# HKUST-Aerial-Robotics/MIND

Measured on AMD Instinct MI355X. Metric: sim steps/sec (whole node) + scenario-tree nodes expanded/sec, AV2 demo scenes, higher is better.
Workload: dtype f32-class (bf16 hi+mid+lo split operands = 24 significand bits, six products, fp32 accumulate) pair kernel + ActorNet, f32 elsewhere in the predictor, f64 iLQR

## Files before the change

### include/mind_hip.h

```cpp
#ifndef MIND_HIP_H
#define MIND_HIP_H

#include <stddef.h>
#include <stdint.h>

#ifdef __cplusplus
extern "C" {
#endif

#define MIND_OK 0
#define MIND_EINVAL (-1)
#define MIND_ENOMEM (-2)
#define MIND_EHIP (-3)
#define MIND_ESTATE (-4)
#define MIND_ENOTFOUND (-5)

typedef struct mind_ctx mind_ctx;

int mind_ctx_create(int device, void *stream, mind_ctx **out);
int mind_ctx_destroy(mind_ctx *ctx);
const char *mind_last_error_string(mind_ctx *ctx);
int mind_ctx_synchronize(mind_ctx *ctx);

typedef struct {
  const char *name;
  const float *data;
  int64_t numel;
} mind_tensor_desc;

int mind_weights_load(mind_ctx *ctx, const mind_tensor_desc *tensors, int n_tensors);

typedef struct {
  int n_scenes;
  const int32_t *actor_off;
  const int32_t *lane_off;
  const float *actors;
  const float *lanes;
  const float *lane_feat;
  const float *actor_ctrs;
  const float *actor_vecs;
  const float *lane_ctrs;
  const float *lane_vecs;
  const float *const *rpe;
  const float *tgt_nodes;
  const float *tgt_rpe;
} mind_scene_batch;

typedef struct {
  float *cls;
  float *reg;
  float *vel;
  float *lane_feat;
  float *actor_emb;
  float *cls_emb;
} mind_pred_out;

int mind_predict_batch(mind_ctx *ctx, const mind_scene_batch *in, mind_pred_out *out);

typedef struct {
  float *cov_vel;
  float *param;
} mind_pred_aux;
int mind_predict_batch_aux(mind_ctx *ctx, const mind_scene_batch *in, mind_pred_out *out, const mind_pred_aux *aux);

#define MIND_BASIS_BEZIER 0
#define MIND_BASIS_MONOMIAL 1
int mind_set_decoder_basis(mind_ctx *ctx, int basis);
int mind_get_decoder_basis(mind_ctx *ctx);

#define MIND_CURVE_MAX_POINTS (1LL << 26)
int mind_curve_eval(mind_ctx *ctx, int basis, const float *param, long long n_rows, const double *tau, int n_tau,
                    float *reg, float *vel, float *cov_vel);
int mind_debug_curve_basis(int basis, const double *tau, int n_tau, float *T, float *Tp);

int mind_last_fusion_stats(mind_ctx *ctx, int *n_launches, float *total_ms, double *pairs_processed);
int mind_last_actor_stats(mind_ctx *ctx, int *layerwise, int *n_launches, int *n_chunks, float *total_ms);
int mind_last_token_stats(mind_ctx *ctx, int *layerwise, int *n_launches, int *n_chunks, float *total_ms);
int mind_last_token_stage_ms(mind_ctx *ctx, float *out_ms, int cap);
int mind_last_ilqr_stats(mind_ctx *ctx, float *kernel_ms, int *n_trees, int *workgroups_per_tree);
int mind_last_ilqr_profile(mind_ctx *ctx, double *out9);
int mind_last_ilqr_trace(mind_ctx *ctx, int tree, int phase, double *out, int cap_rows, int *n_rows);
int mind_set_profiling(mind_ctx *ctx, int enable);
int mind_debug_launch_times(mind_ctx *ctx, int kind, float *clock_ms, float *event_ms, int cap, int *n_clock, int *n_event);
int mind_debug_launch_clock(int n_blocks, int block_slots, int rate_khz, const long long *ops, int n_ops, const unsigned long long *stamps,
                            long long n_slots, double *out, int cap);

#define MIND_PAIR_F32 0
#define MIND_PAIR_BF16X3 1
#define MIND_PAIR_BF16 2
#define MIND_PAIR_BF16X6 3
int mind_set_pair_precision(mind_ctx *ctx, int mode);

int mind_set_tuning(mind_ctx *ctx, const char *name, int value);
int mind_get_tuning(mind_ctx *ctx, const char *name, int *value);
int mind_debug_tuning(int index, const char *name, const char *text, int value, const char **out_name, const char **out_env, int *out_value);
int mind_debug_live_handles(void);
int mind_get_pair_precision(mind_ctx *ctx);
int mind_debug_pack_bfrag(const float *w, int row_stride, uint32_t *out);

int mind_debug_pair_schedule(const int *scene_tokens, const int *scene_actors, int n_scenes, int n_cu, int last_layer, int *out_jobs, int cap,
                             int *out_info);

int mind_debug_predict_choice(const char *const *knob_names, const int *knob_values, int n_knobs, int pair_prec, int n_cu, int have_side,
                              const int *scene_actors, const int *scene_lanes, int n_scenes, long long *out, int cap);

int mind_debug_ilqr_plan(const char *const *knob_names, const int *knob_values, int n_knobs, int n_cu, int mode, int n_trees, const int *n_nodes,
                         const int32_t *parents, long long *out, int cap, int *bad);

int mind_debug_aime_book(int pred_len, int max_depth, int max_rounds, int n_agents, int world, int rank, int force, int n_rounds, const int *dec_len,
                         const float *dec, int n_tokens, int bytes_per_pair, int plan_chunk_mb, int per_scene, long long *out, int cap, char *msg,
                         int msg_cap);

int mind_debug_wait_word(const unsigned *word, unsigned want, double timeout_s, double (*clock)(void *user), void *user, int spins_per_look);

int mind_debug_actor_lw_plan(int n_actors, int np, int chunk, long long *out_launches, int cap, long long *out_info);

int mind_debug_token_lw_plan(int n_tokens, int mode, int chunk, long long *out_launches, int cap, long long *out_info);

int mind_debug_pack_conv_frag(const float *w, int co, int ci, int ksz, uint32_t *out, size_t cap);

int mind_debug_pack(const char *what, const float *w, int a, int b, int c, float *out, size_t cap);
int mind_debug_weight_image(const mind_tensor_desc *tensors, int n_tensors, float *blob, size_t blob_cap, char *names, size_t names_cap,
                            long long *entries, int entries_cap, long long *out_info, char *msg, int msg_cap);
int mind_debug_weight_bind(const mind_tensor_desc *tensors, int n_tensors, const char *drop, char *msg, int msg_cap);

int mind_debug_trig(mind_ctx *ctx, const double *x, int n, double *out);

int mind_debug_dec_scene(mind_ctx *ctx, const float *rows, int n_scenes, int form, float *Cout, float *cls, int reps, float *ms);

int mind_debug_set_layers(mind_ctx *ctx, int n);
int64_t mind_debug_read(mind_ctx *ctx, const char *name, float *host, int64_t max_floats);

typedef struct {
  int n_nodes;
  const int32_t *parent;
  const float *prob;
  int n_agents;
  const float *agent_mean;
  const float *agent_cov;
  const double *field;
  const double *node_w;
} mind_cost_tree;

typedef struct {
  double dt, wheelbase;
  double w_des_state[6];
  double w_state_con[6];
  double state_lower[6], state_upper[6];
  double w_ctrl[2];
  double w_tgt, w_ego, w_ego_cov_offset, w_exo, w_exo_cov_offset, w_exo_cost_offset;
  double grid_res; int grid_w, grid_h;
  int max_iter;
} mind_ilqr_cfg;

typedef struct { int iterations; int converged; double J; double mu; } mind_ilqr_stats;

int mind_ilqr_solve_trees(mind_ctx *ctx, const mind_ilqr_cfg *cfg, const mind_cost_tree *trees,
                          int n_trees, const double *x0, const double *target_lane, int n_lane_pts,
                          double target_vel, int use_exo, const double *us_init, double *xs,
                          double *us, mind_ilqr_stats *stats);

int mind_ilqr_contingency(mind_ctx *ctx, const mind_ilqr_cfg *cfg_warm, const mind_ilqr_cfg *cfg_full,
                          const mind_cost_tree *trees, int n_trees, const double *x0,
                          const double *target_lane, int n_lane_pts, double target_vel, double *xs,
                          double *us, mind_ilqr_stats *stats_warm, mind_ilqr_stats *stats_full);
int mind_ilqr_contingency_begin(mind_ctx *ctx, const mind_ilqr_cfg *cfg_warm, const mind_ilqr_cfg *cfg_full,
                                const mind_cost_tree *trees, int n_trees, const double *x0,
                                const double *target_lane, int n_lane_pts, double target_vel, double *xs,
                                double *us, mind_ilqr_stats *stats_warm, mind_ilqr_stats *stats_full);
int mind_ilqr_contingency_begin_plan(mind_ctx *ctx, const mind_ilqr_cfg *cfg_warm, const mind_ilqr_cfg *cfg_full, const double *x0,
                                     const double *target_lane, int n_lane_pts, double target_vel, double *xs, double *us,
                                     mind_ilqr_stats *stats_warm, mind_ilqr_stats *stats_full);
int mind_ilqr_finish(mind_ctx *ctx);

typedef struct {
  int n_scenes;
  const int32_t *actor_off;
  const float *reg, *vel;
  const float *actor_ctrs, *actor_vecs;
  const float *rot, *orig;
  const float *cov_last;
  const int32_t *last;
  const float *target_lane;
  int n_lane_pts;
  const float *cls;
  const float *scen_prob;
  int lane_check;
  float dist_thres;
} mind_world_in;

typedef struct {
  float *world;
  float *topo;
  float *ego_end;
  float *sel, *sel_prob;
} mind_world_out;

int mind_aime_world(mind_ctx *ctx, const mind_world_in *in, const mind_world_out *out);

int mind_debug_aime_decide(mind_ctx *ctx, int n_scenes, const int32_t *actor_off, const int32_t *cmp, const float *cls, const float *scen_prob,
                           const float *topo, const float *ego_end, const float *world, int lane_check, float dist_thres, float prob_floor,
                           int fused, int by_value, float *sel, float *sel_prob, uint32_t *hit);

typedef struct {
  int n_scenes, n_agents, n_lanes;
  const float *pos, *ang, *vel;
  const float *types;
  const float *pad;
  const float *lane_ctrs, *lane_vecs;
  const float *target_lane;
  const float *target_lane_info;
  int n_lane_pts;
  float time_ahead, min_vel;
  const float *rows_dev;
  const int32_t *parent_slot;
  const int32_t *row0;
  const int32_t *dur;
  int prev_gen;
} mind_rebase_in;

typedef struct {
  float *actors;
  float *actor_ctrs, *actor_vecs;
  float *lane_ctrs, *lane_vecs;
  float *tgt_nodes, *tgt_rpe;
  float *frames;
  int32_t *gen;
} mind_rebase_out;

int mind_aime_rebase(mind_ctx *ctx, const mind_rebase_in *in, const mind_rebase_out *out);

typedef struct {
  int n_agents, n_lanes, n_lane_pts;
  const float *actors;
  const float *actor_ctrs, *actor_vecs;
  const float *lanes;
  const float *lane_ctrs, *lane_vecs;
  const float *tgt_nodes, *tgt_rpe;
  const float *rot, *orig, *tgt_pts;
  const float *hist;
  const float *types;
  const float *target_lane;
  const float *target_lane_info;
  float time_ahead, min_vel, dist_thres;
  int max_depth;
  int max_rounds;
  int pred_len;
  const float *raw_pos, *raw_ang, *raw_vel;
  const float *raw_pad;
  const double *lane_pts;
  const int32_t *lane_flags;
  float travel0;
  const float *script_cls, *script_reg, *script_vel;
  float prob_floor;
  const mind_ilqr_cfg *solve_cfg_warm, *solve_cfg_full;
  const double *solve_x0, *solve_lane;
  int solve_n_lane_pts;
  double solve_target_vel;
} mind_aime_plan_in;

#define MIND_AIME_BRANCH 1
#define MIND_AIME_END 2
#define MIND_AIME_TERMINATE 4
typedef struct {
  int round, scene, mode;
  int parent;
  float prob;
  int cur_t, end_t;
  int flags;
  int dur;
  int64_t row_off;
  float tgt_pts[22];
} mind_aime_node;

typedef struct {
  const mind_aime_node *nodes;
  int n_nodes;
  const float *rows;
  int64_t n_row_floats;
  int n_expanded, n_rounds;
  int root_flags;
  int round_scenes[32];
  float pair_ms;
// ... 233 lines not shown
```

### mind_amd/_lib.py

```python
import ctypes as C
import os

_HERE = os.path.dirname(os.path.abspath(__file__))
LIB_PATH = os.environ.get("MIND_HIP_LIB", os.path.join(_HERE, "libmind_hip.so"))

WAIT_CLOCK = C.CFUNCTYPE(C.c_double, C.c_void_p)
MIND_OK = 0
MIND_EINVAL, MIND_ENOMEM, MIND_EHIP, MIND_ESTATE, MIND_ENOTFOUND = -1, -2, -3, -4, -5


class TensorDesc(C.Structure):
    _fields_ = [("name", C.c_char_p), ("data", C.POINTER(C.c_float)), ("numel", C.c_int64)]


class SceneBatch(C.Structure):
    _fields_ = [("n_scenes", C.c_int), ("actor_off", C.POINTER(C.c_int32)), ("lane_off", C.POINTER(C.c_int32)),
                ("actors", C.c_void_p), ("lanes", C.c_void_p), ("lane_feat", C.c_void_p),
                ("actor_ctrs", C.c_void_p), ("actor_vecs", C.c_void_p), ("lane_ctrs", C.c_void_p),
                ("lane_vecs", C.c_void_p), ("rpe", C.POINTER(C.c_void_p)), ("tgt_nodes", C.c_void_p),
                ("tgt_rpe", C.c_void_p)]


class PredOut(C.Structure):
    _fields_ = [("cls", C.c_void_p), ("reg", C.c_void_p), ("vel", C.c_void_p), ("lane_feat", C.c_void_p),
# ... 47 lines not shown

class AuditRoadEpisodeOut(C.Structure):
    _fields_ = [("step_margin", C.POINTER(C.c_double)), ("step_corner", C.POINTER(C.c_int32)), ("step_ring", C.POINTER(C.c_int32)),
                ("step_edge", C.POINTER(C.c_int32)), ("ego_min", C.POINTER(C.c_double)), ("ego_step", C.POINTER(C.c_int32)),
                ("ego_corner", C.POINTER(C.c_int32)), ("ego_hits", C.POINTER(C.c_int32)), ("ego_first", C.POINTER(C.c_int32))]


class AuditTtcCfg(C.Structure):
    _fields_ = [("horizon", C.c_double), ("bound", C.c_double), ("lanes", C.c_int)]


class AuditTtcOut(C.Structure):
    _fields_ = [("step_ttc", C.POINTER(C.c_double)), ("step_track", C.POINTER(C.c_int32)), ("ego_min", C.POINTER(C.c_double)),
                ("ego_step", C.POINTER(C.c_int32)), ("ego_track", C.POINTER(C.c_int32)), ("ego_hits", C.POINTER(C.c_int32)),
                ("ego_first", C.POINTER(C.c_int32))]


class ForecastCfg(C.Structure):
    _fields_ = [("K", C.c_int), ("T", C.c_int), ("n_h", C.c_int), ("horizon", C.POINTER(C.c_int32)), ("miss_radius", C.c_double),
                ("disc_scale", C.c_double), ("disc_offset", C.c_double)]


FORECAST_OUT = (("ade", "f8", "a", True), ("fde", "f8", "a", True), ("cover", "i4", "a", True), ("first_out", "i4", "a", True),
                ("n_valid", "i4", "a", False), ("last", "i4", "a", False), ("k_ade", "i4", "a", False), ("k_fde", "i4", "a", False),
                ("brier_fde", "f8", "a", False), ("s_n_scored", "i4", "s", False), ("s_ade", "f8", "s", True), ("s_fde", "f8", "s", True),
                ("s_k_ade", "i4", "s", False), ("s_k_fde", "i4", "s", False), ("s_k_top", "i4", "s", False), ("s_brier_fde", "f8", "s", False),
                ("s_miss_rate", "f8", "s", False), ("s_miss_top", "f8", "s", False))


class ForecastOut(C.Structure):
    _fields_ = [(n, C.POINTER(C.c_double if dt == "f8" else C.c_int32)) for n, dt, _, _ in FORECAST_OUT]


class WorldIn(C.Structure):
    _fields_ = [("n_scenes", C.c_int), ("actor_off", C.POINTER(C.c_int32)), ("reg", C.c_void_p), ("vel", C.c_void_p),
                ("actor_ctrs", C.c_void_p), ("actor_vecs", C.c_void_p), ("rot", C.POINTER(C.c_float)),
                ("orig", C.POINTER(C.c_float)), ("cov_last", C.POINTER(C.c_float)), ("last", C.POINTER(C.c_int32)),
                ("target_lane", C.POINTER(C.c_float)), ("n_lane_pts", C.c_int), ("cls", C.c_void_p),
                ("scen_prob", C.POINTER(C.c_float)), ("lane_check", C.c_int), ("dist_thres", C.c_float)]


class WorldOut(C.Structure):
    _fields_ = [("world", C.c_void_p), ("topo", C.c_void_p), ("ego_end", C.c_void_p), ("sel", C.c_void_p), ("sel_prob", C.c_void_p)]


class RebaseIn(C.Structure):
    _fields_ = [("n_scenes", C.c_int), ("n_agents", C.c_int), ("n_lanes", C.c_int), ("pos", C.POINTER(C.c_float)),
                ("ang", C.POINTER(C.c_float)), ("vel", C.POINTER(C.c_float)), ("types", C.POINTER(C.c_float)),
                ("pad", C.POINTER(C.c_float)), ("lane_ctrs", C.POINTER(C.c_float)), ("lane_vecs", C.POINTER(C.c_float)),
                ("target_lane", C.POINTER(C.c_float)), ("target_lane_info", C.POINTER(C.c_float)), ("n_lane_pts", C.c_int),
                ("time_ahead", C.c_float), ("min_vel", C.c_float), ("rows_dev", C.c_void_p), ("parent_slot", C.POINTER(C.c_int32)),
                ("row0", C.POINTER(C.c_int32)), ("dur", C.POINTER(C.c_int32)), ("prev_gen", C.c_int)]


class RebaseOut(C.Structure):
    _fields_ = [("actors", C.c_void_p), ("actor_ctrs", C.c_void_p), ("actor_vecs", C.c_void_p), ("lane_ctrs", C.c_void_p),
                ("lane_vecs", C.c_void_p), ("tgt_nodes", C.c_void_p), ("tgt_rpe", C.c_void_p), ("frames", C.c_void_p),
                ("gen", C.POINTER(C.c_int32))]


class AimePlanIn(C.Structure):
    _fields_ = [("n_agents", C.c_int), ("n_lanes", C.c_int), ("n_lane_pts", C.c_int)] + \
               [(k, C.POINTER(C.c_float)) for k in ("actors", "actor_ctrs", "actor_vecs", "lanes", "lane_ctrs", "lane_vecs", "tgt_nodes", "tgt_rpe",
                                                    "rot", "orig", "tgt_pts", "hist", "types", "target_lane", "target_lane_info")] + \
               [("time_ahead", C.c_float), ("min_vel", C.c_float), ("dist_thres", C.c_float), ("max_depth", C.c_int), ("max_rounds", C.c_int), ("pred_len", C.c_int),
                ("raw_pos", C.POINTER(C.c_float)), ("raw_ang", C.POINTER(C.c_float)), ("raw_vel", C.POINTER(C.c_float)), ("raw_pad", C.POINTER(C.c_float)),
                ("lane_pts", C.POINTER(C.c_double)), ("lane_flags", C.POINTER(C.c_int32)), ("travel0", C.c_float),
                ("script_cls", C.c_void_p), ("script_reg", C.c_void_p), ("script_vel", C.c_void_p), ("prob_floor", C.c_float),
                ("solve_cfg_warm", C.c_void_p), ("solve_cfg_full", C.c_void_p), ("solve_x0", C.c_void_p), ("solve_lane", C.c_void_p),
                ("solve_n_lane_pts", C.c_int), ("solve_target_vel", C.c_double)]


class AimeNode(C.Structure):
    _fields_ = [("round", C.c_int), ("scene", C.c_int), ("mode", C.c_int), ("parent", C.c_int), ("prob", C.c_float),
                ("cur_t", C.c_int), ("end_t", C.c_int), ("flags", C.c_int), ("dur", C.c_int), ("row_off", C.c_int64),
                ("tgt_pts", C.c_float * 22)]


class AimePlanOut(C.Structure):
    _fields_ = [("nodes", C.POINTER(AimeNode)), ("n_nodes", C.c_int), ("rows", C.POINTER(C.c_float)), ("n_row_floats", C.c_int64),
                ("n_expanded", C.c_int), ("n_rounds", C.c_int), ("root_flags", C.c_int), ("round_scenes", C.c_int * 32),
                ("pair_ms", C.c_float), ("pair_launches", C.c_int), ("n_trees", C.c_int), ("tree_top", C.POINTER(C.c_int32)),
                ("tree_off", C.POINTER(C.c_int32)), ("flat_parent", C.POINTER(C.c_int32)), ("flat_prob", C.POINTER(C.c_float)),
                ("flat_mean", C.POINTER(C.c_float)), ("flat_cov", C.POINTER(C.c_float)), ("solves_begun", C.c_int)]


class IlqrCfg(C.Structure):
    _fields_ = [("dt", C.c_double), ("wheelbase", C.c_double), ("w_des_state", C.c_double * 6),
                ("w_state_con", C.c_double * 6), ("state_lower", C.c_double * 6), ("state_upper", C.c_double * 6),
                ("w_ctrl", C.c_double * 2), ("w_tgt", C.c_double), ("w_ego", C.c_double),
                ("w_ego_cov_offset", C.c_double), ("w_exo", C.c_double), ("w_exo_cov_offset", C.c_double),
                ("w_exo_cost_offset", C.c_double), ("grid_res", C.c_double), ("grid_w", C.c_int), ("grid_h", C.c_int),
                ("max_iter", C.c_int)]


class IlqrStats(C.Structure):
    _fields_ = [("iterations", C.c_int), ("converged", C.c_int), ("J", C.c_double), ("mu", C.c_double)]


LOOP_TAN_FN = C.CFUNCTYPE(C.c_double, C.c_double)
LOOP_SINCOS_FN = C.CFUNCTYPE(None, C.c_double, C.POINTER(C.c_double))


class LoopDesc(C.Structure):
    _fields_ = [("n_tracks", C.c_int), ("n_steps", C.c_int), ("clamp_last", C.c_int), ("ego_state", C.c_void_p), ("ego_state_is_f32", C.c_int), ("ego_obs", C.c_void_p), ("ego_trig32", C.c_void_p),
                ("tan_fn", C.c_void_p), ("sincos_fn", C.c_void_p), ("exo_obs", C.c_void_p),
                ("exo_valid", C.c_void_p), ("timestep", C.c_void_p), ("type_slot", C.c_void_p),
                ("sim_step", C.c_double), ("plan_step", C.c_double), ("enable_time", C.c_double),
                ("wheelbase", C.c_double), ("max_speed", C.c_double), ("max_steer", C.c_double), ("max_acc", C.c_double), ("max_dec", C.c_double),
                ("n_lanes", C.c_int), ("lane_pts", C.c_void_p), ("lane_flags", C.c_void_p),
                ("n_lane_pts", C.c_int), ("target_lane", C.c_void_p), ("target_lane_info", C.c_void_p),
                ("time_ahead", C.c_double), ("min_vel", C.c_float), ("dist_thres", C.c_float), ("max_depth", C.c_int), ("max_rounds", C.c_int),
                ("pred_len", C.c_int), ("prob_floor", C.c_float),
                ("cfg_warm", C.c_void_p), ("cfg_full", C.c_void_p), ("solve_n_lane_pts", C.c_int), ("solve_lane", C.c_void_p), ("target_vel", C.c_double),
                ("eval_n_lane_pts", C.c_int), ("eval_lane_is_f32", C.c_int), ("eval_lane", C.c_void_p), ("speculative", C.c_int)]


class LoopTotals(C.Structure):
    _fields_ = [("plans", C.c_longlong), ("expansions", C.c_longlong), ("scen_trees", C.c_longlong), ("rounds", C.c_longlong),
                ("aime_s", C.c_double), ("ilqr_s", C.c_double), ("total_s", C.c_double),
                ("iterations", C.c_longlong), ("node_iterations", C.c_longlong), ("node_iterations_exo", C.c_longlong),
                ("warm_speculated", C.c_longlong), ("warm_hits", C.c_longlong),
                ("pair_ms", C.c_double), ("pair_launches", C.c_longlong), ("scene_n2", C.c_double), ("scene_n_a1", C.c_double),
                ("ilqr_ms", C.c_double), ("ilqr_launches", C.c_longlong), ("ilqr_trees", C.c_longlong), ("ilqr_workgroups_per_tree", C.c_int),
                ("ilqr_prof", C.c_double * 9), ("ilqr_node_steps", C.c_double)]


class LoopOut(C.Structure):
    _fields_ = [("planned", C.c_int), ("enabled", C.c_int), ("n_steps", C.c_longlong), ("n_plans", C.c_longlong), ("episode_steps", C.c_longlong),
                ("sim_time", C.c_double), ("last_trigger", C.c_double), ("state", C.c_double * 4), ("ctrl", C.c_double * 2),
                ("n_agents", C.c_int), ("n_trees", C.c_int), ("best", C.c_int), ("n_expanded", C.c_int), ("n_rounds", C.c_int), ("n_traj_nodes", C.c_int),
                ("costs", C.POINTER(C.c_double)), ("aime_s", C.c_double), ("ilqr_s", C.c_double), ("total_s", C.c_double),
                ("tot", LoopTotals)]


PLANNER_EGO_KEY = -(1 << 63)


class PlannerDesc(C.Structure):
    _fields_ = [("time_ahead", C.c_double), ("min_vel", C.c_float), ("dist_thres", C.c_float), ("max_depth", C.c_int), ("max_rounds", C.c_int),
                ("pred_len", C.c_int), ("prob_floor", C.c_float), ("cfg_warm", C.c_void_p), ("cfg_full", C.c_void_p), ("speculative", C.c_int),
                ("ego_type_slot", C.c_int)]


class PlannerOut(C.Structure):
    _fields_ = [("n_plans", C.c_longlong),
                ("n_agents", C.c_int), ("n_trees", C.c_int), ("best", C.c_int), ("n_expanded", C.c_int), ("n_rounds", C.c_int), ("n_traj_nodes", C.c_int),
                ("costs", C.POINTER(C.c_double)), ("ctrl", C.c_double * 2), ("aime_s", C.c_double), ("ilqr_s", C.c_double), ("total_s", C.c_double),
                ("tot", LoopTotals)]


EXPORTS = ["mind_ctx_create", "mind_ctx_destroy", "mind_last_error_string", "mind_ctx_synchronize",
           "mind_weights_load", "mind_predict_batch", "mind_last_fusion_stats", "mind_last_actor_stats", "mind_debug_actor_lw_plan", "mind_last_token_stats", "mind_last_token_stage_ms", "mind_debug_token_lw_plan", "mind_set_profiling", "mind_debug_launch_times", "mind_debug_launch_clock",
           "mind_ilqr_solve_trees", "mind_ilqr_contingency", "mind_ilqr_solve_fields", "mind_cost_eval", "mind_ilqr_score_trees", "mind_ilqr_gains", "mind_ilqr_policy_rollouts", "mind_lane_dist_field", "mind_aime_world", "mind_aime_rebase", "mind_debug_aime_decide", "mind_debug_set_layers",
           "mind_debug_read", "mind_set_pair_precision", "mind_get_pair_precision", "mind_debug_pack_bfrag", "mind_debug_pack_conv_frag", "mind_debug_pack", "mind_debug_weight_image", "mind_debug_weight_bind", "mind_debug_pair_schedule", "mind_debug_predict_choice", "mind_debug_ilqr_plan", "mind_debug_aime_book", "mind_set_tuning", "mind_get_tuning", "mind_debug_tuning", "mind_debug_live_handles", "mind_last_ilqr_stats", "mind_aime_plan", "mind_last_ilqr_profile", "mind_eval_traj_trees", "mind_last_ilqr_trace", "mind_ilqr_contingency_begin", "mind_ilqr_finish", "mind_fill_tracks", "mind_ilqr_contingency_begin_plan", "mind_debug_trig", "mind_aime_plan_begin", "mind_aime_plan_poll", "mind_aime_plan_finish", "mind_ctx_busy", "mind_ilqr_finish_plan", "mind_debug_dec_scene",
           "mind_set_exchange", "mind_last_exchange_stats", "mind_debug_wait_word",
           "mind_predict_batch_aux", "mind_set_decoder_basis", "mind_get_decoder_basis", "mind_curve_eval", "mind_debug_curve_basis",
           "mind_audit_plan", "mind_audit_episode", "mind_debug_box_clearance",
           "mind_forecast_score", "mind_debug_forecast_score",
           "mind_audit_road_plan", "mind_audit_road_episode", "mind_debug_road_margin",
           "mind_audit_ttc", "mind_debug_box_ttc",
           "mind_loop_create", "mind_loop_destroy", "mind_loop_reset", "mind_loop_advance", "mind_loop_state", "mind_loop_last_plan", "mind_loop_export",
           "mind_planner_create", "mind_planner_destroy", "mind_planner_reset", "mind_planner_observe", "mind_planner_set_lanes", "mind_planner_set_target_lane",
           "mind_planner_set_solve_lane", "mind_planner_set_eval_lane", "mind_planner_plan", "mind_planner_last_plan", "mind_planner_export"]

EXCHANGE_FN = C.CFUNCTYPE(C.c_int, C.c_void_p, C.c_int, C.c_void_p, C.c_void_p, C.c_int64)
XCHG_ALLGATHER, XCHG_ALLREDUCE, XCHG_ALLTOALLV = 0, 1, 2

_lib = None


def load():
    global _lib
    if _lib is not None:
        return _lib
    if not os.path.exists(LIB_PATH):
        raise ImportError(f"{LIB_PATH} is missing: the HIP extension must be built (hipcc --offload-arch=gfx950); "
                          "there is no CPU fallback for the product path")
    lib = C.CDLL(LIB_PATH)
    lib.mind_ctx_create.argtypes = [C.c_int, C.c_void_p, C.POINTER(C.c_void_p)]
    lib.mind_ctx_destroy.argtypes = [C.c_void_p]
    lib.mind_last_error_string.argtypes = [C.c_void_p]
    lib.mind_last_error_string.restype = C.c_char_p
    lib.mind_ctx_synchronize.argtypes = [C.c_void_p]
    lib.mind_weights_load.argtypes = [C.c_void_p, C.POINTER(TensorDesc), C.c_int]
    lib.mind_predict_batch.argtypes = [C.c_void_p, C.POINTER(SceneBatch), C.POINTER(PredOut)]
    lib.mind_predict_batch_aux.argtypes = [C.c_void_p, C.POINTER(SceneBatch), C.POINTER(PredOut), C.POINTER(PredAux)]
    lib.mind_set_decoder_basis.argtypes = [C.c_void_p, C.c_int]
    lib.mind_get_decoder_basis.argtypes = [C.c_void_p]
    lib.mind_curve_eval.argtypes = [C.c_void_p, C.c_int, C.c_void_p, C.c_longlong, C.POINTER(C.c_double), C.c_int, C.c_void_p, C.c_void_p, C.c_void_p]
    lib.mind_debug_curve_basis.argtypes = [C.c_int, C.POINTER(C.c_double), C.c_int, C.POINTER(C.c_float), C.POINTER(C.c_float)]
    lib.mind_last_fusion_stats.argtypes = [C.c_void_p, C.POINTER(C.c_int), C.POINTER(C.c_float), C.POINTER(C.c_double)]
    lib.mind_last_actor_stats.argtypes = [C.c_void_p, C.POINTER(C.c_int), C.POINTER(C.c_int), C.POINTER(C.c_int), C.POINTER(C.c_float)]
    lib.mind_debug_actor_lw_plan.argtypes = [C.c_int, C.c_int, C.c_int, C.POINTER(C.c_longlong), C.c_int, C.POINTER(C.c_longlong)]
    lib.mind_last_token_stats.argtypes = [C.c_void_p, C.POINTER(C.c_int), C.POINTER(C.c_int), C.POINTER(C.c_int), C.POINTER(C.c_float)]
    lib.mind_last_token_stage_ms.argtypes = [C.c_void_p, C.POINTER(C.c_float), C.c_int]
    lib.mind_debug_token_lw_plan.argtypes = [C.c_int, C.c_int, C.c_int, C.POINTER(C.c_longlong), C.c_int, C.POINTER(C.c_longlong)]
    lib.mind_set_profiling.argtypes = [C.c_void_p, C.c_int]
    lib.mind_debug_launch_times.argtypes = [C.c_void_p, C.c_int, C.POINTER(C.c_float), C.POINTER(C.c_float), C.c_int, C.POINTER(C.c_int), C.POINTER(C.c_int)]
    lib.mind_debug_launch_clock.argtypes = [C.c_int, C.c_int, C.c_int, C.POINTER(C.c_longlong), C.c_int, C.POINTER(C.c_ulonglong), C.c_longlong,
                                            C.POINTER(C.c_double), C.c_int]
    lib.mind_ilqr_solve_trees.argtypes = [C.c_void_p, C.POINTER(IlqrCfg), C.POINTER(CostTree), C.c_int,
                                          C.POINTER(C.c_double), C.POINTER(C.c_double), C.c_int, C.c_double, C.c_int,
                                          C.POINTER(C.c_double), C.POINTER(C.c_double), C.POINTER(C.c_double),
                                          C.POINTER(IlqrStats)]
    lib.mind_ilqr_contingency.argtypes = [C.c_void_p, C.POINTER(IlqrCfg), C.POINTER(IlqrCfg), C.POINTER(CostTree), C.c_int,
                                          C.POINTER(C.c_double), C.POINTER(C.c_double), C.c_int, C.c_double,
                                          C.POINTER(C.c_double), C.POINTER(C.c_double), C.POINTER(IlqrStats), C.POINTER(IlqrStats)]
    lib.mind_ilqr_contingency_begin.argtypes = [C.c_void_p, C.POINTER(IlqrCfg), C.POINTER(IlqrCfg), C.POINTER(CostTree), C.c_int,
                                          C.POINTER(C.c_double), C.POINTER(C.c_double), C.c_int, C.c_double,
                                          C.POINTER(C.c_double), C.POINTER(C.c_double), C.POINTER(IlqrStats), C.POINTER(IlqrStats)]
    lib.mind_ilqr_finish.argtypes = [C.c_void_p]
    lib.mind_ilqr_contingency_begin_plan.argtypes = [C.c_void_p, C.POINTER(IlqrCfg), C.POINTER(IlqrCfg), C.c_void_p, C.c_void_p, C.c_int, C.c_double,
                                                     C.c_void_p, C.c_void_p, C.c_void_p, C.c_void_p]
    lib.mind_fill_tracks.argtypes = [C.c_void_p, C.c_int, C.c_int, C.c_void_p, C.c_void_p, C.c_void_p, C.c_void_p, C.c_void_p, C.c_void_p]
    lib.mind_ilqr_solve_fields.argtypes = [C.c_void_p, C.POINTER(IlqrCfg), C.POINTER(FieldGrid), C.POINTER(CostTree), C.c_int,
                                           C.POINTER(C.c_double), C.POINTER(C.c_double), C.POINTER(C.c_double),
                                           C.POINTER(C.c_double), C.POINTER(IlqrStats)]
    lib.mind_cost_eval.argtypes = [C.c_void_p, C.POINTER(IlqrCfg), C.POINTER(FieldGrid), C.POINTER(CostTree),
                                   C.POINTER(C.c_double), C.POINTER(C.c_double), C.c_int, C.c_double, C.c_int, C.c_int,
                                   C.POINTER(C.c_int32), C.POINTER(C.c_double), C.POINTER(C.c_double), C.POINTER(C.c_double)]
    lib.mind_ilqr_score_trees.argtypes = [C.c_void_p, C.POINTER(IlqrCfg), C.POINTER(FieldGrid), C.POINTER(CostTree), C.c_int,
                                          C.POINTER(C.c_double), C.POINTER(C.c_double), C.c_int, C.c_double, C.c_int, C.c_int,
                                          C.POINTER(C.c_double), C.POINTER(C.c_double), C.POINTER(C.c_double), C.POINTER(C.c_double)]
    lib.mind_ilqr_gains.argtypes = [C.c_void_p, C.POINTER(IlqrCfg), C.POINTER(FieldGrid), C.POINTER(CostTree), C.c_int,
                                    C.POINTER(C.c_double), C.POINTER(C.c_double), C.c_int, C.c_double, C.c_int,
                                    C.POINTER(C.c_double), C.POINTER(C.c_double), C.POINTER(IlqrGainsOut)]
    lib.mind_ilqr_policy_rollouts.argtypes = [C.c_void_p, C.POINTER(IlqrCfg), C.POINTER(FieldGrid), C.POINTER(CostTree), C.c_int,
                                              C.POINTER(C.c_double), C.POINTER(C.c_double), C.c_int, C.c_double, C.c_int,
                                              C.POINTER(C.c_double), C.POINTER(C.c_double), C.POINTER(C.c_double), C.c_int,
                                              C.POINTER(C.c_double), C.POINTER(C.c_double), C.POINTER(C.c_double), C.POINTER(C.c_double),
                                              C.POINTER(C.c_double), C.POINTER(C.c_double)]
    lib.mind_lane_dist_field.argtypes = [C.c_void_p, C.POINTER(C.c_double), C.POINTER(C.c_double), C.c_int, C.c_int, C.c_int,
                                         C.c_double] + [C.POINTER(C.c_double)] * 4
    lib.mind_aime_world.argtypes = [C.c_void_p, C.POINTER(WorldIn), C.POINTER(WorldOut)]
    lib.mind_aime_rebase.argtypes = [C.c_void_p, C.POINTER(RebaseIn), C.POINTER(RebaseOut)]
    lib.mind_debug_aime_decide.argtypes = [C.c_void_p, C.c_int, C.POINTER(C.c_int32), C.POINTER(C.c_int32), C.c_void_p, C.POINTER(C.c_float), C.c_void_p,
                                           C.c_void_p, C.c_void_p, C.c_int, C.c_float, C.c_float, C.c_int, C.c_int, C.c_void_p, C.c_void_p, C.c_void_p]
    lib.mind_aime_plan.argtypes = [C.c_void_p, C.POINTER(AimePlanIn), C.POINTER(AimePlanOut)]
    lib.mind_aime_plan_begin.argtypes = [C.c_void_p, C.POINTER(AimePlanIn)]
    lib.mind_aime_plan_poll.argtypes = [C.c_void_p]
    lib.mind_aime_plan_finish.argtypes = [C.c_void_p, C.POINTER(AimePlanOut)]
    lib.mind_ctx_busy.argtypes = [C.c_void_p]
    lib.mind_ilqr_finish_plan.argtypes = [C.c_void_p, C.c_int, C.c_int, C.c_void_p, C.c_void_p, C.c_void_p, C.c_void_p]
    lib.mind_set_pair_precision.argtypes = [C.c_void_p, C.c_int]
    lib.mind_set_tuning.argtypes = [C.c_void_p, C.c_char_p, C.c_int]
    lib.mind_get_tuning.argtypes = [C.c_void_p, C.c_char_p, C.POINTER(C.c_int)]
    lib.mind_debug_tuning.argtypes = [C.c_int, C.c_char_p, C.c_char_p, C.c_int, C.POINTER(C.c_char_p), C.POINTER(C.c_char_p), C.POINTER(C.c_int)]
    lib.mind_debug_live_handles.argtypes = []
    lib.mind_last_ilqr_stats.argtypes = [C.c_void_p, C.POINTER(C.c_float), C.POINTER(C.c_int), C.POINTER(C.c_int)]
    lib.mind_last_ilqr_profile.argtypes = [C.c_void_p, C.POINTER(C.c_double)]
    lib.mind_last_ilqr_trace.argtypes = [C.c_void_p, C.c_int, C.c_int, C.POINTER(C.c_double), C.c_int, C.POINTER(C.c_int)]
    lib.mind_eval_traj_trees.argtypes = [C.POINTER(C.c_double), C.POINTER(C.c_double), C.POINTER(C.c_int32), C.c_int, C.c_void_p, C.c_int, C.c_int,
                                         C.c_double, C.POINTER(C.c_double)]
    lib.mind_get_pair_precision.argtypes = [C.c_void_p]
    lib.mind_debug_pack_bfrag.argtypes = [C.POINTER(C.c_float), C.c_int, C.POINTER(C.c_uint32)]
    lib.mind_debug_pair_schedule.argtypes = [C.POINTER(C.c_int), C.POINTER(C.c_int), C.c_int, C.c_int, C.c_int, C.POINTER(C.c_int), C.c_int, C.POINTER(C.c_int)]
    lib.mind_debug_predict_choice.argtypes = [C.POINTER(C.c_char_p), C.POINTER(C.c_int), C.c_int, C.c_int, C.c_int, C.c_int, C.POINTER(C.c_int), C.POINTER(C.c_int),
                                              C.c_int, C.POINTER(C.c_longlong), C.c_int]
    lib.mind_debug_ilqr_plan.argtypes = [C.POINTER(C.c_char_p), C.POINTER(C.c_int), C.c_int, C.c_int, C.c_int, C.c_int, C.POINTER(C.c_int), C.POINTER(C.c_int32),
                                         C.POINTER(C.c_longlong), C.c_int, C.POINTER(C.c_int)]
    lib.mind_debug_wait_word.argtypes = [C.POINTER(C.c_uint), C.c_uint, C.c_double, WAIT_CLOCK, C.c_void_p, C.c_int]
    lib.mind_debug_aime_book.argtypes = [C.c_int] * 8 + [C.POINTER(C.c_int), C.POINTER(C.c_float)] + [C.c_int] * 4 + [C.POINTER(C.c_longlong), C.c_int, C.c_char_p, C.c_int]
    lib.mind_debug_trig.argtypes = [C.c_void_p, C.POINTER(C.c_double), C.c_int, C.POINTER(C.c_double)]
    lib.mind_debug_pack_conv_frag.argtypes = [C.POINTER(C.c_float), C.c_int, C.c_int, C.c_int, C.POINTER(C.c_uint32), C.c_size_t]
    lib.mind_debug_pack.argtypes = [C.c_char_p, C.POINTER(C.c_float), C.c_int, C.c_int, C.c_int, C.POINTER(C.c_float), C.c_size_t]
    lib.mind_debug_weight_image.argtypes = [C.POINTER(TensorDesc), C.c_int, C.POINTER(C.c_float), C.c_size_t, C.c_char_p, C.c_size_t,
                                            C.POINTER(C.c_longlong), C.c_int, C.POINTER(C.c_longlong), C.c_char_p, C.c_int]
    lib.mind_debug_weight_bind.argtypes = [C.POINTER(TensorDesc), C.c_int, C.c_char_p, C.c_char_p, C.c_int]
    lib.mind_debug_dec_scene.argtypes = [C.c_void_p, C.POINTER(C.c_float), C.c_int, C.c_int, C.POINTER(C.c_float), C.POINTER(C.c_float), C.c_int, C.POINTER(C.c_float)]
    lib.mind_debug_set_layers.argtypes = [C.c_void_p, C.c_int]
    lib.mind_debug_read.argtypes = [C.c_void_p, C.c_char_p, C.POINTER(C.c_float), C.c_int64]
    lib.mind_set_exchange.argtypes = [C.c_void_p, C.c_int, C.c_int, EXCHANGE_FN, C.c_void_p, C.c_int]
    lib.mind_last_exchange_stats.argtypes = [C.c_void_p, C.POINTER(C.c_longlong), C.POINTER(C.c_longlong)]
    lib.mind_loop_create.argtypes = [C.c_void_p, C.POINTER(LoopDesc), C.POINTER(C.c_void_p)]
    lib.mind_loop_destroy.argtypes = [C.c_void_p]
    lib.mind_loop_reset.argtypes = [C.c_void_p]
    lib.mind_loop_advance.argtypes = [C.c_void_p, C.c_int, C.c_double, C.c_longlong, C.POINTER(LoopOut)]
    lib.mind_loop_state.argtypes = [C.c_void_p, C.POINTER(LoopOut)]
    lib.mind_loop_last_plan.argtypes = [C.c_void_p, C.POINTER(AimePlanOut)] + [C.POINTER(C.c_void_p)] * 6 + [C.c_void_p]
    lib.mind_loop_export.argtypes = [C.c_void_p, C.c_int, C.POINTER(C.c_int), C.c_void_p, C.c_void_p, C.c_void_p]
    lib.mind_planner_create.argtypes = [C.c_void_p, C.POINTER(PlannerDesc), C.POINTER(C.c_void_p)]
    lib.mind_planner_destroy.argtypes = [C.c_void_p]
    lib.mind_planner_reset.argtypes = [C.c_void_p]
    lib.mind_planner_observe.argtypes = [C.c_void_p, C.c_int, C.c_void_p, C.c_int, C.c_void_p, C.c_void_p, C.c_void_p]
    lib.mind_planner_set_lanes.argtypes = [C.c_void_p, C.c_int, C.c_void_p, C.c_void_p]
    lib.mind_planner_set_target_lane.argtypes = [C.c_void_p, C.c_int, C.c_void_p, C.c_void_p]
    lib.mind_planner_set_solve_lane.argtypes = [C.c_void_p, C.c_int, C.c_void_p, C.c_double]
    lib.mind_planner_set_eval_lane.argtypes = [C.c_void_p, C.c_int, C.c_void_p, C.c_int]
    lib.mind_planner_plan.argtypes = [C.c_void_p, C.c_void_p, C.c_void_p, C.POINTER(PlannerOut)]
    lib.mind_planner_last_plan.argtypes = [C.c_void_p, C.POINTER(AimePlanOut)] + [C.POINTER(C.c_void_p)] * 6 + [C.c_void_p]
    lib.mind_planner_export.argtypes = [C.c_void_p, C.c_int, C.POINTER(C.c_int), C.c_void_p, C.c_void_p, C.c_void_p]
    lib.mind_audit_plan.argtypes = [C.c_void_p, C.POINTER(AuditBox), C.c_double, C.POINTER(CostTree), C.c_int, C.c_int, C.POINTER(C.c_double),
                                    C.POINTER(AuditPlanOut)]
    lib.mind_audit_episode.argtypes = [C.c_void_p, C.POINTER(AuditBox), C.c_int, C.c_int, C.c_int, C.POINTER(C.c_double), C.POINTER(C.c_double),
                                       C.POINTER(C.c_uint8), C.POINTER(C.c_double), C.POINTER(AuditEpisodeOut)]
    lib.mind_debug_box_clearance.argtypes = [C.c_int, C.c_int, C.POINTER(C.c_double), C.POINTER(C.c_double), C.POINTER(C.c_double), C.POINTER(C.c_double)]
    fc_tail = [C.POINTER(ForecastCfg), C.c_int, C.POINTER(C.c_int32), C.c_void_p, C.c_void_p, C.POINTER(C.c_double), C.POINTER(C.c_uint8),
               C.POINTER(C.c_uint8), C.POINTER(ForecastOut)]
    lib.mind_forecast_score.argtypes = [C.c_void_p] + fc_tail
    lib.mind_debug_forecast_score.argtypes = fc_tail
    road = [C.POINTER(C.c_double), C.POINTER(C.c_int32), C.c_int]
    lib.mind_audit_road_plan.argtypes = [C.c_void_p, C.POINTER(AuditBox)] + road + [C.POINTER(CostTree), C.c_int, C.c_int, C.POINTER(C.c_double),
                                                                                   C.POINTER(AuditRoadPlanOut)]
    lib.mind_audit_road_episode.argtypes = [C.c_void_p, C.POINTER(AuditBox)] + road + [C.c_int, C.c_int, C.POINTER(C.c_double),
                                                                                      C.POINTER(AuditRoadEpisodeOut)]
    lib.mind_debug_road_margin.argtypes = [C.c_int, C.POINTER(C.c_double), C.POINTER(AuditBox)] + road + [C.POINTER(C.c_double), C.POINTER(C.c_double)] + \
        [C.POINTER(C.c_int32)] * 3
    lib.mind_audit_ttc.argtypes = [C.c_void_p, C.POINTER(AuditBox), C.POINTER(AuditTtcCfg), C.c_int, C.c_int, C.c_int, C.POINTER(C.c_double),
                                   C.POINTER(C.c_double), C.POINTER(C.c_uint8), C.POINTER(C.c_double), C.POINTER(AuditTtcOut)]
    lib.mind_debug_box_ttc.argtypes = [C.c_int, C.POINTER(C.c_double), C.POINTER(C.c_double), C.POINTER(C.c_double), C.POINTER(C.c_double)]
    for n in EXPORTS:
        getattr(lib, n)
        if n not in ("mind_last_error_string", "mind_debug_read"):
            getattr(lib, n).restype = C.c_int
    lib.mind_debug_read.restype = C.c_int64
    _lib = lib
    return lib


PRED_CHOICE_FIELDS = ("header", "n_runs", "np", "actor_form", "actor_arg", "actor_grid", "actor_chunk", "actor_chunks", "actor_launches", "qsplit", "qk_stride",
                      "tiled", "edge_bf16", "edge_pair_bytes", "tok_chunk", "tok_lw", "tok_chunks", "pair_family", "pair_np", "l5_jobs5", "xcd_lanes",
                      "xcd_lanes5", "dec_actor", "dec_np", "fp32_dec", "split_dec", "want_mw", "mw_blocks", "cls_on_side", "tgt_wait_first",
                      "dec_head_ra", "dec_chain_g")
PAIR_PREC = ("f32", "bf16x3", "bf16", "bf16x6")


def predict_choice(knobs, prec, scenes, n_cu=256, have_side=True):
    lib = load()
    names = (C.c_char_p * max(1, len(knobs)))(*[k.encode() for k in knobs])
    vals = (C.c_int * max(1, len(knobs)))(*[int(v) for v in knobs.values()])
    sa = (C.c_int * len(scenes))(*[a for a, _ in scenes])
    sl = (C.c_int * len(scenes))(*[l for _, l in scenes])
    cap = 32 + 6 * len(scenes)
    out = (C.c_longlong * cap)()
    n = lib.mind_debug_predict_choice(names, vals, len(knobs), PAIR_PREC.index(prec) if isinstance(prec, str) else prec, n_cu, int(have_side),
                                      sa, sl, len(scenes), out, cap)
    if n == MIND_EINVAL:
        return None
    assert 0 < n <= cap and out[0] == 32 and n == 32 + 6 * out[1], n
    d = dict(zip(PRED_CHOICE_FIELDS, out[:32]))
    d["runs"] = [tuple(out[32 + 6 * i:38 + 6 * i]) for i in range(out[1])]
    return d


def dec_scene(lib, ctx, rows, form, reps=1, timed=False):
    import numpy as np
    rows = np.ascontiguousarray(rows, np.float32)
    B = rows.shape[0]
    assert rows.shape == (B, 128)
    fp = C.POINTER(C.c_float)
    cout, cls, ms = np.empty((B, 6, 128), np.float32), np.empty((B, 6), np.float32), np.zeros(reps, np.float32)
    check(lib, ctx, lib.mind_debug_dec_scene(ctx, rows.ctypes.data_as(fp), B, int(form), cout.ctypes.data_as(fp), cls.ctypes.data_as(fp), reps,
                                             ms.ctypes.data_as(fp) if timed else None), "mind_debug_dec_scene")
    return (cout, cls, ms) if timed else (cout, cls)


def knobs():
    lib = load()
    name, env, val = C.c_char_p(), C.c_char_p(), C.c_int()
    rows = []
    while not rows or len(rows) < n:
        n = lib.mind_debug_tuning(len(rows), None, None, 0, C.byref(name), C.byref(env), C.byref(val))
        assert n > 0, n
        rows.append((name.value.decode(), env.value.decode() if env.value else None, val.value))
    return rows


def knob_stored(name, value=None, text=None):
    val = C.c_int()
    rc = load().mind_debug_tuning(-1, name.encode(), None if text is None else text.encode(), 0 if value is None else int(value), None, None, C.byref(val))
    return val.value if rc == MIND_OK else None


ILQR_PLAN_FIELDS = ("header", "n_trees", "form", "G", "GS", "spec", "nslot", "grid", "workgroups_per_tree", "host_out", "early", "starve_followers")
ILQR_TREE_FIELDS = ("M", "nl", "nseg", "nsl", "maxls", "nfs")
ILQR_TREE_TABLES = ("level_start", "level_nodes", "child_start", "child_list", "seg_start", "seg_nodes", "slevel_start", "slevel_segs", "seg_rec",
                    "fstep_start", "fstep_items", "fstep_q1", "fstep_nstart", "fstep_nodes")


def ilqr_plan(knobs, parents, n_cu=256, generic=False, evaluate=False, two_fits=False):
    lib = load()
    names = (C.c_char_p * max(1, len(knobs)))(*[k.encode() for k in knobs])
    vals = (C.c_int * max(1, len(knobs)))(*[int(v) for v in knobs.values()])
    nn = (C.c_int * len(parents))(*[len(p) for p in parents])
    flat = [int(v) for p in parents for v in p]
    par = (C.c_int32 * max(1, len(flat)))(*flat)
    bad = (C.c_int * 2)()
    mode = int(generic) | int(evaluate) << 1 | int(two_fits) << 2
    n = lib.mind_debug_ilqr_plan(names, vals, len(knobs), n_cu, mode, len(parents), nn, par, None, 0, bad)
    if n == MIND_EINVAL:
        return {"bad": (bad[0], bad[1])} if bad[0] >= 0 else None
    out = (C.c_longlong * n)()
    assert lib.mind_debug_ilqr_plan(names, vals, len(knobs), n_cu, mode, len(parents), nn, par, out, n, bad) == n and out[0] == 16
    d = dict(zip(ILQR_PLAN_FIELDS, out[:12]))
    d["trees"], o = [], 16
    for _ in parents:
        tr = dict(zip(ILQR_TREE_FIELDS, out[o:o + 6]))
        lens, o = out[o + 6:o + 20], o + 20
        for name, ln in zip(ILQR_TREE_TABLES, lens):
            tr[name], o = list(out[o:o + ln]), o + ln
        d["trees"].append(tr)
    assert o == n
    return d


AIME_ROUND_FIELDS = ("B", "lo", "hi", "Bmax", "chunk", "S", "s0", "Sm", "any")
AIME_NODE_FIELDS = ("round", "scene", "mode", "parent", "prob", "cur_t", "end_t", "flags", "dur", "row_off", "owner", "lscene")


def aime_book(pred_len, max_depth, n_agents, rounds, world=1, rank=0, force=False, max_rounds=32, n_tokens=0, bytes_per_pair=512, plan_chunk_mb=96 * 1024,
              per_scene=1):
    import numpy as np
    lib = load()
    arrs = [np.ascontiguousarray(r, np.float32).ravel() for r in rounds]
    lens = (C.c_int * max(1, len(arrs)))(*[a.size for a in arrs])
    dec = np.concatenate(arrs + [np.zeros(1, np.float32)])
    msg = C.create_string_buffer(256)
    args = [pred_len, max_depth, max_rounds, n_agents, world, rank, int(force), len(arrs), lens, dec.ctypes.data_as(C.POINTER(C.c_float)), n_tokens,
            bytes_per_pair, plan_chunk_mb, per_scene]
    n = lib.mind_debug_aime_book(*args, None, 0, msg, 256)
    if n == MIND_EINVAL:
        return None
    out = (C.c_longlong * n)()
# ... 223 lines not shown
```

### mind_amd/csrc/actor_mfma_kernels.hip

```cpp
#include <hip/hip_runtime.h>
#include <stdint.h>

#define AM_T 1024
#ifdef MIND_ACTOR_TRACE
__device__ long long am_tr_[64];
__device__ int am_trn_;
#define AM_MARK() do { if (blockIdx.x == 0 && threadIdx.x == 0) { const long long n_ = clock64(); am_tr_[am_trn_ & 63] = n_; ++am_trn_; } } while (0)
#else
#define AM_MARK() do {} while (0)
#endif
#define AM_WAVES 16
#define AM_MAXT 2
#define AM_RSD(C) (3 * (C) / 2 + 4)
#define AM_BUF 2496
#define AM_XIN 0
#define AM_O0 1344
#define AM_FA (AM_O0 + 7 * AM_BUF)
#define AM_RED (AM_FA + 48 * AM_RSD(128))
#define AM_LDS_DWORDS (AM_RED + 64)

#include "weight_tables.h"
#include "launch_clock.h"
typedef u32 u32x2 __attribute__((ext_vector_type(2)));

__device__ __forceinline__ float am_block_sum(float v, float *red, int flip) {
  v = wave_sum(v);
  float *r = red + (flip & 1) * 32;
  if ((threadIdx.x & 63) == 0) r[threadIdx.x >> 6] = v;
  __syncthreads();
  float s = 0.f;
#pragma unroll
  for (int w = 0; w < AM_WAVES; ++w) s += r[w];
  return s;
}

template <int NP>
__device__ __forceinline__ void am_store_split(u32 *rowp, int plane, const f32x4 &y) {
  u32x2 h, m, l;
  h[0] = pk_bf16(y[0], y[1]); h[1] = pk_bf16(y[2], y[3]);
  *(u32x2 *)rowp = h;
  if (NP == 1) return;
  const float r0 = y[0] - bf_lo_f32(h[0]), r1 = y[1] - bf_hi_f32(h[0]), r2 = y[2] - bf_lo_f32(h[1]), r3 = y[3] - bf_hi_f32(h[1]);
  m[0] = pk_bf16(r0, r1); m[1] = pk_bf16(r2, r3);
  *(u32x2 *)(rowp + plane) = m;
  l[0] = pk_bf16(r0 - bf_lo_f32(m[0]), r1 - bf_hi_f32(m[0])); l[1] = pk_bf16(r2 - bf_lo_f32(m[1]), r3 - bf_hi_f32(m[1]));
  *(u32x2 *)(rowp + 2 * plane) = l;
}
template <int NP>
__device__ __forceinline__ f32x4 am_load_split(const u32 *rowp, int plane) {
  const u32x2 h = *(const u32x2 *)rowp;
  f32x4 y = {bf_lo_f32(h[0]), bf_hi_f32(h[0]), bf_lo_f32(h[1]), bf_hi_f32(h[1])};
  if (NP == 1) return y;
  const u32x2 m = *(const u32x2 *)(rowp + plane), l = *(const u32x2 *)(rowp + 2 * plane);
  y[0] = (y[0] + bf_lo_f32(m[0])) + bf_lo_f32(l[0]); y[1] = (y[1] + bf_hi_f32(m[0])) + bf_hi_f32(l[0]);
  y[2] = (y[2] + bf_lo_f32(m[1])) + bf_lo_f32(l[1]); y[3] = (y[3] + bf_hi_f32(m[1])) + bf_hi_f32(l[1]);
  return y;
}

template <int NP, int LGC , int KSZ, int STRIDE>
__device__ __forceinline__ void am_conv(const u32 *in, int Tin, const u32 *__restrict__ Wf, int Cout, int Tout,
                                        f32x4 (&acc)[AM_MAXT]) {
  constexpr int CP = 1 << LGC, RSD = AM_RSD(CP), PLANE = CP / 2, PAD = (KSZ - 1) / 2;
  constexpr int KS = (KSZ * CP + 31) / 32;
  const int lane = threadIdx.x & 63, wave = threadIdx.x >> 6;
  const int r = lane & 15, q = lane >> 4;
  const int ntt = (Tout + 15) >> 4;
  const int tiles = (Cout >> 4) * ntt;
#pragma unroll
  for (int i = 0; i < AM_MAXT; ++i) {
    acc[i] = (f32x4){0.f, 0.f, 0.f, 0.f};
    const int ti = wave + AM_WAVES * i;
    if (ti >= tiles) continue;
    const int mt = ti / ntt, nt = ti - mt * ntt;
    const int t = nt * 16 + r;
    const u32 *wp = Wf + (size_t)mt * KS * 768 + lane * 4;
    f32x4 corr = {0.f, 0.f, 0.f, 0.f};
#pragma unroll 4
    for (int ks = 0; ks < KS; ++ks) {
      const u32x4 ah = *(const u32x4 *)(wp + (size_t)ks * 768);
      u32x4 am, al;
      if (NP >= 3) am = *(const u32x4 *)(wp + (size_t)ks * 768 + 256);
      if (NP == 6) al = *(const u32x4 *)(wp + (size_t)ks * 768 + 512);
      const int k0 = ks * 32 + q * 8;
      const int dk = k0 >> LGC, ci = k0 & (CP - 1);
      const int row = t * STRIDE + dk - PAD;
      u32x4 bh = {0u, 0u, 0u, 0u}, bm = {0u, 0u, 0u, 0u}, bl = {0u, 0u, 0u, 0u};
      if (dk < KSZ && t < Tout && row >= 0 && row < Tin) {
        const u32 *bp = in + row * RSD + (ci >> 1);
        bh = *(const u32x4 *)bp;
        if (NP >= 3) bm = *(const u32x4 *)(bp + PLANE);
        if (NP == 6) bl = *(const u32x4 *)(bp + 2 * PLANE);
      }
      acc[i] = MFMA_BF(ah, bh, acc[i]);
      if (NP >= 3) {
        if (NP == 6) {
          corr = MFMA_BF(al, bh, corr);
          corr = MFMA_BF(ah, bl, corr);
          corr = MFMA_BF(am, bm, corr);
        }
        corr = MFMA_BF(am, bh, corr);
        corr = MFMA_BF(ah, bm, corr);
      }
    }
    if (NP >= 3) acc[i] += corr;
  }
}

template <int NP>
__device__ __forceinline__ void am_gn(f32x4 (&acc)[AM_MAXT], int Cout, int Tout, const float *__restrict__ g,
                                      const float *__restrict__ b, const u32 *resid, const float *up, bool relu, u32 *outs,
                                      float *outf, float *__restrict__ gout, float *red) {
  const int lane = threadIdx.x & 63, wave = threadIdx.x >> 6;
  const int r = lane & 15, q = lane >> 4;
  const int ntt = (Tout + 15) >> 4;
  const int tiles = (Cout >> 4) * ntt;
  const int RSD = AM_RSD(Cout), PLANE = Cout >> 1;
  f32x4 gg[AM_MAXT], bb[AM_MAXT];
  float s = 0.f;
#pragma unroll
  for (int i = 0; i < AM_MAXT; ++i) {
    const int ti = wave + AM_WAVES * i;
    if (ti >= tiles) continue;
    const int mt = ti / ntt, nt = ti - mt * ntt;
    gg[i] = *(const f32x4 *)(g + mt * 16 + q * 4);
    bb[i] = *(const f32x4 *)(b + mt * 16 + q * 4);
    if (nt * 16 + r < Tout) s += (acc[i][0] + acc[i][1]) + (acc[i][2] + acc[i][3]);
  }
  const float n = (float)(Cout * Tout);
  const float mean = am_block_sum(s, red, 0) / n;
  float v = 0.f;
#pragma unroll
  for (int i = 0; i < AM_MAXT; ++i) {
    const int ti = wave + AM_WAVES * i;
    if (ti >= tiles) continue;
    const int nt = ti % ntt;
    if (nt * 16 + r < Tout) {
#pragma unroll
      for (int e = 0; e < 4; ++e) { const float d = acc[i][e] - mean; v = fmaf(d, d, v); }
    }
  }
  const float rstd = 1.0f / sqrtf(am_block_sum(v, red, 1) / n + 1e-5f);
#pragma unroll
  for (int i = 0; i < AM_MAXT; ++i) {
    const int ti = wave + AM_WAVES * i;
    if (ti >= tiles) continue;
    const int mt = ti / ntt, nt = ti - mt * ntt;
    const int t = nt * 16 + r, co = mt * 16 + q * 4;
    if (t >= Tout) continue;
    f32x4 y;
#pragma unroll
    for (int e = 0; e < 4; ++e) y[e] = (acc[i][e] - mean) * rstd * gg[i][e] + bb[i][e];
    if (resid) y += am_load_split<NP>(resid + t * RSD + (co >> 1), PLANE);
    if (up) {
      const int Th = Tout >> 1;
      float sp = (t + 0.5f) * 0.5f - 0.5f;
      sp = sp < 0.f ? 0.f : sp;
      const int i0 = (int)sp;
      const int i1 = i0 + 1 < Th ? i0 + 1 : Th - 1;
      const float l1 = sp - (float)i0;
      const f32x4 a0 = *(const f32x4 *)(up + i0 * 132 + co), a1 = *(const f32x4 *)(up + i1 * 132 + co);
#pragma unroll
      for (int e = 0; e < 4; ++e) y[e] += (1.0f - l1) * a0[e] + l1 * a1[e];
    }
    if (relu) {
#pragma unroll
      for (int e = 0; e < 4; ++e) y[e] = fmaxf(y[e], 0.f);
    }
    if (gout) {
      if (t == Tout - 1) *(f32x4 *)(gout + co) = y;
    } else if (outf) {
      *(f32x4 *)(outf + t * 132 + co) = y;
    } else {
      am_store_split<NP>(outs + t * RSD + (co >> 1), PLANE, y);
    }
  }
  __syncthreads();
}

template <int NP, int LGCI, int LGCO, int STRIDE, bool DS>
__device__ __forceinline__ void am_res(const u32 *in, int Tin, const AmRes &W, u32 *out, u32 *t1, u32 *t2, float *red) {
  constexpr int Cout = 1 << LGCO;
  const int Tout = Tin / STRIDE;
  f32x4 acc[AM_MAXT];
  am_conv<NP, LGCI, 3, STRIDE>(in, Tin, W.c1, Cout, Tout, acc);
  AM_MARK();
  am_gn<NP>(acc, Cout, Tout, W.g1, W.b1, nullptr, nullptr, true, t1, nullptr, nullptr, red);
  AM_MARK();
  const u32 *resid = in;
  if (DS) {
    am_conv<NP, LGCI, 1, STRIDE>(in, Tin, W.ds, Cout, Tout, acc);
    AM_MARK();
    am_gn<NP>(acc, Cout, Tout, W.gd, W.bd, nullptr, nullptr, false, t2, nullptr, nullptr, red);
    AM_MARK();
    resid = t2;
  }
  am_conv<NP, LGCO, 3, 1>(t1, Tout, W.c2, Cout, Tout, acc);
  AM_MARK();
  am_gn<NP>(acc, Cout, Tout, W.g2, W.b2, resid, nullptr, true, out, nullptr, nullptr, red);
  AM_MARK();
}

template <int NP, int LGC>
__device__ __forceinline__ void am_lateral(const u32 *src, int T, const AmLat &W, const float *up, float *dstf, u32 *dsts,
                                           float *red) {
  f32x4 acc[AM_MAXT];
  am_conv<NP, LGC, 3, 1>(src, T, W.w, 128, T, acc);
  AM_MARK();
  am_gn<NP>(acc, 128, T, W.g, W.b, nullptr, up, false, dsts, dstf, nullptr, red);
  AM_MARK();
}

template <int NP>
__global__ __launch_bounds__(AM_T) void k_actor_mfma(const float *__restrict__ actors , int n_actors,
                                                     float *__restrict__ out , AmW W, LcSlot *clk) {
  lc_stamp_in(clk);
  extern __shared__ __attribute__((aligned(16))) u32 smu[];
  u32 *xin = smu + AM_XIN;
  u32 *o0 = smu + AM_O0, *o1 = o0 + AM_BUF, *o2 = o1 + AM_BUF, *o3 = o2 + AM_BUF;
  u32 *ta = o3 + AM_BUF, *tb = ta + AM_BUF, *tc = tb + AM_BUF;
  u32 *fa = smu + AM_FA;
  float *red = (float *)(smu + AM_RED);
  const int tid = threadIdx.x;
  const int a = blockIdx.x;
  if (a >= n_actors) { lc_stamp_both(clk); return; }
  if (tid < 48 * 8) {
    const int t = tid >> 3, c = (tid & 7) * 2;
    const float v0 = c < 14 ? actors[((size_t)a * 14 + c) * 48 + t] : 0.f;
    const float v1 = c + 1 < 14 ? actors[((size_t)a * 14 + c + 1) * 48 + t] : 0.f;
    u32 *p = xin + t * AM_RSD(16) + (c >> 1);
    const u32 h = pk_bf16(v0, v1);
    const float r0 = v0 - bf_lo_f32(h), r1 = v1 - bf_hi_f32(h);
    const u32 m = pk_bf16(r0, r1);
    p[0] = h; p[8] = m; p[16] = pk_bf16(r0 - bf_lo_f32(m), r1 - bf_hi_f32(m));
  }
  __syncthreads();
#ifdef MIND_ACTOR_TRACE
  if (blockIdx.x == 0 && tid == 0) am_trn_ = 0;
#endif
  AM_MARK();
  am_res<NP, 4, 5, 1, true>(xin, 48, W.res[0], ta, tb, tc, red);
  am_res<NP, 5, 5, 1, false>(ta, 48, W.res[1], o0, tb, tc, red);
  am_res<NP, 5, 6, 2, true>(o0, 48, W.res[2], ta, tb, tc, red);
  am_res<NP, 6, 6, 1, false>(ta, 24, W.res[3], o1, tb, tc, red);
  am_res<NP, 6, 7, 2, true>(o1, 24, W.res[4], ta, tb, tc, red);
  am_res<NP, 7, 7, 1, false>(ta, 12, W.res[5], o2, tb, tc, red);
  am_res<NP, 7, 8, 2, true>(o2, 12, W.res[6], ta, tb, tc, red);
  am_res<NP, 8, 8, 1, false>(ta, 6, W.res[7], o3, tb, tc, red);
  am_lateral<NP, 8>(o3, 6, W.lat[3], nullptr, (float *)ta, nullptr, red);
  am_lateral<NP, 7>(o2, 12, W.lat[2], (const float *)ta, (float *)tb, nullptr, red);
  am_lateral<NP, 6>(o1, 24, W.lat[1], (const float *)tb, (float *)o2, nullptr, red);
  am_lateral<NP, 5>(o0, 48, W.lat[0], (const float *)o2, nullptr, fa, red);
  {
    const AmRes &R = W.res[8];
    f32x4 acc[AM_MAXT];
    am_conv<NP, 7, 3, 1>(fa, 48, R.c1, 128, 48, acc);
    AM_MARK();
    am_gn<NP>(acc, 128, 48, R.g1, R.b1, nullptr, nullptr, true, o0, nullptr, nullptr, red);
    AM_MARK();
    am_conv<NP, 7, 3, 1>(o0, 48, R.c2, 128, 48, acc);
    AM_MARK();
    am_gn<NP>(acc, 128, 48, R.g2, R.b2, fa, nullptr, true, nullptr, nullptr, out + (size_t)a * 128, red);
    AM_MARK();
  }
#ifdef MIND_ACTOR_TRACE
  if (blockIdx.x == 0 && tid == 0) {
    printf("[k_actor_mfma<%d>] cycles conv/gn per stage:", NP);
    for (int q = 1; q < am_trn_ && q < 64; ++q) printf(" %lld", am_tr_[q] - am_tr_[q - 1]);
    printf("\n");
  }
#endif
  lc_stamp_out(clk);
}
extern "C" size_t mind_actor_mfma_lds_bytes() { return (size_t)AM_LDS_DWORDS * sizeof(u32); }
```

### mind_amd/csrc/encdec_kernels.hip

```cpp
#include <hip/hip_runtime.h>
#include <stdint.h>

#include "weight_tables.h"
#include "dec_curve.h"
#include "launch_clock.h"
#include "dec_chain.h"

typedef float f32x4 __attribute__((ext_vector_type(4)));

#define NT 256

__device__ __forceinline__ float wave_sum(float v) {
  v += __shfl_xor(v, 32, 64);
  v += __shfl_xor(v, 16, 64);
  v += __shfl_xor(v, 8, 64);
  v += __shfl_xor(v, 4, 64);
  v += __shfl_xor(v, 2, 64);
  v += __shfl_xor(v, 1, 64);
  return v;
}

__device__ __forceinline__ float block_sum(float v, float *red) {
  v = wave_sum(v);
  __syncthreads();
  if ((threadIdx.x & 63) == 0) red[threadIdx.x >> 6] = v;
  __syncthreads();
  return red[0] + red[1] + red[2] + red[3];
}

#ifndef DB
#define DB 16
#endif
#define DENSE_ROW_FENCE() __builtin_amdgcn_sched_barrier(0)
#define DBQ 8
template <int R>
__device__ __forceinline__ void dense_quads(const float *in, int ldi, int K, const float *__restrict__ WT,
                                            const float *__restrict__ b, int NOUT, float *out, int ldo,
                                            float *part, int part_floats) {
  const int nthr = blockDim.x;
  const int NQ = NOUT >> 2;
  int KP = 1;
  while (KP * 2 * NQ <= nthr && KP * 2 * R * NOUT <= part_floats && KP * 2 <= (K >> 2)) KP *= 2;
  const int Kc = ((K / 4 + KP - 1) / KP) * 4;
  for (int item = threadIdx.x; item < KP * NQ; item += nthr) {
    const int kp = item / NQ, o = (item % NQ) * 4;
    float acc[R][4];
#pragma unroll
    for (int r = 0; r < R; ++r)
#pragma unroll
      for (int c = 0; c < 4; ++c) acc[r][c] = (KP == 1 && b) ? b[o + c] : 0.f;
    const int k0 = kp * Kc, k1 = min(K, k0 + Kc);
    int k = k0;
    for (; k + DBQ <= k1; k += DBQ) {
      f32x4 w[DBQ];
#pragma unroll
      for (int q = 0; q < DBQ; ++q) w[q] = *(const f32x4 *)(WT + (size_t)(k + q) * NOUT + o);
#pragma unroll
      for (int r = 0; r < R; ++r) {
#pragma unroll
        for (int q4 = 0; q4 < DBQ / 4; ++q4) {
          const f32x4 x = *(const f32x4 *)(in + r * ldi + k + 4 * q4);
#pragma unroll
          for (int j = 0; j < 4; ++j)
#pragma unroll
            for (int c = 0; c < 4; ++c) acc[r][c] = fmaf(w[4 * q4 + j][c], x[j], acc[r][c]);
        }
        DENSE_ROW_FENCE();
      }
    }
    for (; k < k1; k += 4) {
#pragma unroll
      for (int j = 0; j < 4; ++j) {
        const f32x4 w = *(const f32x4 *)(WT + (size_t)(k + j) * NOUT + o);
#pragma unroll
        for (int r = 0; r < R; ++r) {
          const float x = in[r * ldi + k + j];
#pragma unroll
          for (int c = 0; c < 4; ++c) acc[r][c] = fmaf(w[c], x, acc[r][c]);
        }
      }
    }
#pragma unroll
    for (int r = 0; r < R; ++r)
#pragma unroll
      for (int c = 0; c < 4; ++c) {
        if (KP == 1) out[r * ldo + o + c] = acc[r][c];
        else part[(kp * R + r) * NOUT + o + c] = acc[r][c];
      }
  }
  if (KP == 1) return;
  __syncthreads();
  for (int i = threadIdx.x; i < R * NOUT; i += nthr) {
    const int r = i / NOUT, oo = i % NOUT;
    float v = b ? b[oo] : 0.f;
    for (int q = 0; q < KP; ++q) v += part[(q * R + r) * NOUT + oo];
    out[r * ldo + oo] = v;
  }
}

#ifndef DT
#define DT 1024
#endif
template <int R>
__device__ __forceinline__ void dense_quads_part(const float *in, int ldi, int K, const float *__restrict__ WT, const float *__restrict__ b, int NOUT,
                                                 float *out, int ldo, float *part, int part_floats, int wg, int G) {
  const int nthr = blockDim.x;
  const int NQ = NOUT >> 2;
  int KP = 1;
  while (KP * 2 * NQ <= DT && KP * 2 * R * NOUT <= part_floats && KP * 2 <= (K >> 2)) KP *= 2;
  const int Kc = ((K / 4 + KP - 1) / KP) * 4;
  const int q_lo = NQ * wg / G, q_hi = NQ * (wg + 1) / G, NQg = q_hi - q_lo;
  for (int item = threadIdx.x; item < KP * NQg; item += nthr) {
    const int kp = item / NQg, o = (q_lo + item % NQg) * 4;
    float acc[R][4];
#pragma unroll
    for (int r = 0; r < R; ++r)
#pragma unroll
      for (int c = 0; c < 4; ++c) acc[r][c] = (KP == 1 && b) ? b[o + c] : 0.f;
    const int k0 = kp * Kc, k1 = min(K, k0 + Kc);
    int k = k0;
    for (; k + DBQ <= k1; k += DBQ) {
      f32x4 w[DBQ];
#pragma unroll
      for (int q = 0; q < DBQ; ++q) w[q] = *(const f32x4 *)(WT + (size_t)(k + q) * NOUT + o);
#pragma unroll
      for (int r = 0; r < R; ++r) {
#pragma unroll
        for (int q4 = 0; q4 < DBQ / 4; ++q4) {
          const f32x4 x = *(const f32x4 *)(in + r * ldi + k + 4 * q4);
#pragma unroll
          for (int j = 0; j < 4; ++j)
#pragma unroll
            for (int c = 0; c < 4; ++c) acc[r][c] = fmaf(w[4 * q4 + j][c], x[j], acc[r][c]);
        }
        DENSE_ROW_FENCE();
      }
    }
    for (; k < k1; k += 4) {
#pragma unroll
      for (int j = 0; j < 4; ++j) {
        const f32x4 w = *(const f32x4 *)(WT + (size_t)(k + j) * NOUT + o);
#pragma unroll
        for (int r = 0; r < R; ++r) {
          const float x = in[r * ldi + k + j];
#pragma unroll
          for (int c = 0; c < 4; ++c) acc[r][c] = fmaf(w[c], x, acc[r][c]);
        }
      }
    }
#pragma unroll
    for (int r = 0; r < R; ++r)
#pragma unroll
      for (int c = 0; c < 4; ++c) {
        if (KP == 1) out[r * ldo + o + c] = acc[r][c];
        else part[(kp * R + r) * NOUT + o + c] = acc[r][c];
      }
  }
  if (KP == 1) return;
  __syncthreads();
  const int o_lo = q_lo * 4, no = NQg * 4;
  for (int i = threadIdx.x; i < R * no; i += nthr) {
    const int r = i / no, oo = o_lo + i % no;
    float v = b ? b[oo] : 0.f;
    for (int q = 0; q < KP; ++q) v += part[(q * R + r) * NOUT + oo];
    out[r * ldo + oo] = v;
  }
}

#define DEC_SYNC_SPINS (1u << 22)
__device__ __forceinline__ bool dec_grid_sync(unsigned *bar, int G, unsigned *abort_word) {
  __shared__ int sh_ab;
  __syncthreads();
  if (threadIdx.x == 0) {
// ... 51 lines not shown
    return;
  }
  int KP = 1;
  if (part && NOUT < nthr) {
    KP = nthr / NOUT;
    while (KP > 1 && (KP * R * NOUT > part_floats || (K / 4) < KP)) KP >>= 1;
    int p2 = 1;
    while (p2 * 2 <= KP) p2 *= 2;
    KP = p2;
  }
  if (KP == 1) {
    for (int o = threadIdx.x; o < NOUT; o += nthr) {
      float acc[R];
      const float bv = b ? b[o] : 0.f;
#pragma unroll
      for (int r = 0; r < R; ++r) acc[r] = bv;
      int k = 0;
      for (; k + DB <= K; k += DB) {
        float w[DB];
#pragma unroll
        for (int q = 0; q < DB; ++q) w[q] = WT[(size_t)(k + q) * NOUT + o];
#pragma unroll
        for (int r = 0; r < R; ++r) {
#pragma unroll
          for (int q4 = 0; q4 < DB / 4; ++q4) {
            const f32x4 x = *(const f32x4 *)(in + r * ldi + k + 4 * q4);
            acc[r] = fmaf(w[4 * q4 + 0], x[0], acc[r]);
            acc[r] = fmaf(w[4 * q4 + 1], x[1], acc[r]);
            acc[r] = fmaf(w[4 * q4 + 2], x[2], acc[r]);
            acc[r] = fmaf(w[4 * q4 + 3], x[3], acc[r]);
          }
        DENSE_ROW_FENCE();
        }
      }
      for (; k < K; k += 4) {
#pragma unroll
        for (int r = 0; r < R; ++r) {
          const f32x4 x = *(const f32x4 *)(in + r * ldi + k);
#pragma unroll
          for (int q = 0; q < 4; ++q) acc[r] = fmaf(WT[(size_t)(k + q) * NOUT + o], x[q], acc[r]);
        }
      }
#pragma unroll
      for (int r = 0; r < R; ++r) out[r * ldo + o] = acc[r];
    }
    return;
  }
  const int kp = threadIdx.x / NOUT, o = threadIdx.x % NOUT;
  const int Kc = ((K / 4 + KP - 1) / KP) * 4;
  if (kp < KP) {
    float acc[R];
#pragma unroll
    for (int r = 0; r < R; ++r) acc[r] = 0.f;
    const int k0 = kp * Kc, k1 = min(K, k0 + Kc);
    int k = k0;
    for (; k + DB <= k1; k += DB) {
      float w[DB];
#pragma unroll
      for (int q = 0; q < DB; ++q) w[q] = WT[(size_t)(k + q) * NOUT + o];
#pragma unroll
      for (int r = 0; r < R; ++r) {
#pragma unroll
        for (int q4 = 0; q4 < DB / 4; ++q4) {
          const f32x4 x = *(const f32x4 *)(in + r * ldi + k + 4 * q4);
          acc[r] = fmaf(w[4 * q4 + 0], x[0], acc[r]);
          acc[r] = fmaf(w[4 * q4 + 1], x[1], acc[r]);
          acc[r] = fmaf(w[4 * q4 + 2], x[2], acc[r]);
          acc[r] = fmaf(w[4 * q4 + 3], x[3], acc[r]);
        }
        DENSE_ROW_FENCE();
      }
    }
    for (; k < k1; k += 4) {
#pragma unroll
      for (int r = 0; r < R; ++r) {
        const f32x4 x = *(const f32x4 *)(in + r * ldi + k);
#pragma unroll
        for (int q = 0; q < 4; ++q) acc[r] = fmaf(WT[(size_t)(k + q) * NOUT + o], x[q], acc[r]);
      }
    }
#pragma unroll
    for (int r = 0; r < R; ++r) part[(kp * R + r) * NOUT + o] = acc[r];
  }
  __syncthreads();
  for (int i = threadIdx.x; i < R * NOUT; i += nthr) {
    const int r = i / NOUT, oo = i % NOUT;
    float v = b ? b[oo] : 0.f;
    for (int q = 0; q < KP; ++q) v += part[(q * R + r) * NOUT + oo];
    out[r * ldo + oo] = v;
  }
}

constexpr int dense_scalar_kp(int R, int NOUT, int K, int nthr, int part_floats) {
  int KP = NOUT < nthr ? nthr / NOUT : 1;
  while (KP > 1 && (KP * R * NOUT > part_floats || (K / 4) < KP)) KP >>= 1;
  int p2 = 1;
  while (p2 * 2 <= KP) p2 *= 2;
  return p2;
}

template <int R, int RPT>
__device__ __forceinline__ void dense_ksplit(const float *in, int ldi, int K, const float *__restrict__ WT, const float *__restrict__ b, int NOUT,
                                             float *out, int ldo, float *part, int KP) {
  const int nthr = blockDim.x;
  constexpr int NG = (R + RPT - 1) / RPT;
  const int Kc = ((K / 4 + KP - 1) / KP) * 4;
  for (int item = threadIdx.x; item < NG * KP * NOUT; item += nthr) {
    const int o = item % NOUT, kp = (item / NOUT) % KP, r0 = (item / (NOUT * KP)) * RPT;
    float acc[RPT];
#pragma unroll
    for (int j = 0; j < RPT; ++j) acc[j] = 0.f;
    const int k0 = kp * Kc, k1 = min(K, k0 + Kc);
    int k = k0;
    for (; k + DB <= k1; k += DB) {
      float w[DB];
#pragma unroll
      for (int q = 0; q < DB; ++q) w[q] = WT[(size_t)(k + q) * NOUT + o];
#pragma unroll
      for (int j = 0; j < RPT; ++j) {
        if (r0 + j >= R) continue;
#pragma unroll
        for (int q4 = 0; q4 < DB / 4; ++q4) {
          const f32x4 x = *(const f32x4 *)(in + (r0 + j) * ldi + k + 4 * q4);
          acc[j] = fmaf(w[4 * q4 + 0], x[0], acc[j]);
          acc[j] = fmaf(w[4 * q4 + 1], x[1], acc[j]);
          acc[j] = fmaf(w[4 * q4 + 2], x[2], acc[j]);
          acc[j] = fmaf(w[4 * q4 + 3], x[3], acc[j]);
        }
      }
    }
    for (; k < k1; k += 4) {
#pragma unroll
      for (int j = 0; j < RPT; ++j) {
        if (r0 + j >= R) continue;
        const f32x4 x = *(const f32x4 *)(in + (r0 + j) * ldi + k);
#pragma unroll
        for (int q = 0; q < 4; ++q) acc[j] = fmaf(WT[(size_t)(k + q) * NOUT + o], x[q], acc[j]);
      }
    }
#pragma unroll
    for (int j = 0; j < RPT; ++j)
      if (r0 + j < R) part[(kp * R + r0 + j) * NOUT + o] = acc[j];
  }
  __syncthreads();
  for (int i = threadIdx.x; i < R * NOUT; i += nthr) {
    const int r = i / NOUT, oo = i % NOUT;
    float v = b ? b[oo] : 0.f;
    for (int q = 0; q < KP; ++q) v += part[(q * R + r) * NOUT + oo];
    out[r * ldo + oo] = v;
  }
}

#define LN_REGS 12
__device__ __forceinline__ void ln_rows(float *buf, int ld, int R, int n, const float *__restrict__ g,
                                        const float *__restrict__ be, bool relu) {
  const int lane = threadIdx.x & 63, wave = threadIdx.x >> 6, nw = blockDim.x >> 6;
  for (int r = wave; r < R; r += nw) {
    if (n <= 64 * LN_REGS) {
      float xv[LN_REGS], gv[LN_REGS], bv[LN_REGS];
#pragma unroll
      for (int i = 0; i < LN_REGS; ++i) {
        const int k = lane + 64 * i;
        const bool in = k < n;
        xv[i] = in ? buf[r * ld + k] : 0.f;
        gv[i] = in ? g[k] : 0.f;
        bv[i] = in ? be[k] : 0.f;
      }
      float s = 0.f;
#pragma unroll
      for (int i = 0; i < LN_REGS; ++i) if (lane + 64 * i < n) s += xv[i];
      const float mean = wave_sum(s) / (float)n;
      float v = 0.f;
#pragma unroll
      for (int i = 0; i < LN_REGS; ++i) if (lane + 64 * i < n) { const float d = xv[i] - mean; v = fmaf(d, d, v); }
      const float rstd = 1.0f / sqrtf(wave_sum(v) / (float)n + 1e-5f);
#pragma unroll
      for (int i = 0; i < LN_REGS; ++i) {
        const int k = lane + 64 * i;
        if (k < n) {
          float y = (xv[i] - mean) * rstd * gv[i] + bv[i];
          if (relu) y = fmaxf(y, 0.f);
          buf[r * ld + k] = y;
        }
      }
      continue;
    }
    float s = 0.f;
    for (int k = lane; k < n; k += 64) s += buf[r * ld + k];
    const float mean = wave_sum(s) / (float)n;
    float v = 0.f;
    for (int k = lane; k < n; k += 64) { const float d = buf[r * ld + k] - mean; v = fmaf(d, d, v); }
    const float rstd = 1.0f / sqrtf(wave_sum(v) / (float)n + 1e-5f);
    for (int k = lane; k < n; k += 64) {
      float y = (buf[r * ld + k] - mean) * rstd * g[k] + be[k];
      if (relu) y = fmaxf(y, 0.f);
      buf[r * ld + k] = y;
    }
  }
}

#define PL 2
#define LR (PL * 10)

#ifndef DT
#define DT 1024
#endif
__global__ __launch_bounds__(DT) void k_lane_net(const float *__restrict__ feats, int n_poly,
                                                 float *__restrict__ out, LaneW W) {
  __shared__ __attribute__((aligned(16))) float xin[LR][16];
  __shared__ __attribute__((aligned(16))) float x[LR][128];
  __shared__ __attribute__((aligned(16))) float hcat[LR][256];
  __shared__ __attribute__((aligned(16))) float t1[LR][128];
  __shared__ __attribute__((aligned(16))) float part[2 * LR * 128];
  const int PF = 2 * LR * 128;
  const int tid = threadIdx.x;
  const int p0 = blockIdx.x * PL;
  for (int i = tid; i < LR * 16; i += blockDim.x) {
    const int r = i / 16, c = i % 16;
    const int pl = p0 + r / 10;
    xin[r][c] = pl < n_poly ? feats[((size_t)pl * 10 + r % 10) * 16 + c] : 0.f;
  }
  __syncthreads();
  dense<LR>(&xin[0][0], 16, 16, W.pW, W.pb, 128, &x[0][0], 128, part, PF);
  __syncthreads();
  ln_rows(&x[0][0], 128, LR, 128, W.pg, W.pbe, true);
  __syncthreads();
  for (int blk = 0; blk < 2; ++blk) {
    dense<LR>(&x[0][0], 128, 128, W.f10W[blk], W.f10b[blk], 128, &t1[0][0], 128, part, PF);
    __syncthreads();
    ln_rows(&t1[0][0], 128, LR, 128, W.f10g[blk], W.f10be[blk], true);
    __syncthreads();
    dense<LR>(&t1[0][0], 128, 128, W.f13W[blk], W.f13b[blk], 128, &hcat[0][0], 256, part, PF);
    __syncthreads();
    ln_rows(&hcat[0][0], 256, LR, 128, W.f13g[blk], W.f13be[blk], true);
    __syncthreads();
    for (int i = tid; i < PL * 128; i += blockDim.x) {
      const int pl = i / 128, c = i % 128;
      float m = hcat[pl * 10][c];
      for (int q = 1; q < 10; ++q) m = fmaxf(m, hcat[pl * 10 + q][c]);
      for (int q = 0; q < 10; ++q) hcat[pl * 10 + q][128 + c] = m;
    }
    __syncthreads();
    dense<LR>(&hcat[0][0], 256, 256, W.f20W[blk], W.f20b[blk], 128, &t1[0][0], 128, part, PF);
    __syncthreads();
    ln_rows(&t1[0][0], 128, LR, 128, W.f20g[blk], W.f20be[blk], true);
    __syncthreads();
    dense<LR>(&t1[0][0], 128, 128, W.f23W[blk], W.f23b[blk], 128, &hcat[0][0], 256, part, PF);
    __syncthreads();
    ln_rows(&hcat[0][0], 256, LR, 128, W.f23g[blk], W.f23be[blk], true);
    __syncthreads();
    for (int i = tid; i < LR * 128; i += blockDim.x) x[i / 128][i % 128] += hcat[i / 128][i % 128];
    __syncthreads();
    ln_rows(&x[0][0], 128, LR, 128, W.ng[blk], W.nbe[blk], false);
    __syncthreads();
  }
  for (int i = tid; i < PL * 128; i += blockDim.x) {
    const int pl = i / 128, c = i % 128;
    if (p0 + pl < n_poly) {
      float m = x[pl * 10][c];
      for (int q = 1; q < 10; ++q) m = fmaxf(m, x[pl * 10 + q][c]);
      out[(size_t)(p0 + pl) * 128 + c] = m;
    }
  }
}

#ifndef AT
#define AT 1024
#endif

template <int TCH, int STRIDE, int KSZ>
__device__ __forceinline__ void conv_chunk(const float *in, int Cin, int Tin, const float *__restrict__ W,
                                           int Cout, int Tout, float *out, float *part, int KP) {
  constexpr int SPAN = (TCH - 1) * STRIDE + KSZ, PAD = (KSZ - 1) / 2;
  const int tid = threadIdx.x;
  const int nch = (Tout + TCH - 1) / TCH;
  const int CG = Cout >> 2;
  const int groups = CG * nch;
  const int kp = tid / groups, g = tid % groups;
  const int co = (g % CG) * 4, t0 = (g / CG) * TCH;
  const int cpk = (Cin + KP - 1) / KP;
  if (kp < KP) {
    float acc[4][TCH];
#pragma unroll
    for (int c = 0; c < 4; ++c)
#pragma unroll
      for (int i = 0; i < TCH; ++i) acc[c][i] = 0.f;
    const int c0 = kp * cpk, c1 = min(Cin, c0 + cpk);
    const int base = t0 * STRIDE - PAD;
#ifndef CONV_UNROLL
#define CONV_UNROLL 4
#endif
#pragma unroll CONV_UNROLL
    for (int ci = c0; ci < c1; ++ci) {
      f32x4 w[KSZ];
      float xw[SPAN];
#pragma unroll
      for (int dk = 0; dk < KSZ; ++dk) w[dk] = *(const f32x4 *)(W + ((size_t)ci * KSZ + dk) * Cout + co);
#pragma unroll
      for (int j = 0; j < SPAN; ++j) {
        const int ti = base + j;
        xw[j] = (ti >= 0 && ti < Tin) ? in[ci * Tin + ti] : 0.f;
      }
#pragma unroll
      for (int dk = 0; dk < KSZ; ++dk)
#pragma unroll
        for (int i = 0; i < TCH; ++i) {
          const float x = xw[i * STRIDE + dk];
#pragma unroll
          for (int c = 0; c < 4; ++c) acc[c][i] = fmaf(w[dk][c], x, acc[c][i]);
        }
      DENSE_ROW_FENCE();
    }
    float *dst = KP > 1 ? part + (size_t)kp * Cout * Tout : out;
#pragma unroll
    for (int c = 0; c < 4; ++c)
#pragma unroll
      for (int i = 0; i < TCH; ++i)
        if (t0 + i < Tout) dst[(co + c) * Tout + t0 + i] = acc[c][i];
  }
  if (KP > 1) {
    __syncthreads();
    for (int i = tid; i < Cout * Tout; i += AT) {
      float v = part[i];
      for (int q = 1; q < KP; ++q) v += part[(size_t)q * Cout * Tout + i];
      out[i] = v;
    }
  }
}

template <int STRIDE, int KSZ>
__device__ __forceinline__ void conv(const float *in, int Cin, int Tin, const float *W, int Cout, int Tout,
                                     float *out, float *part, int part_floats) {
const int groups = (Cout >> 2) * ((Tout + 2) / 3);
  int KP = AT / groups;
  while (KP > 1 && (KP * Cout * Tout > part_floats || KP > Cin)) KP >>= 1;
  if (KP < 1) KP = 1;
  conv_chunk<3, STRIDE, KSZ>(in, Cin, Tin, W, Cout, Tout, out, part, KP);
}

__device__ __forceinline__ float block_sum_a(float v, float *red, int flip) {
  v = wave_sum(v);
  float *r = red + (flip & 1) * 16;
  if ((threadIdx.x & 63) == 0) r[threadIdx.x >> 6] = v;
  __syncthreads();
  float s = 0.f;
#pragma unroll
  for (int w = 0; w < AT / 64; ++w) s += r[w];
  return s;
}

#define GN_NE 6
__device__ __forceinline__ void gn(float *buf, int C, int T, const float *__restrict__ g,
                                   const float *__restrict__ b, const float *resid, bool relu, float *red) {
  const int n = C * T;
  float x[GN_NE], gg[GN_NE], bb[GN_NE];
  float s = 0.f;
#pragma unroll
  for (int e = 0; e < GN_NE; ++e) {
    const int i = threadIdx.x + e * AT;
    if (i < n) {
      const int c = i / T;
      x[e] = buf[i];
      gg[e] = g[c];
      bb[e] = b[c];
      s += x[e];
    }
  }
  const float mean = block_sum_a(s, red, 0) / (float)n;
  float v = 0.f;
#pragma unroll
  for (int e = 0; e < GN_NE; ++e)
    if ((int)threadIdx.x + e * AT < n) { const float d = x[e] - mean; v = fmaf(d, d, v); }
  const float rstd = 1.0f / sqrtf(block_sum_a(v, red, 1) / (float)n + 1e-5f);
#pragma unroll
  for (int e = 0; e < GN_NE; ++e) {
    const int i = threadIdx.x + e * AT;
    if (i < n) {
      float y = (x[e] - mean) * rstd * gg[e] + bb[e];
      if (resid) y += resid[i];
      if (relu) y = fmaxf(y, 0.f);
      buf[i] = y;
    }
  }
  __syncthreads();
}

__device__ __forceinline__ void res1d(const float *in, int Cin, int Tin, const ResW &w, int Cout, int stride,
                                      float *out, float *t1, float *t2, float *red, float *part, int pf) {
  const int Tout = Tin / stride;
  if (stride == 1) conv<1, 3>(in, Cin, Tin, w.c1, Cout, Tout, t1, part, pf);
  else conv<2, 3>(in, Cin, Tin, w.c1, Cout, Tout, t1, part, pf);
  __syncthreads();
  gn(t1, Cout, Tout, w.g1, w.b1, nullptr, true, red);
  conv<1, 3>(t1, Cout, Tout, w.c2, Cout, Tout, out, part, pf);
  __syncthreads();
  const float *resid = in;
  if (w.ds) {
    if (stride == 1) conv<1, 1>(in, Cin, Tin, w.ds, Cout, Tout, t2, part, pf);
    else conv<2, 1>(in, Cin, Tin, w.ds, Cout, Tout, t2, part, pf);
    __syncthreads();
      gn(t2, Cout, Tout, w.gd, w.bd, nullptr, false, red);
      resid = t2;
  }
  gn(out, Cout, Tout, w.g2, w.b2, resid, true, red);
}

#define ACT_PART 12288
#define ACT_LDS_FLOATS (672 + 7 * 1536 + 2 * 6144 + 32 + ACT_PART)
__global__ __launch_bounds__(AT) void k_actor_net(const float *__restrict__ actors, int n_actors,
// ... 552 lines not shown
```

### mind_amd/csrc/mind_hip.hip

```cpp
#include <hip/hip_runtime.h>

#include <cmath>
#include <cstdarg>
#include <cstdio>
#include <cstdlib>
#include <algorithm>
#include <cstring>
#include <map>
#include <memory>
#include <string>
#include <thread>
#include <atomic>
#include <functional>
#include <vector>

#include "../../include/mind_hip.h"
#include "encdec_kernels.hip"
#include "fusion_kernels.hip"
#include "pair_bf16_kernels.hip"
#include "pair_tile_kernels.hip"
#include "pair_tile6_kernels.hip"
#include "token_mfma_kernels.hip"
#include "actor_mfma_kernels.hip"
#include "actor_lw_kernels.hip"
// ... 19 lines not shown
static_assert(TN_RA == RA && TN_IL_SLOTS == IL_SLOTS, "tuning.h restates the two kernel constants its clamps need");

static std::atomic<long> live_handles{0};

template <class H, hipError_t (*Release)(H)> struct Owned {
  H p = nullptr;
  size_t cap = 0;
  Owned() = default;
  Owned(Owned &&o) noexcept : p(o.p), cap(o.cap) { o.p = nullptr; o.cap = 0; }
  Owned &operator=(Owned &&o) noexcept { if (this != &o) { reset(); p = o.p; cap = o.cap; o.p = nullptr; o.cap = 0; } return *this; }
  ~Owned() { reset(); }
  operator H() const { return p; }
  template <class T> T *as() const { return (T *)p; }
  void reset() {
    if (p) { (void)Release(p); live_handles.fetch_sub(1, std::memory_order_relaxed); }
    p = nullptr; cap = 0;
  }
  hipError_t took(hipError_t e, size_t bytes = 0) {
    if (e == hipSuccess) { live_handles.fetch_add(1, std::memory_order_relaxed); cap = bytes; } else p = nullptr;
    return e;
  }
};
struct Event : Owned<hipEvent_t, hipEventDestroy> { hipError_t create(unsigned flags = hipEventDefault) { reset(); return took(hipEventCreateWithFlags(&p, flags)); } };
struct Stream : Owned<hipStream_t, hipStreamDestroy> { hipError_t create() { reset(); return took(hipStreamCreateWithFlags(&p, hipStreamNonBlocking)); } };
struct Pinned : Owned<void *, hipHostFree> {
  hipError_t alloc(size_t bytes, unsigned flags = hipHostMallocDefault) { reset(); return took(hipHostMalloc(&p, bytes, flags), bytes); }
};
struct DevBuf : Owned<void *, hipFree> {
  hipError_t alloc(size_t bytes) { reset(); return took(hipMalloc(&p, bytes), bytes); }
};

struct TableSet {
  std::vector<int> key;
  DevBuf meta, jobs, jobs5, rows;
  std::vector<int> actor_row, cls_row, scene_n;
  long long edge_pairs = 0, edge_pairs_t = 0, stamp = 0;
  int ntok = 0, slot = 0, njobs = 0, njobs5 = 0;
  double pairs_full = 0, pairs_l5 = 0;
};
#define MIND_TABLE_SETS 8

struct mind_ctx {
  int device = 0;
  hipStream_t stream = nullptr;
  Stream side;
  Event ev_side, ev_main, ev_stage, ev_tgt, ev_cls;
  std::vector<char> aime_stage;
  bool aime_stage_busy = false;
  std::string err;
  DevBuf wdev;
  bool have_weights = false;
  WeightTables W = {};
  PredTuning pt; IlqrTuning it; CtxTuning ct;
  TnRefs knobs() { return {&pt, &it, &ct}; }
  int dec_basis = MIND_BASIS_BEZIER;
  DevBuf curve_tab;
  std::vector<double> curve_tau;
  int curve_tab_basis = -1;
  DevBuf tok_lw_arena;
  std::vector<TlLaunch> tok_lw_plan;
  int last_tok_lw = 0, last_tok_launches = 0, last_tok_chunks = 0;
  float tok_ms = 0.f, tok_stage_ms[TL_NSTAGE + 1] = {};
  std::vector<Event> ev_tok;
  std::vector<int> ev_tok_tag;
  TableSet tabs[MIND_TABLE_SETS];
  long long tab_clock = 0;
  long long n_table_hits = 0;
  unsigned dec_gen = 0;
  DevBuf pl_cnt;
  std::function<int(hipStream_t)> enc_pre, enc_post;
  std::vector<IlTables> il_tab;
  struct IlImage { std::vector<double> hD; std::vector<float> hF; std::vector<int> hI; } il_img;
  struct IlEarly { const double *xs = nullptr, *us = nullptr; volatile unsigned *done = nullptr; unsigned gen = 0; int n_trees = 0; long nodes = 0; } il_early;
  unsigned il_gen = 0;
  long long il_spec_req = 0, il_spec_hit = 0;
  DevBuf actor_lw_arena;
  std::vector<LwLaunch> actor_lw_plan;
  int last_actor_lw = 0, last_actor_launches = 0, last_actor_chunks = 0;
  float actor_ms = 0.f;
  Event ev_act0, ev_act1;
  int pair_prec = 3;
  std::vector<int> last_scene_n;
  bool last_edge_tiled = false, last_edge_bf16 = false;
  DevBuf edge, x, ST, QK, part, tokpos, meta, jobs, actor_feat, lane_feat, tgt_feat, cmode, tgt_emb,
      rows, rpe_ptrs;
  DevBuf ilqr_dev, aime_dev, rebase_dev2[2], dec_h2;
  DevBuf audit_dev;
  DevBuf pl_root, pl_in[2], pl_lf, pl_lrep, pl_pred, pl_small, pl_tab[2], pl_win[2];
  std::vector<DevBuf> pl_world;
  Pinned pl_pin[8];
  Event ev_pl, ev_tab, ev_root;
  DevBuf il_field;
  Pinned il_field_pin;
  Event ev_field;
  bool il_field_valid = false;
  double il_field_key[5] = {0, 0, 0, 0, 0};
  std::vector<double> il_field_lane;
  int xr = 0, xw = 1;
  mind_exchange_fn xfn = nullptr;
  void *xuser = nullptr;
  bool xforce = false;
  DevBuf x_send, x_recv, x_seg;
  long long x_collectives = 0, x_bytes = 0;
  Stream pl_copy;
  std::vector<double> pl_sol_xs, pl_sol_us;
  std::vector<mind_ilqr_stats> pl_sol_stw, pl_sol_stf;
  std::thread pa_thread;
  std::atomic<int> pa_state{0};
  mind_aime_plan_in pa_in;
  mind_aime_plan_out pa_out;
  int pa_rc = 0;
  struct Plan {
    AimeBook book;
    int agents = 0;
    long long gen = 0;
    const float *rows_p = nullptr, *fmean_p = nullptr, *fcov_p = nullptr;
    const float *dev_fmean = nullptr, *dev_fcov = nullptr;
  } plan;
  DevBuf pl_flat;
  DevBuf dec_xbuf, dec_bars;
  DevBuf dec_chain;
  Pinned dec_abort;
  int rb_cur = 0, rb_gen = 0;
  size_t rb_S = 0, rb_a = 0;
  bool profiling = false;
  Event ev_il0, ev_il1;
  float ilqr_ms = 0.f;
  int ilqr_multi = 0, ilqr_trees = 0;
  std::function<int()> il_finish;
  bool il_finish_owned = false;
  Event ev_rows;
  std::vector<const double *> il_trace_dev;
  std::vector<int> il_trace_its;
  int il_trace_cap = 0, il_trace_phases = 0;
  double il_prof[9] = {0, 0, 0, 0, 0, 0, 0, 0, 0};
  long long n_ilqr_fallbacks = 0;
  int n_pair_launch = 0;
  float pair_ms = 0.f;
  double pairs_done = 0.0;
  std::vector<Event> ev;
  bool ev_defer = false;
  std::vector<Event> ev_pool;
  size_t ev_pool_used = 0;
  std::vector<size_t> ev_pending;
  int wall_khz = 0;
  LcRing lc;
  DevBuf lc_dev;
  Pinned lc_host;
  double lc_carry_ms[LC_KINDS] = {0, 0, 0};
  int lc_carry_n[LC_KINDS] = {0, 0, 0};
  std::vector<float> lc_last[LC_KINDS], ev_last[LC_KINDS];
  int n_cu = 256;
  int debug_layers = 6;
  int last_ntok = 0;
  size_t il_dbg[6] = {0, 0, 0, 0, 0, 0};
  long long last_edge_pairs = 0;
  int last_slots = 0, last_A = 0, last_B = 0;
};

static int fail(mind_ctx *c, int code, const char *fmt, ...) {
  char buf[512];
  va_list ap;
  va_start(ap, fmt);
  vsnprintf(buf, sizeof(buf), fmt, ap);
  va_end(ap);
  if (c) c->err = buf;
  return code;
}

#define HIPCHK(c, call)                                                                        \
  do {                                                                                         \
    hipError_t e_ = (call);                                                                    \
    if (e_ != hipSuccess)                                                                      \
      return fail(c, MIND_EHIP, "%s failed: %s (%s:%d)", #call, hipGetErrorString(e_), __FILE__, __LINE__); \
  } while (0)

static int ensure(mind_ctx *c, DevBuf &b, size_t bytes) {
  if (bytes <= b.cap) return MIND_OK;
  b.reset();
  const size_t want = bytes < ((size_t)64 << 20) ? std::max<size_t>(2 * bytes, (size_t)1 << 20) : bytes + bytes / 4 + 4096;
  if (b.alloc(want) != hipSuccess) {
    const hipError_t e = b.alloc(bytes);
    if (e != hipSuccess) return fail(c, MIND_ENOMEM, "hipMalloc(%zu) failed: %s", bytes, hipGetErrorString(e));
  }
  return MIND_OK;
}

static int ensure_exact(mind_ctx *c, DevBuf &b, size_t bytes, const char *what) {
  if (bytes <= b.cap) return MIND_OK;
  HIPCHK(c, hipStreamSynchronize(c->stream));
  if (b.alloc(bytes) != hipSuccess) return fail(c, MIND_ENOMEM, "hipMalloc(%zu) for %s failed", bytes, what);
  return MIND_OK;
}

struct KernelLds {
  const void *kernel; size_t bytes;
  template <class K> KernelLds(K *k, size_t b) : kernel((const void *)k), bytes(b) {}
};
static void set_kernel_attributes() {
  const size_t pair = mind_pair_lds_bytes(), pair_bf = mind_pair_bf_lds_bytes(), actor_m = mind_actor_mfma_lds_bytes(), dec_m = mind_dec_actor_mfma_lds_bytes(),
               il = il_lds_bytes(0), tok_m = mind_token_mfma_lds_bytes(), dec_s = mind_dec_scene_lds_bytes(), dec_a = mind_dec_actor_lds_bytes();
  const KernelLds lds[] = {
      {k_pair<0>, pair}, {k_pair<1>, pair}, {k_pair_bf<0, 3>, pair_bf}, {k_pair_bf<1, 3>, pair_bf}, {k_pair_bf<0, 1>, pair_bf}, {k_pair_bf<1, 1>, pair_bf},
      {k_pair_t<0, 3>, pair_bf}, {k_pair_t<1, 3>, pair_bf}, {k_pair_t<0, 1>, pair_bf}, {k_pair_t<1, 1>, pair_bf}, {k_pair_t6<0>, pair_bf}, {k_pair_t6<1>, pair_bf},
      {k_actor_net, mind_actor_lds_bytes()}, {k_actor_mfma<3>, actor_m}, {k_actor_mfma<6>, actor_m}, {k_actor_mfma<1>, actor_m},
      {k_dec_actor_mfma<1>, dec_m}, {k_dec_actor_mfma<3>, dec_m}, {k_dec_actor_mfma<6>, dec_m}, {k_actor_f32<1>, mind_actor_f32_lds_bytes(1)}, {k_actor_f32<2>, mind_actor_f32_lds_bytes(2)},
      {k_ilqr<true, 0>, il}, {k_ilqr<false, 1>, il}, {k_ilqr<false, 0>, il}, {k_ilqr<false, 2>, il}, {k_token_mfma<0>, tok_m}, {k_token_mfma<1>, tok_m},
      {k_dec_scene, dec_s}, {k_dec_scene_mw, dec_s}, {k_dec_scene_c, dec_s}, {k_dec_cls, dec_s}, {k_dec_tgt, dec_s},
      {k_dec_chain1<8>, dec_s}, {k_dec_chain2<8>, dec_s}, {k_dec_chain3<8>, dec_s}, {k_dec_chain1<16>, dec_s}, {k_dec_chain2<16>, dec_s}, {k_dec_chain3<16>, dec_s},
      {k_dec_chain1<32>, dec_s}, {k_dec_chain2<32>, dec_s}, {k_dec_chain3<32>, dec_s}, {k_dec_chain4, dec_s},
      {k_dec_actor<0>, dec_a}, {k_dec_actor<1>, dec_a}, {k_dec_actor<2>, dec_a}, {k_dec_actor<2, 1>, dec_a}, {k_dec_actor<2, 2>, dec_a},
  };
  for (const KernelLds &k : lds) (void)hipFuncSetAttribute(k.kernel, hipFuncAttributeMaxDynamicSharedMemorySize, (int)k.bytes);
  lw_set_attributes();
}

static const char *const PAIR_PREC_NAMES[4] = {"f32", "bf16x3", "bf16", "bf16x6"};

extern "C" int mind_ctx_create(int device, void *stream, mind_ctx **out) {
  if (!out) return MIND_EINVAL;
  *out = nullptr;
  int n = 0;
  if (hipGetDeviceCount(&n) != hipSuccess || n <= 0) return MIND_EHIP;
  if (device < 0 || device >= n) return MIND_EINVAL;
  std::unique_ptr<mind_ctx> c(new mind_ctx());
  c->device = device;
  if (hipSetDevice(device) != hipSuccess) return MIND_EHIP;
  c->stream = (hipStream_t)stream;
  if (c->side.create() != hipSuccess || c->ev_side.create(hipEventDisableTiming) != hipSuccess || c->ev_main.create(hipEventDisableTiming) != hipSuccess ||
      c->ev_tgt.create(hipEventDisableTiming) != hipSuccess)
    c->side.reset();
  if (c->ev_stage.create(hipEventDisableTiming) != hipSuccess) return MIND_EHIP;
  hipDeviceProp_t prop;
  if (hipGetDeviceProperties(&prop, device) == hipSuccess) c->n_cu = prop.multiProcessorCount;
  if (hipDeviceGetAttribute(&c->wall_khz, hipDeviceAttributeWallClockRate, device) != hipSuccess || c->wall_khz < 0) c->wall_khz = 0;
  set_kernel_attributes();
  tn_apply_env(c->knobs(), [](const char *name) -> const char * { return getenv(name); });
  if (const char *pe = getenv("MIND_PAIR_PREC"))
    for (int m = 0; m < 4; ++m)
      if (!strcmp(pe, PAIR_PREC_NAMES[m]) || (pe[0] == '0' + m && !pe[1])) (void)mind_set_pair_precision(c.get(), m);
  *out = c.release();
  return MIND_OK;
}

extern "C" int mind_ctx_destroy(mind_ctx *c) {
  if (!c) return MIND_EINVAL;
  if (c->pa_thread.joinable()) c->pa_thread.join();
  (void)hipSetDevice(c->device);
  (void)hipStreamSynchronize(c->stream);
  if (c->side) (void)hipStreamSynchronize(c->side);
  if (c->pl_copy) (void)hipStreamSynchronize(c->pl_copy);
  c->il_finish = nullptr;
  delete c;
  return MIND_OK;
}

extern "C" const char *mind_last_error_string(mind_ctx *c) { return c ? c->err.c_str() : "null context"; }

extern "C" int mind_ctx_synchronize(mind_ctx *c) {
  if (!c) return MIND_EINVAL;
  HIPCHK(c, hipStreamSynchronize(c->stream));
  return MIND_OK;
}

extern "C" int mind_set_tuning(mind_ctx *c, const char *name, int value) {
  if (!c || !name) return MIND_EINVAL;
  if (!tn_set(c->knobs(), name, value)) return fail(c, MIND_EINVAL, "mind_set_tuning: unknown knob '%s'", name);
  return MIND_OK;
}

extern "C" int mind_get_tuning(mind_ctx *c, const char *name, int *value) {
  if (!c || !name || !value) return MIND_EINVAL;
  if (!tn_get(c->knobs(), name, value)) return fail(c, MIND_EINVAL, "mind_get_tuning: unknown knob '%s'", name);
  return MIND_OK;
}

extern "C" int mind_debug_tuning(int index, const char *name, const char *text, int value, const char **out_name, const char **out_env, int *out_value) {
  PredTuning pt; IlqrTuning it; CtxTuning ct;
  const TnRefs fresh{&pt, &it, &ct};
  const TnRow *row = name ? tn_find(name) : (index >= 0 && index < TN_ROWS) ? &TN_TABLE[index] : nullptr;
  if (!row || !out_value || (name && text && !row->env)) return MIND_EINVAL;
  if (name && text) tn_apply_env(fresh, [&](const char *var) { return strcmp(var, row->env) ? nullptr : text; });
  else if (name) (void)tn_set(fresh, name, value);
  if (out_name) *out_name = row->name;
  if (out_env) *out_env = row->env;
  (void)tn_get(fresh, row->name, out_value);
  return name ? MIND_OK : TN_ROWS;
}

extern "C" int mind_debug_live_handles(void) { return (int)live_handles.load(std::memory_order_relaxed); }

extern "C" int mind_set_exchange(mind_ctx *c, int rank, int world, mind_exchange_fn fn, void *user, int force) {
  if (!c) return MIND_EINVAL;
  if (fn && (world < 1 || rank < 0 || rank >= world)) return fail(c, MIND_EINVAL, "mind_set_exchange: rank %d of %d", rank, world);
  c->xfn = fn; c->xuser = user;
  c->xr = fn ? rank : 0; c->xw = fn ? world : 1; c->xforce = fn && force != 0;
  return MIND_OK;
}

extern "C" int mind_last_exchange_stats(mind_ctx *c, long long *collectives, long long *bytes) {
  if (!c) return MIND_EINVAL;
  if (collectives) *collectives = c->x_collectives;
  if (bytes) *bytes = c->x_bytes;
  return MIND_OK;
}

extern "C" int mind_set_pair_precision(mind_ctx *c, int mode) {
  if (!c || mode < 0 || mode > 3) return MIND_EINVAL;
  c->pair_prec = mode;
  return MIND_OK;
}

extern "C" int mind_get_pair_precision(mind_ctx *c) { return c ? c->pair_prec : MIND_EINVAL; }

extern "C" int mind_debug_pack_bfrag(const float *w, int row_stride, uint32_t *out) {
  if (!w || !out || row_stride < 128) return MIND_EINVAL;
  std::vector<float> v(w, w + (size_t)127 * row_stride + 128);
  v.resize((size_t)128 * row_stride, 0.f);
  const std::vector<float> t = pack_bfrag(v, row_stride);
  memcpy(out, t.data(), 16384 * sizeof(uint32_t));
  return MIND_OK;
}

static int lc_reserve(mind_ctx *c, int records, int grid);
extern "C" int mind_set_profiling(mind_ctx *c, int enable) {
  if (!c) return MIND_EINVAL;
  c->profiling = enable != 0;
  if (c->profiling && c->ct.prof_clock != 0 && c->wall_khz > 0 && c->lc.n_blocks == 0) {
    HIPCHK(c, hipSetDevice(c->device));
    return lc_reserve(c, 12, c->n_cu);
  }
  return MIND_OK;
}

extern "C" int mind_last_ilqr_stats(mind_ctx *c, float *kernel_ms, int *n_trees, int *workgroups_per_tree) {
  if (!c) return MIND_EINVAL;
  if (kernel_ms) *kernel_ms = c->ilqr_ms;
  if (n_trees) *n_trees = c->ilqr_trees;
  if (workgroups_per_tree) *workgroups_per_tree = c->ilqr_multi;
  return MIND_OK;
}

extern "C" int mind_last_ilqr_trace(mind_ctx *c, int tree, int phase, double *out, int cap_rows, int *n_rows) {
  if (!c || !n_rows || (cap_rows > 0 && !out)) return MIND_EINVAL;
  if (tree < 0 || tree >= (int)c->il_trace_dev.size() || phase < 0 || phase >= c->il_trace_phases || !c->il_trace_dev[tree])
    return fail(c, MIND_ESTATE, "mind_last_ilqr_trace: no trace for tree %d phase %d (the last tree-iLQR call had %d trees, %d phases)", tree, phase,
                (int)c->il_trace_dev.size(), c->il_trace_phases);
  const int rows = std::min(c->il_trace_its[2 * tree + phase], c->il_trace_cap);
  *n_rows = rows;
  const int take = std::min(rows, cap_rows);
  if (take > 0) {
    HIPCHK(c, hipMemcpyAsync(out, c->il_trace_dev[tree] + (size_t)phase * c->il_trace_cap * IL_TRACE_W, (size_t)take * IL_TRACE_W * sizeof(double),
                             hipMemcpyDeviceToHost, c->stream));
    HIPCHK(c, hipStreamSynchronize(c->stream));
  }
  return MIND_OK;
}

// ... 566 lines not shown
    bool saw_nan = false;
    int b_best = b_prev;
    auto price_block = [&](int b) {
      const int q0 = b * BS, q1 = std::min(S, q0 + BS);
      for (int q = q0; q < q1; ++q) {
        if (emin < INFINITY) {
          const double cxq = px - sx_[q], cyq = py - sy_[q], lim = rmin + sr_[q];
          if (cxq * cxq + cyq * cyq > lim * lim) continue;
        }
        const double sx = (double)lane[2 * q], sy = (double)lane[2 * q + 1], ddx = (double)dx[q], ddy = (double)dy[q];
        double t = ((px - sx) * ddx + (py - sy) * ddy) / (double)l2[q];
        t = t < 0.0 ? 0.0 : (t > 1.0 ? 1.0 : t);
        const double ex = px - (sx + t * ddx), ey = py - (sy + t * ddy);
        const double e = ex * ex + ey * ey;
        if (e < emin) { emin = e; rmin = sqrt(e) * (1.0 + 1e-9) + 1e-9; b_best = b; }
        else if (e != e) saw_nan = true;
      }
    };
    price_block(b_prev);
    for (int b = 0; b < NB; ++b) {
      if (b == b_prev) continue;
      if (emin < INFINITY) {
        const double cxb = px - bx[b], cyb = py - by[b], lim = rmin + br[b];
        if (cxb * cxb + cyb * cyb > lim * lim) continue;
      }
      price_block(b);
    }
    b_prev = b_best;
    const double dmin = saw_nan ? (double)NAN : sqrt(emin);
    const double c0 = ct[2 * i], c1 = ct[2 * i + 1], dv = tv - st[6 * i + 2];
    per_node[i] = ((0.1 * (c0 * c0) + 5.0 * (c1 * c1)) + 0.01 * (dv * dv)) + 0.01 * dmin;
  }
}
}

extern "C" int mind_fill_tracks(const double *raw , int a, int T, const int32_t *slot ,
                                float *pos , float *ang , float *vel , int16_t *typ ,
                                int16_t *have ) {
  if (!raw || !slot || !pos || !ang || !vel || !typ || !have || a < 0 || T <= 0) return MIND_EINVAL;
  for (int i = 0; i < a; ++i) {
    const double *r = raw + (size_t)i * T * 6;
    int first = 0;
    for (int t = 0; t < T; ++t)
      if (r[t * 6] != 0.0) { first = t; break; }
    int src = -1;
    for (int t = 0; t < T; ++t) {
      const bool h = r[t * 6] != 0.0;
      if (h) src = t;
      const int f = src < 0 ? first : src;
      const bool hf = r[f * 6] != 0.0;
      const size_t o = (size_t)i * T + t;
      pos[2 * o] = hf ? (float)r[f * 6 + 1] : 0.f;
      pos[2 * o + 1] = hf ? (float)r[f * 6 + 2] : 0.f;
      ang[o] = hf ? (float)r[f * 6 + 3] : 0.f;
      vel[2 * o] = h ? (float)r[t * 6 + 4] : 0.f;
      vel[2 * o + 1] = h ? (float)r[t * 6 + 5] : 0.f;
      have[o] = h ? 1 : 0;
      for (int k = 0; k < 7; ++k) typ[o * 7 + k] = (h && k == slot[i]) ? 1 : 0;
    }
  }
  return MIND_OK;
}

extern "C" int mind_eval_traj_trees(const double *states, const double *ctrls, const int32_t *counts, int n_trees, const void *lane,
                                    int lane_is_f32, int n_lane_pts, double target_vel, double *out) {
  if (!states || !ctrls || !counts || n_trees <= 0 || !lane || n_lane_pts < 2 || !out) return MIND_EINVAL;
  long N = 0;
  for (int t = 0; t < n_trees; ++t) { if (counts[t] <= 0) return MIND_EINVAL; N += counts[t]; }
  std::vector<double> per(N);
  auto run = [&](long lo, long hi) {
    if (lane_is_f32) eval_nodes<float>(states + 6 * lo, ctrls + 2 * lo, hi - lo, (const float *)lane, n_lane_pts, target_vel, per.data() + lo);
    else eval_nodes<double>(states + 6 * lo, ctrls + 2 * lo, hi - lo, (const double *)lane, n_lane_pts, target_vel, per.data() + lo);
  };
  const long nth = std::min<long>(std::min<long>(8, (long)std::max(1u, std::thread::hardware_concurrency())), N / 8192);
  if (nth <= 1) run(0, N);
  else {
    std::vector<std::thread> th;
    for (long k = 0; k < nth; ++k) th.emplace_back(run, N * k / nth, N * (k + 1) / nth);
    for (std::thread &t : th) t.join();
  }
  long o = 0;
  for (int t = 0; t < n_trees; ++t) {
    const long n = counts[t];
    out[t] = (n > 1 ? per[o] + np_pairwise(per.data() + o + 1, n - 1) : per[o]) / (double)n;
    o += n;
  }
  return MIND_OK;
}

__global__ void k_debug_trig(const double *__restrict__ x, int n, double *__restrict__ out) {
  const int i = blockIdx.x * blockDim.x + threadIdx.x;
  const double v = i < n ? x[i] : 0.0;
  double s, c, t, c2;
  mind_sincos(v, &s, &c);
  mind_tan_cos(v, &t, &c2);
  if (i < n) { out[4 * i] = s; out[4 * i + 1] = c; out[4 * i + 2] = t; out[4 * i + 3] = c2; }
}
extern "C" int mind_debug_trig(mind_ctx *c, const double *x, int n, double *out) {
  if (!c || !x || !out || n <= 0) return MIND_EINVAL;
  HIPCHK(c, hipSetDevice(c->device));
  double *d = nullptr;
  HIPCHK(c, hipMalloc((void **)&d, (size_t)n * 5 * sizeof(double)));
  hipError_t e = hipMemcpy(d, x, (size_t)n * sizeof(double), hipMemcpyHostToDevice);
  if (e == hipSuccess) {
    hipLaunchKernelGGL(k_debug_trig, dim3((n + 63) / 64), dim3(64), 0, c->stream, d, n, d + n);
    e = hipStreamSynchronize(c->stream);
  }
  if (e == hipSuccess) e = hipMemcpy(out, d + n, (size_t)n * 4 * sizeof(double), hipMemcpyDeviceToHost);
  (void)hipFree(d);
  if (e != hipSuccess) return fail(c, MIND_EHIP, "mind_debug_trig: %s", hipGetErrorString(e));
  return MIND_OK;
}

extern "C" int mind_debug_dec_scene(mind_ctx *c, const float *rows, int n_scenes, int form, float *Cout, float *cls, int reps, float *ms) {
  if (!c || !rows || !Cout || !cls || n_scenes <= 0 || n_scenes > 4096 || !(form == 0 || dc_valid_g(form)) || reps < 1 || reps > 1024) return MIND_EINVAL;
  if (!c->have_weights) return fail(c, MIND_ESTATE, "weights not loaded");
  HIPCHK(c, hipSetDevice(c->device));
  const int B = n_scenes;
  const size_t nx = (size_t)B * 128, nc = (size_t)B * 768, nk = (size_t)B * 6;
  DevBuf d;
  if (d.alloc((nx + nc + nk) * sizeof(float) + (size_t)B * sizeof(int)) != hipSuccess) return fail(c, MIND_ENOMEM, "mind_debug_dec_scene: hipMalloc failed");
  float *dx = d.as<float>(), *dC = dx + nx, *dk = dC + nc;
  int *drow = (int *)(dk + nk);
  std::vector<int> row(B);
  for (int b = 0; b < B; ++b) row[b] = b;
  HIPCHK(c, hipMemcpy(dx, rows, nx * sizeof(float), hipMemcpyHostToDevice));
  HIPCHK(c, hipMemcpy(drow, row.data(), (size_t)B * sizeof(int), hipMemcpyHostToDevice));
  Event e0, e1;
  if (ms && (e0.create() != hipSuccess || e1.create() != hipSuccess)) return fail(c, MIND_EHIP, "mind_debug_dec_scene: no events");
  for (int it = 0; it < reps; ++it) {
    if (ms) HIPCHK(c, hipEventRecord(e0, c->stream));
    if (form == 0)
      hipLaunchKernelGGL(k_dec_scene, dim3(B), dim3(DT), mind_dec_scene_lds_bytes(), c->stream, (const float *)dx, (const int *)drow, dC, dk, c->W.dec);
    else if (int rc = dec_chain_run(c, form, B, dx, drow, dC, dk, c->stream))
      return rc;
    if (ms) {
      HIPCHK(c, hipEventRecord(e1, c->stream));
      HIPCHK(c, hipEventSynchronize(e1));
      HIPCHK(c, hipEventElapsedTime(&ms[it], e0, e1));
    }
  }
  HIPCHK(c, hipGetLastError());
  HIPCHK(c, hipStreamSynchronize(c->stream));
  HIPCHK(c, hipMemcpy(Cout, dC, nc * sizeof(float), hipMemcpyDeviceToHost));
  HIPCHK(c, hipMemcpy(cls, dk, nk * sizeof(float), hipMemcpyDeviceToHost));
  return MIND_OK;
}

extern "C" int mind_debug_set_layers(mind_ctx *c, int n) {
  if (!c || n < 0 || n > 6) return MIND_EINVAL;
  c->debug_layers = n;
  return MIND_OK;
}
extern "C" int64_t mind_debug_read(mind_ctx *c, const char *name, float *host, int64_t max_floats) {
  if (!c || !name) return MIND_EINVAL;
  const void *src = nullptr;
  int64_t n = 0;
  std::string k = name;
  if (k == "x") { src = c->x.p; n = (int64_t)c->last_ntok * 128; }
  else if (k == "ST") { src = c->ST.p; n = (int64_t)c->last_ntok * 256; }
  else if (k == "QK") { src = c->QK.p; n = (int64_t)c->last_ntok * 1024; }
  else if (k == "edge") { src = c->edge.p; n = c->last_edge_pairs * 128; }
  else if (k == "part") { src = c->part.p; n = (int64_t)c->last_slots * PART_STRIDE; }
  else if (k == "actor_feat") { src = c->actor_feat.p; n = (int64_t)c->last_A * 128; }
  else if (k == "tokpos") { src = c->tokpos.p; n = (int64_t)c->last_ntok * 4; }
  else if (k == "cmode") { src = c->cmode.p; n = (int64_t)c->last_B * 768; }
  else if (k == "tgt_emb") { src = c->tgt_emb.p; n = (int64_t)c->last_B * 128; }
  else if (k == "tgt_feat") { src = c->tgt_feat.p; n = (int64_t)c->last_B * 128; }
  else if (k == "pl_root") { src = c->pl_root.p; n = (int64_t)(c->pl_root.cap / sizeof(float)); }
  else if (k == "il_spec") {
    if (!host) return 2;
    if (max_floats < 2) return MIND_EINVAL;
    host[0] = (float)c->il_spec_req; host[1] = (float)c->il_spec_hit;
    return 2;
  }
  else if (k.rfind("il_", 0) == 0 && c->il_dbg[5]) {
    const size_t M = c->il_dbg[5];
    int w = -1; size_t per = 0;
    if (k == "il_L") { w = 0; per = 1; } else if (k == "il_Lx") { w = 1; per = 6; } else if (k == "il_Lxx") { w = 2; per = 36; }
    else if (k == "il_Fx") { w = 3; per = 36; } else if (k == "il_xs") { w = 4; per = 6; }
    if (w < 0) return MIND_EINVAL;
    src = (const char *)c->ilqr_dev.p + c->il_dbg[w];
    n = (int64_t)(M * per * 2);
  }
  else return MIND_EINVAL;
  if (!host) return n;
  if (n > max_floats) n = max_floats;
  if (hipStreamSynchronize(c->stream) != hipSuccess) return MIND_EHIP;
  if (k == "edge" && c->last_edge_tiled) {
    long long pt = 0;
    for (int N : c->last_scene_n) pt += (long long)N * (((N + 15) / 16) * 16);
    const bool eb = c->last_edge_bf16;
    std::vector<float> raw((size_t)pt * (eb ? 64 : 128));
    if (hipMemcpy(raw.data(), src, raw.size() * sizeof(float), hipMemcpyDeviceToHost) != hipSuccess) return MIND_EHIP;
    int64_t o = 0;
    size_t sb = 0;
    for (int N : c->last_scene_n) {
      const int rows = ((N + 15) / 16) * 16;
      for (int j = 0; j < N; ++j)
        for (int i = 0; i < N; ++i)
          for (int f = 0; f < 128 && o < n; ++f, ++o) {
            const int t = i >> 4, pp = i & 15, b = f >> 4, qq = (f >> 2) & 3, r = f & 3;
            const size_t tile0 = sb + (size_t)j * rows + (size_t)t * 16;
            if (!eb) host[o] = raw[tile0 * 128 + ((b * 64 + qq * 16 + pp) * 4 + r)];
            else {
              uint32_t w;
              memcpy(&w, &raw[tile0 * 64 + (((b >> 1) * 64 + qq * 16 + pp) * 4 + 2 * (b & 1) + (r >> 1))], 4);
              w = (r & 1) ? (w & 0xffff0000u) : (w << 16);
              memcpy(&host[o], &w, 4);
            }
          }
      sb += (size_t)N * rows;
    }
    return n;
  }
  if (hipMemcpy(host, src, (size_t)n * sizeof(float), hipMemcpyDeviceToHost) != hipSuccess) return MIND_EHIP;
  return n;
}

#include "loop.hip"

#include "audit_host.hip"

#include "forecast_host.hip"

#include "road_host.hip"

#include "ttc_host.hip"
```

### mind_amd/csrc/predict.hip

```cpp
__global__ void k_tokpos(const TokMeta *__restrict__ meta, int n_tok, const float *__restrict__ actr,
                         const float *__restrict__ avec, const float *__restrict__ lctr,
                         const float *__restrict__ lvec, float *__restrict__ tokpos) {
  const int t = blockIdx.x * blockDim.x + threadIdx.x;
  if (t >= n_tok) return;
  const TokMeta m = meta[t];
  float4 o = make_float4(0.f, 0.f, 0.f, 0.f);
  if (m.type == 0 && actr) o = make_float4(actr[m.src * 2], actr[m.src * 2 + 1], avec[m.src * 2], avec[m.src * 2 + 1]);
  if (m.type == 1 && lctr) o = make_float4(lctr[m.src * 2], lctr[m.src * 2 + 1], lvec[m.src * 2], lvec[m.src * 2 + 1]);
  ((float4 *)tokpos)[t] = o;
}

struct PairTables {
  std::vector<TokMeta> meta;
  std::vector<PairJob> jobs, jobs5;
  std::vector<int> actor_row, actor_scene, cls_row, scene_n;
  long long edge_pairs = 0, edge_pairs_t = 0;
  int ntok = 0, slot = 0;
  double pairs_full = 0, pairs_l5 = 0;
};

static void pair_tables_build(int Bn, const int *scene_actors, const int *scene_lanes, bool xcd_order, int n_cu, PairTables &T) {
  int A = 0;
  for (int b = 0; b < Bn; ++b) A += scene_actors[b];
  T.actor_row.assign(A, 0); T.actor_scene.assign(A, 0); T.cls_row.assign(Bn, 0); T.scene_n.assign(Bn, 0);
// ... 147 lines not shown

static int lc_copy_async(mind_ctx *c, hipStream_t s, int i0, int n) {
  int first[2], count[2];
  const int runs = c->lc.pending_runs(i0, n, first, count);
  for (int k = 0; k < runs; ++k) {
    const size_t o = c->lc.slot_of(first[k]), b = (size_t)count[k] * c->lc.block_slots * sizeof(LcSlot);
    HIPCHK(c, hipMemcpyAsync(c->lc_host.as<LcSlot>() + o, (const LcSlot *)c->lc_dev.p + o, b, hipMemcpyDeviceToHost, s));
  }
  if (runs > 0) c->lc.mark_copied(i0, n);
  return MIND_OK;
}

static int lc_resolve(mind_ctx *c, int n, unsigned kinds, double (&ms)[LC_KINDS], int (&cnt)[LC_KINDS]) {
  for (int k = 0; k < LC_KINDS; ++k) {
    ms[k] = 0.0; cnt[k] = 0;
    if (kinds >> k & 1u) c->lc_last[k].clear();
  }
  if (n < 0 || n > (int)c->lc.pending.size()) n = (int)c->lc.pending.size();
  if (!c->lc.copied(n)) {
    int rc;
    if ((rc = lc_flush(c, true))) return rc;
  } else {
    for (int i = 0; i < n; ++i) lc_account(c, c->lc.pending[i], c->lc_carry_ms, c->lc_carry_n);
    c->lc.drained(n);
  }
  for (int k = 0; k < LC_KINDS; ++k)
    if (kinds >> k & 1u) { ms[k] = c->lc_carry_ms[k]; cnt[k] = c->lc_carry_n[k]; c->lc_carry_ms[k] = 0.0; c->lc_carry_n[k] = 0; }
  return MIND_OK;
}

struct PredCall {
  mind_ctx *c;
  const mind_scene_batch *in;
  mind_pred_out *out;
  const mind_pred_aux *aux;
  const PredChoice &ch;
  int Bn, A, Ltot;
  hipStream_t st, ss;
  TableSet *ts = nullptr;
  const float *lane_feat = nullptr;
  const float *const *rpe_dev = nullptr;
  Event *evs = nullptr;
  bool tok_timed = false;
  bool act_ev = false, pair_ev = false;
  bool pair_clk = false;
  size_t ev_tok_used = 0;
  float *x() const { return (float *)c->x.p; }
  const int *rows() const { return (const int *)ts->rows.p; }
};

static int pred_tables(PredCall &p, const int *scene_actors, const int *scene_lanes) {
  mind_ctx *c = p.c;
  const int Bn = p.Bn, A = p.A;
  std::vector<int> key;
  key.reserve(2 * Bn + 3);
  key.push_back(Bn);
  for (int b = 0; b <= Bn; ++b) key.push_back(p.in->actor_off[b]);
  for (int b = 0; b <= Bn; ++b) key.push_back(p.in->lane_off[b]);
  TableSet *ts = nullptr;
  for (TableSet &t : c->tabs)
    if (t.key == key) ts = &t;
  const bool tab_hit = ts != nullptr;
  if (!ts) {
    ts = &c->tabs[0];
    for (TableSet &t : c->tabs)
      if (t.stamp < ts->stamp) ts = &t;
  }
  ts->stamp = ++c->tab_clock;
  p.ts = ts;
  if (tab_hit) {
    c->n_table_hits++;
    return MIND_OK;
  }
  PairTables T;
  pair_tables_build(Bn, scene_actors, scene_lanes, c->pt.xcd_order, c->n_cu, T);
  int rc;
  ts->key.clear();
  if ((rc = ensure(c, ts->meta, T.meta.size() * sizeof(TokMeta)))) return rc;
  if ((rc = ensure(c, ts->jobs, T.jobs.size() * sizeof(PairJob)))) return rc;
  if ((rc = ensure(c, ts->jobs5, T.jobs5.size() * sizeof(PairJob)))) return rc;
  if ((rc = ensure(c, ts->rows, (size_t)(2 * A + Bn) * sizeof(int)))) return rc;
  HIPCHK(c, hipMemcpyAsync(ts->meta.p, T.meta.data(), T.meta.size() * sizeof(TokMeta), hipMemcpyHostToDevice, p.st));
  HIPCHK(c, hipMemcpyAsync(ts->jobs.p, T.jobs.data(), T.jobs.size() * sizeof(PairJob), hipMemcpyHostToDevice, p.st));
  HIPCHK(c, hipMemcpyAsync(ts->jobs5.p, T.jobs5.data(), T.jobs5.size() * sizeof(PairJob), hipMemcpyHostToDevice, p.st));
  std::vector<int> rows(2 * A + Bn);
  memcpy(rows.data(), T.actor_row.data(), A * sizeof(int));
  memcpy(rows.data() + A, T.actor_scene.data(), A * sizeof(int));
  memcpy(rows.data() + 2 * A, T.cls_row.data(), Bn * sizeof(int));
  HIPCHK(c, hipMemcpyAsync(ts->rows.p, rows.data(), rows.size() * sizeof(int), hipMemcpyHostToDevice, p.st));
  HIPCHK(c, hipStreamSynchronize(p.st));
  ts->actor_row.swap(T.actor_row);
  ts->cls_row.swap(T.cls_row);
  ts->scene_n.swap(T.scene_n);
  ts->edge_pairs = T.edge_pairs; ts->edge_pairs_t = T.edge_pairs_t; ts->ntok = T.ntok; ts->slot = T.slot; ts->njobs = (int)T.jobs.size();
  ts->njobs5 = (int)T.jobs5.size();
  ts->pairs_full = T.pairs_full; ts->pairs_l5 = T.pairs_l5;
  ts->key.swap(key);
  return MIND_OK;
}

static int pred_workspaces(PredCall &p) {
  mind_ctx *c = p.c;
  const TableSet *ts = p.ts;
  const int ntok = ts->ntok, Bn = p.Bn;
  int rc;
  if ((rc = ensure(c, c->edge, (size_t)(p.ch.tiled ? ts->edge_pairs_t : ts->edge_pairs) * 128 * sizeof(float)))) return rc;
  if ((rc = ensure(c, c->x, (size_t)ntok * 128 * sizeof(float)))) return rc;
  if ((rc = ensure(c, c->ST, (size_t)ntok * 256 * sizeof(float)))) return rc;
  if ((rc = ensure(c, c->QK, (size_t)(ntok + 1) * p.ch.qk_stride * sizeof(float)))) return rc;
  if ((rc = ensure(c, c->part, (size_t)ts->slot * PART_STRIDE * sizeof(float)))) return rc;
  if ((rc = ensure(c, c->tokpos, (size_t)ntok * 4 * sizeof(float)))) return rc;
  if ((rc = ensure(c, c->actor_feat, (size_t)p.A * 128 * sizeof(float)))) return rc;
  if ((rc = ensure(c, c->lane_feat, (size_t)(p.Ltot > 0 ? p.Ltot : 1) * 128 * sizeof(float)))) return rc;
  if ((rc = ensure(c, c->tgt_feat, (size_t)Bn * 128 * sizeof(float)))) return rc;
  if ((rc = ensure(c, c->cmode, (size_t)Bn * 768 * sizeof(float)))) return rc;
  if ((rc = ensure(c, c->tgt_emb, (size_t)Bn * 128 * sizeof(float)))) return rc;
  if (p.in->rpe) {
    if ((rc = ensure(c, c->rpe_ptrs, (size_t)Bn * sizeof(float *)))) return rc;
    HIPCHK(c, hipMemcpyAsync(c->rpe_ptrs.p, p.in->rpe, (size_t)Bn * sizeof(float *), hipMemcpyHostToDevice, p.st));
    HIPCHK(c, hipStreamSynchronize(p.st));
    p.rpe_dev = (const float *const *)c->rpe_ptrs.p;
  }
  return MIND_OK;
}

static int pred_actor_net(PredCall &p, LcSlot *clk) {
  mind_ctx *c = p.c;
  const PredChoice &ch = p.ch;
  const float *actors = p.in->actors;
  float *actor_feat = (float *)c->actor_feat.p;
  const int A = p.A;
  const dim3 grid(ch.actor_grid);
  switch (ch.actor_form) {
  case PRED_ACTOR_F32:
    if (ch.actor_arg == 2) hipLaunchKernelGGL(k_actor_f32<2>, grid, dim3(AF_T), mind_actor_f32_lds_bytes(2), p.st, actors, A, actor_feat, c->W.actorF, clk);
    else hipLaunchKernelGGL(k_actor_f32<1>, grid, dim3(AF_T), mind_actor_f32_lds_bytes(1), p.st, actors, A, actor_feat, c->W.actorF, clk);
    break;
  case PRED_ACTOR_VALU:
    hipLaunchKernelGGL(k_actor_net, grid, dim3(AT), mind_actor_lds_bytes(), p.st, actors, A, actor_feat, c->W.actor, clk);
    break;
  case PRED_ACTOR_LW: {
    int rc;
    if ((rc = ensure_exact(c, c->actor_lw_arena, lw_arena_bytes(ch.actor_chunk), "the layer-wise ActorNet's arena"))) return rc;
    lw_build_plan(A, ch.actor_chunk, c->actor_lw_plan);
    u32 *arena = (u32 *)c->actor_lw_arena.p;
    const int nl = ch.np == 6 ? lw_run<6>(c->actor_lw_plan, p.st, arena, actors, actor_feat, c->W.actorB)
                 : ch.np == 3 ? lw_run<3>(c->actor_lw_plan, p.st, arena, actors, actor_feat, c->W.actorB)
                              : lw_run<1>(c->actor_lw_plan, p.st, arena, actors, actor_feat, c->W.actorB);
    if (nl < 0) return fail(c, MIND_ESTATE, "layer-wise ActorNet: a stage has no kernel");
    c->last_actor_lw = 1; c->last_actor_launches = nl; c->last_actor_chunks = ch.actor_chunks;
    break;
  }
  default:
    if (ch.np == 6) hipLaunchKernelGGL(k_actor_mfma<6>, grid, dim3(AM_T), mind_actor_mfma_lds_bytes(), p.st, actors, A, actor_feat, c->W.actorB, clk);
    else if (ch.np == 3) hipLaunchKernelGGL(k_actor_mfma<3>, grid, dim3(AM_T), mind_actor_mfma_lds_bytes(), p.st, actors, A, actor_feat, c->W.actorB, clk);
    else hipLaunchKernelGGL(k_actor_mfma<1>, grid, dim3(AM_T), mind_actor_mfma_lds_bytes(), p.st, actors, A, actor_feat, c->W.actorB, clk);
  }
  return MIND_OK;
}

static int pred_encoders(PredCall &p) {
  mind_ctx *c = p.c;
  const mind_scene_batch *in = p.in;
  hipStream_t st = p.st, ss = p.ss;
  const int Bn = p.Bn, Ltot = p.Ltot, ntok = p.ts->ntok;
  if (c->side) {
    HIPCHK(c, hipEventRecord(c->ev_main, st));
    HIPCHK(c, hipStreamWaitEvent(c->side, c->ev_main, 0));
  }
  const bool act_timed = c->profiling && !c->ev_defer;
  int rc;
  LcSlot *act_clk = nullptr;
  if (act_timed && lc_on(c) && p.ch.actor_form != PRED_ACTOR_LW) {
    if ((rc = lc_reserve(c, 1, p.ch.actor_grid))) return rc;
    act_clk = lc_take(c, p.ch.actor_grid, LC_ACTOR);
  }
  p.act_ev = act_timed && (lc_events(c) || !act_clk);
  if (p.act_ev && !c->ev_act0) {
    HIPCHK(c, c->ev_act0.create());
    HIPCHK(c, c->ev_act1.create());
  }
  c->last_actor_lw = 0; c->last_actor_launches = 1; c->last_actor_chunks = 1; c->actor_ms = 0.f;
  if (p.act_ev) HIPCHK(c, hipEventRecord(c->ev_act0, st));
  if ((rc = pred_actor_net(p, act_clk))) return rc;
  if (p.act_ev) HIPCHK(c, hipEventRecord(c->ev_act1, st));
  if (c->enc_pre) {
    const std::function<int(hipStream_t)> pre = std::move(c->enc_pre);
    c->enc_pre = nullptr;
    if ((rc = pre(ss))) return rc;
  }
  p.lane_feat = in->lane_feat;
  if (!p.lane_feat) {
    float *lf = p.out->lane_feat ? p.out->lane_feat : (float *)c->lane_feat.p;
    if (Ltot > 0)
      hipLaunchKernelGGL(k_lane_net, dim3((Ltot + PL - 1) / PL), dim3(DT), 0, ss, in->lanes, Ltot, lf, c->W.lane);
    p.lane_feat = lf;
  } else if (p.out->lane_feat && p.out->lane_feat != in->lane_feat && Ltot > 0) {
    HIPCHK(c, hipMemcpyAsync(p.out->lane_feat, in->lane_feat, (size_t)Ltot * 128 * sizeof(float), hipMemcpyDeviceToDevice, ss));
  }
  hipLaunchKernelGGL(k_tokpos, dim3((ntok + 255) / 256), dim3(256), 0, ss, (const TokMeta *)p.ts->meta.p, ntok, in->actor_ctrs, in->actor_vecs,
                     in->lane_ctrs, in->lane_vecs, (float *)c->tokpos.p);
  if (c->side) {
    HIPCHK(c, hipEventRecord(c->ev_side, c->side));
    HIPCHK(c, hipStreamWaitEvent(st, c->ev_side, 0));
  }
  hipLaunchKernelGGL(k_lane_net, dim3((Bn + PL - 1) / PL), dim3(DT), 0, ss, in->tgt_nodes, Bn, (float *)c->tgt_feat.p, c->W.lane);
  hipLaunchKernelGGL(k_dec_tgt, dim3(Bn), dim3(DT), mind_dec_scene_lds_bytes(), ss, (const float *)c->tgt_feat.p, in->tgt_rpe, (float *)c->tgt_emb.p,
                     c->W.dec);
  if (c->enc_post) {
    const std::function<int(hipStream_t)> post = std::move(c->enc_post);
    c->enc_post = nullptr;
    if ((rc = post(ss))) return rc;
  }
  if (c->side) HIPCHK(c, hipEventRecord(c->ev_tgt, c->side));
  if (p.ch.tgt_wait_first) HIPCHK(c, hipStreamWaitEvent(st, c->ev_tgt, 0));
  return MIND_OK;
}

static hipError_t ev_grow(std::vector<Event> &v, size_t n) {
  hipError_t rc = hipSuccess;
  for (Event e; v.size() < n && (rc = e.create()) == hipSuccess;) v.push_back(std::move(e));
  return rc;
}

static hipError_t pred_tok_mark(PredCall &p, int tag) {
  mind_ctx *c = p.c;
  if (!p.tok_timed) return hipSuccess;
  if (p.ev_tok_used == c->ev_tok.size()) {
    const hipError_t rc_ = ev_grow(c->ev_tok, p.ev_tok_used + 1);
    if (rc_ != hipSuccess) return rc_;
    c->ev_tok_tag.push_back(0);
  }
  c->ev_tok_tag[p.ev_tok_used] = tag;
  return hipEventRecord(c->ev_tok[p.ev_tok_used++], p.st);
}

static int pred_token_step(PredCall &p, int mode, int Lw) {
  mind_ctx *c = p.c;
  hipStream_t st = p.st;
  const size_t qk_stride = p.ch.qk_stride, tokm_lds = mind_token_mfma_lds_bytes();
  const float *actor_feat = (const float *)c->actor_feat.p, *lane_feat = p.lane_feat;
  float *part = (float *)c->part.p;
  HIPCHK(c, pred_tok_mark(p, -1));
  for (const PredTokRun &r : p.ch.tok_runs) {
    const TokMeta *m_ = (const TokMeta *)p.ts->meta.p + r.t0;
    float *x_ = p.x() + (size_t)r.t0 * 128, *ST_ = (float *)c->ST.p + (size_t)r.t0 * 256, *QK_ = (float *)c->QK.p + (size_t)r.t0 * qk_stride;
    if (r.layerwise) {
      tl_build_plan(r.n, mode, p.ch.tok_chunk, c->n_cu, c->tok_lw_plan);
      for (const TlLaunch &L : c->tok_lw_plan) {
        if (tl_launch(L, st, mode, m_, actor_feat, lane_feat, x_, part, ST_, QK_, qk_stride, c->W.tok[Lw], c->W.tokM[Lw], (float *)c->tok_lw_arena.p, p.ch.tok_chunk))
          return fail(c, MIND_ESTATE, "layer-wise token stage: a stage has no kernel");
        HIPCHK(c, pred_tok_mark(p, L.stage));
      }
      c->last_tok_launches += (int)c->tok_lw_plan.size();
      continue;
    }
    c->last_tok_launches++;
    if (r.kind == 0) {
      const int tpw = r.small ? TOK_TPW_SMALL : TOK_TPW_BIG;
      hipLaunchKernelGGL(r.small ? (r.merged ? k_token_m : k_token<TOK_TPW_SMALL>) : k_token<TOK_TPW_BIG>, dim3((r.n + tpw - 1) / tpw), dim3(TT_THREADS), 0,
                         st, m_, r.n, mode, actor_feat, lane_feat, x_, part, ST_, QK_, c->W.tok[Lw]);
    } else if (r.kind == 1) {
      hipLaunchKernelGGL(k_token_mfma<0>, dim3((r.n + TM_TOK - 1) / TM_TOK), dim3(TM_THREADS), tokm_lds, st, m_, r.n, mode, actor_feat, lane_feat, x_,
                         part, ST_, QK_, c->W.tok[Lw], c->W.tokM[Lw]);
    } else {
      hipLaunchKernelGGL(k_token_mfma<1>, dim3((r.n + TM_TOK - 1) / TM_TOK), dim3(TM_THREADS), tokm_lds, st, m_, r.n, mode, actor_feat, lane_feat, x_,
                         part, ST_, QK_, c->W.tok[Lw], c->W.tokB[Lw]);
    }
    HIPCHK(c, pred_tok_mark(p, TL_NSTAGE));
  }
  return MIND_OK;
}

static int pred_pair_layer(PredCall &p, int L) {
  mind_ctx *c = p.c;
  const PredChoice &ch = p.ch;
  const TableSet *ts = p.ts;
  const bool last = L == 5, own5 = last && ch.l5_jobs5;
  const int um = L < 4 ? 0 : (L == 4 ? 1 : 2);
  const PairJob *jl = (const PairJob *)(own5 ? ts->jobs5.p : ts->jobs.p);
  const int nj = own5 ? ts->njobs5 : ts->njobs;
  const dim3 grid(pair_grid(nj, c->n_cu)), block(PAIR_THREADS);
  float *edge = (float *)c->edge.p, *ST = (float *)c->ST.p, *QK = (float *)c->QK.p, *part = (float *)c->part.p, *tokpos = (float *)c->tokpos.p;
  const size_t ldsb = mind_pair_bf_lds_bytes();
  const u32 *we = c->W.pair.WBe[L], *wp = last ? c->W.pair.WBe[L] : c->W.pair.WBp[L];
  LcSlot *clk = p.pair_clk ? lc_take(c, (int)grid.x, LC_PAIR) : nullptr;
  if (p.pair_ev) HIPCHK(c, hipEventRecord(p.evs[2 * L], p.st));
#define PAIR_GO(K0, K1, LDS, ...)                                                                                                             \
  do {                                                                                                                                        \
    if (L == 0) hipLaunchKernelGGL(K0, grid, block, LDS, p.st, jl, nj, edge, ST, QK, part, __VA_ARGS__, c->W.pair.vtab[L], c->W.pair.rtab, tokpos, p.rpe_dev, um, clk); \
    else hipLaunchKernelGGL(K1, grid, block, LDS, p.st, jl, nj, edge, ST, QK, part, __VA_ARGS__, c->W.pair.vtab[L], c->W.pair.rtab, tokpos, p.rpe_dev, um, clk);   \
  } while (0)
  switch (ch.pair_family) {
  case PRED_PAIR_F32: PAIR_GO((k_pair<0>), (k_pair<1>), mind_pair_lds_bytes(), c->W.pair.WAe[L], last ? c->W.pair.WAe[L] : c->W.pair.WAp[L]); break;
  case PRED_PAIR_T6: PAIR_GO((k_pair_t6<0>), (k_pair_t6<1>), ldsb, we, wp, c->W.pair.WLe[L], last ? c->W.pair.WLe[L] : c->W.pair.WLp[L]); break;
  case PRED_PAIR_T:
    if (ch.pair_np == 3) PAIR_GO((k_pair_t<0, 3>), (k_pair_t<1, 3>), ldsb, we, wp);
    else PAIR_GO((k_pair_t<0, 1>), (k_pair_t<1, 1>), ldsb, we, wp);
    break;
  default:
    if (ch.pair_np == 3) PAIR_GO((k_pair_bf<0, 3>), (k_pair_bf<1, 3>), ldsb, we, wp);
    else PAIR_GO((k_pair_bf<0, 1>), (k_pair_bf<1, 1>), ldsb, we, wp);
  }
#undef PAIR_GO
  if (p.pair_ev) HIPCHK(c, hipEventRecord(p.evs[2 * L + 1], p.st));
  c->n_pair_launch++;
  c->pairs_done += last ? ts->pairs_l5 : ts->pairs_full;
  return MIND_OK;
}

static int pred_fusion(PredCall &p) {
  mind_ctx *c = p.c;
  const PredChoice &ch = p.ch;
  const TableSet *ts = p.ts;
  int rc;
  c->last_tok_lw = ch.tok_lw; c->last_tok_launches = 0; c->last_tok_chunks = ch.last_tok_chunks; c->tok_ms = 0.f;
  for (float &v : c->tok_stage_ms) v = 0.f;
  if (ch.tok_lw && (rc = ensure_exact(c, c->tok_lw_arena, tl_arena_bytes(ch.tok_chunk), "the layer-wise token stage's arena"))) return rc;
  p.tok_timed = c->profiling && !c->ev_defer;
  if ((rc = pred_token_step(p, 1 | 4 | ch.qsplit, 0))) return rc;
  c->n_pair_launch = 0;
  c->pairs_done = 0;
  p.pair_clk = lc_on(c);
  p.pair_ev = lc_events(c);
  if (p.pair_clk && (rc = lc_reserve(c, c->debug_layers, std::max(pair_grid(ts->njobs, c->n_cu), pair_grid(ts->njobs5, c->n_cu))))) return rc;
  if (p.pair_ev) HIPCHK(c, ev_grow(c->ev, 12));
  p.evs = c->ev.data();
  if (p.pair_ev && c->ev_defer) {
    HIPCHK(c, ev_grow(c->ev_pool, c->ev_pool_used + 12));
    p.evs = c->ev_pool.data() + c->ev_pool_used;
    c->ev_pending.push_back(c->ev_pool_used);
    c->ev_pool_used += 12;
  }
  c->last_ntok = ts->ntok; c->last_edge_pairs = ts->edge_pairs; c->last_slots = ts->slot; c->last_A = p.A; c->last_B = p.Bn;
  c->last_scene_n = ts->scene_n; c->last_edge_tiled = ch.tiled; c->last_edge_bf16 = ch.edge_bf16;
  for (int L = 0; L < c->debug_layers; ++L) {
    if ((rc = pred_pair_layer(p, L))) return rc;
    if ((rc = pred_token_step(p, 2 | (L < 5 ? 4 : 8) | ch.qsplit, L + 1))) return rc;
  }
  return MIND_OK;
}

static int dec_chain_run(mind_ctx *c, int G, int Bn, const float *x, const int *d_cls_row, float *Cout, float *cls, hipStream_t st) {
  if (!dc_valid_g(G) || Bn <= 0) return fail(c, MIND_EINVAL, "decoder chain: %d workgroups per scene, %d scenes", G, Bn);
  int rc;
  if ((rc = ensure(c, c->dec_chain, (size_t)std::max(Bn, c->n_cu / 8) * DC_SCENE_FLOATS * sizeof(float)))) return rc;
  float *buf = (float *)c->dec_chain.p;
  const size_t lds = mind_dec_scene_lds_bytes();
#define DEC_CHAIN(GV)                                                                                                  \
  do {                                                                                                                 \
    hipLaunchKernelGGL(k_dec_chain1<GV>, dim3(Bn * GV), dim3(DT), lds, st, x, d_cls_row, buf, c->W.dec);                \
    hipLaunchKernelGGL(k_dec_chain2<GV>, dim3(Bn * GV), dim3(DT), lds, st, buf, c->W.dec);                              \
    hipLaunchKernelGGL(k_dec_chain3<GV>, dim3(Bn * GV), dim3(DT), lds, st, buf, c->W.dec);                              \
  } while (0)
  if (G == 32) DEC_CHAIN(32);
  else if (G == 16) DEC_CHAIN(16);
  else DEC_CHAIN(8);
#undef DEC_CHAIN
  hipLaunchKernelGGL(k_dec_chain4, dim3(Bn), dim3(DT), lds, st, (const float *)buf, Cout, cls, c->W.dec);
// ... 160 lines not shown
```

### mind_amd/predictor.py

```python
import ctypes as C

import numpy as np
import torch

from . import _lib


AIME_NODE_DTYPE = np.dtype({"names": ["round", "scene", "mode", "parent", "prob", "cur_t", "end_t", "flags", "dur", "row_off", "tgt_pts"],
                            "formats": ["<i4", "<i4", "<i4", "<i4", "<f4", "<i4", "<i4", "<i4", "<i4", "<i8", ("<f4", (22,))],
                            "offsets": [0, 4, 8, 12, 16, 20, 24, 28, 32, 40, 48], "itemsize": 136})


class IlqrCall:

    def __init__(self, lib, cfg, flats, x0, lane, target_vel, cfg_full=None, use_exo=1, us_init=None, background=False):
        self.lib, self.cfg, self.cfg_full, self.use_exo = lib, cfg, cfg_full, int(use_exo)
        self.background = bool(background)
        n = self.n = len(flats)
        self.trees = (_lib.CostTree * n)()
        self.keep, self.Ms = [], []
        for i, f in enumerate(flats):
            par = np.ascontiguousarray(f["parent"], np.int32)
            prob = np.ascontiguousarray(f["prob"], np.float32)
            mean = np.ascontiguousarray(f["mean"], np.float32)
# ... 97 lines not shown
        self.ctx, self._rt, self._begun, self.rc = rt.ctx, rt, True, 0

    def begin(self, rt):
        return self

    def wait(self):
        if getattr(self, "_begun", False):
            self._begun = False
            rt = self._rt
            if rt.ctx is None or rt.ctx.value != self.ctx.value:
                self.rc = _lib.MIND_ESTATE
            else:
                self.rc = self.lib.mind_ilqr_finish_plan(self.ctx, int(sum(self.Ms)), self.n, self.xs.ctypes.data, self.us.ctypes.data,
                                                         C.cast(self.st, C.c_void_p), C.cast(self.st_full, C.c_void_p))
        return self


class HipPredictor:

    def __init__(self, device=0):
        self.lib = _lib.load()
        if not torch.cuda.is_available():
            raise RuntimeError("HipPredictor needs a GPU (no CPU fallback)")
        self.device = torch.device("cuda", device if isinstance(device, int) else (device.index or 0))
        torch.cuda.set_device(self.device)
        self.ctx = C.c_void_p()
        stream = torch.cuda.current_stream(self.device).cuda_stream
        self.on_default_stream = int(stream or 0) == 0
        rc = self.lib.mind_ctx_create(self.device.index, C.c_void_p(stream), C.byref(self.ctx))
        _lib.check(self.lib, None, rc, "mind_ctx_create")
        self._keep = []

    def close(self):
        if getattr(self, "ctx", None):
            self.lib.mind_ctx_destroy(self.ctx)
            self.ctx = None

    def __del__(self):
        try:
            self.close()
        except Exception:
            pass

    def load_state_dict(self, sd, param_out=None):
        if param_out is not None:
            self.set_decoder_basis(param_out)
        descs, keep = _lib.tensor_descs(sd)
        rc = self.lib.mind_weights_load(self.ctx, descs, len(sd))
        _lib.check(self.lib, self.ctx, rc, "mind_weights_load")

    PAIR_PREC = ("f32", "bf16x3", "bf16", "bf16x6")

    def pair_precision(self):
        return self.PAIR_PREC[self.lib.mind_get_pair_precision(self.ctx)]

    def set_tuning(self, name, value):
        _lib.check(self.lib, self.ctx, self.lib.mind_set_tuning(self.ctx, name.encode(), int(value)), "mind_set_tuning")
        if name == "ilqr_wgs":
            self._ilqr_wgs_saved = None

    def get_tuning(self, name):
        v = C.c_int()
        _lib.check(self.lib, self.ctx, self.lib.mind_get_tuning(self.ctx, name.encode(), C.byref(v)), "mind_get_tuning")
        return v.value

    _ilqr_wgs_saved = None

    def ilqr_background(self, on):
        if on and self._ilqr_wgs_saved is None:
            self._ilqr_wgs_saved = self.get_tuning("ilqr_wgs")
            self.lib.mind_set_tuning(self.ctx, b"ilqr_wgs", 1)
        elif not on and self._ilqr_wgs_saved is not None:
            self.lib.mind_set_tuning(self.ctx, b"ilqr_wgs", self._ilqr_wgs_saved)
            self._ilqr_wgs_saved = None

    def set_pair_precision(self, name):
        _lib.check(self.lib, self.ctx, self.lib.mind_set_pair_precision(self.ctx, self.PAIR_PREC.index(name)), "mind_set_pair_precision")

    def set_decoder_basis(self, name):
        if name not in _lib.BASIS:
            raise ValueError(f"unknown decoder basis {name!r}: one of {_lib.BASIS}")
        _lib.check(self.lib, self.ctx, self.lib.mind_set_decoder_basis(self.ctx, _lib.BASIS.index(name)), "mind_set_decoder_basis")

    def get_decoder_basis(self):
        return _lib.BASIS[self.lib.mind_get_decoder_basis(self.ctx)]

    def curve_eval(self, param, tau, basis=None, want=("reg", "vel", "cov_vel")):
        assert param.device == self.device and param.dtype == torch.float32 and tuple(param.shape[-2:]) == (8, 5), (param.device, param.dtype, param.shape)
        if basis is not None and basis not in _lib.BASIS:
            raise ValueError(f"unknown decoder basis {basis!r}: one of {_lib.BASIS}")
        widths = {"reg": 5, "vel": 2, "cov_vel": 3}
        if any(k not in widths for k in want):
            raise ValueError(f"curve_eval: want names {tuple(want)!r}, of {tuple(widths)}")
        param = param.contiguous()
        tau = np.ascontiguousarray(tau, np.float64).ravel()
        lead, n = tuple(param.shape[:-2]), param.numel() // 40
        out = {k: torch.empty(lead + (tau.size, w), device=self.device) for k, w in widths.items() if k in want}
        ptr = lambda k: C.c_void_p(out[k].data_ptr()) if k in out and out[k].numel() > 0 else None
        rc = self.lib.mind_curve_eval(self.ctx, -1 if basis is None else _lib.BASIS.index(basis), C.c_void_p(param.data_ptr()) if n else None, n,
                                      tau.ctypes.data_as(C.POINTER(C.c_double)), tau.size, ptr("reg"), ptr("vel"), ptr("cov_vel"))
        _lib.check(self.lib, self.ctx, rc, "mind_curve_eval")
        return out

    def set_profiling(self, on):
        self.lib.mind_set_profiling(self.ctx, 1 if on else 0)

    def ilqr_stats(self):
        ms, n, g = C.c_float(), C.c_int(), C.c_int()
        self.lib.mind_last_ilqr_stats(self.ctx, C.byref(ms), C.byref(n), C.byref(g))
        return ms.value, n.value, g.value

    def ilqr_profile(self):
        v = (C.c_double * 9)()
        self.lib.mind_last_ilqr_profile(self.ctx, v)
        keys = ("nodes", "depth", "passes", "derivatives", "backward", "state_chain", "cost_pass", "selection", "trees")
        return dict(zip(keys, [float(x) for x in v]))

    def ilqr_trace(self, tree, phase=0):
        n = C.c_int()
        buf = np.zeros((256, 4), np.float64)
        _lib.check(self.lib, self.ctx, self.lib.mind_last_ilqr_trace(self.ctx, int(tree), int(phase), buf.ctypes.data_as(C.POINTER(C.c_double)), 256,
                                                                    C.byref(n)), "mind_last_ilqr_trace")
        return buf[:min(n.value, 256)].copy()

    def fusion_stats(self):
        n = C.c_int()
        ms = C.c_float()
        pairs = C.c_double()
        self.lib.mind_last_fusion_stats(self.ctx, C.byref(n), C.byref(ms), C.byref(pairs))
        return n.value, ms.value, pairs.value

    def launch_times(self, kind="pair"):
        cap = 4096
        ck, ev = (C.c_float * cap)(), (C.c_float * cap)()
        nc, ne = C.c_int(), C.c_int()
        _lib.check(self.lib, self.ctx, self.lib.mind_debug_launch_times(self.ctx, {"pair": 0, "actor": 1}[kind], ck, ev, cap, C.byref(nc), C.byref(ne)),
                   "mind_debug_launch_times")
        return [float(v) for v in ck[:min(nc.value, cap)]], [float(v) for v in ev[:min(ne.value, cap)]]

    def last_actor_stats(self):
        lw, n, ch, ms = C.c_int(), C.c_int(), C.c_int(), C.c_float()
        _lib.check(self.lib, self.ctx, self.lib.mind_last_actor_stats(self.ctx, C.byref(lw), C.byref(n), C.byref(ch), C.byref(ms)), "mind_last_actor_stats")
        return dict(layerwise=lw.value, launches=n.value, chunks=ch.value, ms=ms.value)

    def last_token_stats(self):
        lw, n, ch, ms = C.c_int(), C.c_int(), C.c_int(), C.c_float()
        _lib.check(self.lib, self.ctx, self.lib.mind_last_token_stats(self.ctx, C.byref(lw), C.byref(n), C.byref(ch), C.byref(ms)), "mind_last_token_stats")
        st = (C.c_float * 8)()
        self.lib.mind_last_token_stage_ms(self.ctx, st, 8)
        return dict(layerwise=lw.value, launches=n.value, chunks=ch.value, ms=ms.value, stage_ms=[float(v) for v in st])

    def debug_set_layers(self, n):
        _lib.check(self.lib, self.ctx, self.lib.mind_debug_set_layers(self.ctx, n), "mind_debug_set_layers")

    def debug_read(self, name):
        n = self.lib.mind_debug_read(self.ctx, name.encode(), None, 0)
        if n < 0:
            raise _lib.MindError(f"mind_debug_read({name}) -> {n}")
        buf = np.empty(n, np.float32)
        got = self.lib.mind_debug_read(self.ctx, name.encode(), buf.ctypes.data_as(C.POINTER(C.c_float)), n)
        assert got == n, (got, n)
        return buf

    def synchronize(self):
        _lib.check(self.lib, self.ctx, self.lib.mind_ctx_synchronize(self.ctx), "mind_ctx_synchronize")

    def predict(self, actors, actor_off, lanes, lane_off, actor_ctrs, actor_vecs, lane_ctrs, lane_vecs,
                tgt_nodes, tgt_rpe, rpe=None, lane_feat=None, want_lane_feat=False, taps=False, aux=False):
        dev = self.device
        B = len(actor_off) - 1
        A, L = int(actor_off[-1]), int(lane_off[-1])

        def f32(t):
            if t is None:
                return None
            assert t.device == dev and t.dtype == torch.float32, (t.device, t.dtype)
            return t.contiguous()

        actors, lanes, lane_feat = f32(actors), f32(lanes), f32(lane_feat)
        actor_ctrs, actor_vecs, lane_ctrs, lane_vecs = f32(actor_ctrs), f32(actor_vecs), f32(lane_ctrs), f32(lane_vecs)
        tgt_nodes, tgt_rpe = f32(tgt_nodes), f32(tgt_rpe)
        assert actors.shape == (A, 14, 48) and tgt_nodes.shape == (B, 10, 16) and tgt_rpe.shape == (B, 20)
        ao = (C.c_int32 * (B + 1))(*[int(v) for v in actor_off])
        lo = (C.c_int32 * (B + 1))(*[int(v) for v in lane_off])
        sb = _lib.SceneBatch()
        sb.n_scenes = B
        sb.actor_off, sb.lane_off = ao, lo

        def ptr(t):
            return C.c_void_p(t.data_ptr()) if t is not None and t.numel() > 0 else None

        sb.actors, sb.lanes, sb.lane_feat = ptr(actors), ptr(lanes), ptr(lane_feat)
        sb.actor_ctrs, sb.actor_vecs, sb.lane_ctrs, sb.lane_vecs = ptr(actor_ctrs), ptr(actor_vecs), ptr(lane_ctrs), ptr(lane_vecs)
        rpe_keep = None
        if rpe is not None:
            rpe_keep = [f32(r) for r in rpe]
            arr = (C.c_void_p * B)(*[r.data_ptr() for r in rpe_keep])
            sb.rpe = arr
        sb.tgt_nodes, sb.tgt_rpe = ptr(tgt_nodes), ptr(tgt_rpe)
        out = {"cls": torch.empty(B, 6, device=dev), "reg": torch.empty(A, 6, 60, 5, device=dev),
               "vel": torch.empty(A, 6, 60, 2, device=dev)}
        po = _lib.PredOut()
        po.cls, po.reg, po.vel = ptr(out["cls"]), ptr(out["reg"]), ptr(out["vel"])
        if want_lane_feat and lane_feat is None and L > 0:
            out["lane_feat"] = torch.empty(L, 128, device=dev)
            po.lane_feat = ptr(out["lane_feat"])
        if taps:
            out["actor_emb"] = torch.empty(A, 128, device=dev)
            out["cls_emb"] = torch.empty(B, 128, device=dev)
            po.actor_emb, po.cls_emb = ptr(out["actor_emb"]), ptr(out["cls_emb"])
        if aux:
            out["cov_vel"] = torch.empty(A, 6, 60, 3, device=dev)
            out["param"] = torch.empty(A, 6, 8, 5, device=dev)
            pa = _lib.PredAux(ptr(out["cov_vel"]), ptr(out["param"]))
            rc = self.lib.mind_predict_batch_aux(self.ctx, C.byref(sb), C.byref(po), C.byref(pa))
        else:
            rc = self.lib.mind_predict_batch(self.ctx, C.byref(sb), C.byref(po))
        _lib.check(self.lib, self.ctx, rc, "mind_predict_batch")
        return out

    def ilqr_contingency(self, cfg_warm, cfg_full, flats, x0, lane, target_vel):
        call = IlqrCall(self.lib, cfg_warm, flats, x0, lane, target_vel, cfg_full=cfg_full)
        call.run(self)
        return call.finish()

    def ilqr_solve(self, cfg, flats, x0, lane, target_vel, use_exo, us_init=None):
        call = IlqrCall(self.lib, cfg, flats, x0, lane, target_vel, use_exo=use_exo, us_init=us_init)
        call.run(self)
        return call.finish()

    @staticmethod
    def _generic_tree(tree, keep):
        ct = _lib.CostTree()
        par = np.ascontiguousarray(tree["parent"], np.int32)
        fld = np.ascontiguousarray(tree["field"], np.float64)
        nw = np.ascontiguousarray(tree["node_w"], np.float64)
        if fld.ndim != 3 or fld.shape[0] != len(par) or nw.shape != (len(par), 32):
            raise ValueError("generic cost tree: field [M,H,W] / node_w [M,32] do not match parent [M]")
        keep += [par, fld, nw]
        ct.n_nodes, ct.n_agents = len(par), 0
        ct.parent = par.ctypes.data_as(C.POINTER(C.c_int32))
        ct.field = fld.ctypes.data_as(C.POINTER(C.c_double))
        ct.node_w = nw.ctypes.data_as(C.POINTER(C.c_double))
        return ct

    @staticmethod
    def _grid(grid, keep):
        g = _lib.FieldGrid()
        gx = np.ascontiguousarray(grid["gx"], np.float64)
        gy = np.ascontiguousarray(grid["gy"], np.float64)
        keep += [gx, gy]
        g.W, g.H, g.res = len(gx), len(gy), float(grid["res"])
        g.off_x, g.off_y = float(grid["offset"][0]), float(grid["offset"][1])
        g.gx = gx.ctypes.data_as(C.POINTER(C.c_double))
        g.gy = gy.ctypes.data_as(C.POINTER(C.c_double))
        return g

    def ilqr_solve_fields(self, cfg, grid, tree, x0, us_init=None):
        keep = []
        ct = self._generic_tree(tree, keep)
        g = self._grid(grid, keep)
        M = ct.n_nodes
        x0 = np.ascontiguousarray(x0, np.float64)
        xs, us = np.zeros((M, 6)), np.zeros((M, 2))
        st = _lib.IlqrStats()
        ui = None if us_init is None else np.ascontiguousarray(us_init, np.float64)
        dp = lambda a: a.ctypes.data_as(C.POINTER(C.c_double)) if a is not None else None
        rc = self.lib.mind_ilqr_solve_fields(self.ctx, C.byref(cfg), C.byref(g), C.byref(ct), 1, dp(x0), dp(ui), dp(xs), dp(us),
                                             C.byref(st))
        _lib.check(self.lib, self.ctx, rc, "mind_ilqr_solve_fields")
        return xs, us, dict(iterations=st.iterations, converged=st.converged, J=st.J, mu=st.mu)

    def cost_eval(self, cfg, node, x, u, tree, grid=None, x0=None, lane=None, target_vel=0.0, use_exo=0):
        keep = []
        if grid is not None:
            ct = self._generic_tree(tree, keep)
            g = C.byref(self._grid(grid, keep))
            x0 = np.zeros(6) if x0 is None else x0
        else:
            ct = _lib.CostTree()
            par = np.ascontiguousarray(tree["parent"], np.int32)
            prob = np.ascontiguousarray(tree["prob"], np.float32)
            mean = np.ascontiguousarray(tree["mean"], np.float32)
            cov = np.ascontiguousarray(tree["cov"], np.float32)
            keep += [par, prob, mean, cov]
            ct.n_nodes, ct.n_agents = len(par), mean.shape[1]
            ct.parent = par.ctypes.data_as(C.POINTER(C.c_int32))
            ct.prob = prob.ctypes.data_as(C.POINTER(C.c_float))
            ct.agent_mean = mean.ctypes.data_as(C.POINTER(C.c_float))
            ct.agent_cov = cov.ctypes.data_as(C.POINTER(C.c_float))
            g = None
        node = np.ascontiguousarray(node, np.int32)
        x = np.ascontiguousarray(x, np.float64).reshape(len(node), 6)
        u = np.ascontiguousarray(u, np.float64).reshape(len(node), 2)
        x0 = np.ascontiguousarray(x0, np.float64)
        lane_a = None if lane is None else np.ascontiguousarray(lane, np.float64)
        out = np.zeros((len(node), 47))
        dp = lambda a: a.ctypes.data_as(C.POINTER(C.c_double)) if a is not None else None
        rc = self.lib.mind_cost_eval(self.ctx, C.byref(cfg), g, C.byref(ct), dp(x0), dp(lane_a), 0 if lane_a is None else len(lane_a),
                                     C.c_double(float(target_vel)), int(use_exo), len(node),
                                     node.ctypes.data_as(C.POINTER(C.c_int32)), dp(x), dp(u), dp(out))
        _lib.check(self.lib, self.ctx, rc, "mind_cost_eval")
        luu = np.zeros((len(node), 2, 2))
        luu[:, 0, 0], luu[:, 1, 1] = out[:, 45], out[:, 46]
        return dict(l=out[:, 0].copy(), l_x=out[:, 1:7].copy(), l_u=out[:, 7:9].copy(), l_xx=out[:, 9:45].reshape(-1, 6, 6).copy(), l_uu=luu)

# ... 496 lines not shown
```

Before: 1929.

## Fuse paired GroupNorm reductions in actor encoder and add DPP wave sum

In the actor MFMA kernel, the main conv and downsample conv of each residual block now run back to back, and their GroupNorm statistics are reduced together, so one pair of block barriers serves both. The lateral FPN layers are handled the same way in pairs. A permlane/DPP register-based wave reduction replaces the shuffle-based one. The lane net can also run one item per block when the count fits the CU count. The goal is fewer __syncthreads and cheaper cross-lane reductions, at the cost of holding two accumulator sets in registers, which raises register pressure.

```diff
diff --git a/include/mind_hip.h b/include/mind_hip.h
--- a/include/mind_hip.h
+++ b/include/mind_hip.h
@@ -129,6 +129,8 @@
 int mind_debug_dec_scene(mind_ctx *ctx, const float *rows, int n_scenes, int form, float *Cout, float *cls, int reps, float *ms);
 
 int mind_debug_set_layers(mind_ctx *ctx, int n);
+int mind_debug_encoder_forms(mind_ctx *ctx, int actor_form, int lane_form, int wave_sum_form);
+int mind_debug_wave_sum(mind_ctx *ctx, const float *in, int n_waves, float *out_shuffle, float *out_register);
 int64_t mind_debug_read(mind_ctx *ctx, const char *name, float *host, int64_t max_floats);
 
 typedef struct {
diff --git a/mind_amd/_lib.py b/mind_amd/_lib.py
--- a/mind_amd/_lib.py
+++ b/mind_amd/_lib.py
@@ -223,7 +223,7 @@
 
 EXPORTS = ["mind_ctx_create", "mind_ctx_destroy", "mind_last_error_string", "mind_ctx_synchronize",
            "mind_weights_load", "mind_predict_batch", "mind_last_fusion_stats", "mind_last_actor_stats", "mind_debug_actor_lw_plan", "mind_last_token_stats", "mind_last_token_stage_ms", "mind_debug_token_lw_plan", "mind_set_profiling", "mind_debug_launch_times", "mind_debug_launch_clock",
-           "mind_ilqr_solve_trees", "mind_ilqr_contingency", "mind_ilqr_solve_fields", "mind_cost_eval", "mind_ilqr_score_trees", "mind_ilqr_gains", "mind_ilqr_policy_rollouts", "mind_lane_dist_field", "mind_aime_world", "mind_aime_rebase", "mind_debug_aime_decide", "mind_debug_set_layers",
+           "mind_ilqr_solve_trees", "mind_ilqr_contingency", "mind_ilqr_solve_fields", "mind_cost_eval", "mind_ilqr_score_trees", "mind_ilqr_gains", "mind_ilqr_policy_rollouts", "mind_lane_dist_field", "mind_aime_world", "mind_aime_rebase", "mind_debug_aime_decide", "mind_debug_set_layers", "mind_debug_encoder_forms", "mind_debug_wave_sum",
            "mind_debug_read", "mind_set_pair_precision", "mind_get_pair_precision", "mind_debug_pack_bfrag", "mind_debug_pack_conv_frag", "mind_debug_pack", "mind_debug_weight_image", "mind_debug_weight_bind", "mind_debug_pair_schedule", "mind_debug_predict_choice", "mind_debug_ilqr_plan", "mind_debug_aime_book", "mind_set_tuning", "mind_get_tuning", "mind_debug_tuning", "mind_debug_live_handles", "mind_last_ilqr_stats", "mind_aime_plan", "mind_last_ilqr_profile", "mind_eval_traj_trees", "mind_last_ilqr_trace", "mind_ilqr_contingency_begin", "mind_ilqr_finish", "mind_fill_tracks", "mind_ilqr_contingency_begin_plan", "mind_debug_trig", "mind_aime_plan_begin", "mind_aime_plan_poll", "mind_aime_plan_finish", "mind_ctx_busy", "mind_ilqr_finish_plan", "mind_debug_dec_scene",
            "mind_set_exchange", "mind_last_exchange_stats", "mind_debug_wait_word",
            "mind_predict_batch_aux", "mind_set_decoder_basis", "mind_get_decoder_basis", "mind_curve_eval", "mind_debug_curve_basis",
@@ -341,6 +341,8 @@
     lib.mind_debug_weight_bind.argtypes = [C.POINTER(TensorDesc), C.c_int, C.c_char_p, C.c_char_p, C.c_int]
     lib.mind_debug_dec_scene.argtypes = [C.c_void_p, C.POINTER(C.c_float), C.c_int, C.c_int, C.POINTER(C.c_float), C.POINTER(C.c_float), C.c_int, C.POINTER(C.c_float)]
     lib.mind_debug_set_layers.argtypes = [C.c_void_p, C.c_int]
+    lib.mind_debug_encoder_forms.argtypes = [C.c_void_p, C.c_int, C.c_int, C.c_int]
+    lib.mind_debug_wave_sum.argtypes = [C.c_void_p, C.POINTER(C.c_float), C.c_int, C.POINTER(C.c_float), C.POINTER(C.c_float)]
     lib.mind_debug_read.argtypes = [C.c_void_p, C.c_char_p, C.POINTER(C.c_float), C.c_int64]
     lib.mind_set_exchange.argtypes = [C.c_void_p, C.c_int, C.c_int, EXCHANGE_FN, C.c_void_p, C.c_int]
     lib.mind_last_exchange_stats.argtypes = [C.c_void_p, C.POINTER(C.c_longlong), C.POINTER(C.c_longlong)]
diff --git a/mind_amd/csrc/actor_mfma_kernels.hip b/mind_amd/csrc/actor_mfma_kernels.hip
--- a/mind_amd/csrc/actor_mfma_kernels.hip
+++ b/mind_amd/csrc/actor_mfma_kernels.hip
@@ -21,18 +21,10 @@
 
 #include "weight_tables.h"
 #include "launch_clock.h"
+#include "wave_sum.h"
 typedef u32 u32x2 __attribute__((ext_vector_type(2)));
 
-__device__ __forceinline__ float am_block_sum(float v, float *red, int flip) {
-  v = wave_sum(v);
-  float *r = red + (flip & 1) * 32;
-  if ((threadIdx.x & 63) == 0) r[threadIdx.x >> 6] = v;
-  __syncthreads();
-  float s = 0.f;
-#pragma unroll
-  for (int w = 0; w < AM_WAVES; ++w) s += r[w];
-  return s;
-}
+__device__ __forceinline__ float *am_red_row(float *red, int j, int flip) { return red + (flip & 1) * 32 + (j & 1) * 16; }
 
 template <int NP>
 __device__ __forceinline__ void am_store_split(u32 *rowp, int plane, const f32x4 &y) {
@@ -106,40 +98,89 @@
   }
 }
 
+template <int WS, int N>
+__device__ __forceinline__ void am_gn_stats(const f32x4 (&acc)[N][AM_MAXT], const int (&Cout)[N], const int (&Tout)[N], float *red,
+                                            float (&mean)[N], float (&rstd)[N]) {
+  const int lane = threadIdx.x & 63, wave = threadIdx.x >> 6;
+  const int r = lane & 15;
+#pragma unroll
+  for (int j = 0; j < N; ++j) {
+    const int ntt = (Tout[j] + 15) >> 4;
+    const int tiles = (Cout[j] >> 4) * ntt;
+    float s = 0.f;
+#pragma unroll
+    for (int i = 0; i < AM_MAXT; ++i) {
+      const int ti = wave + AM_WAVES * i;
+      if (ti >= tiles) continue;
+      const int nt = ti % ntt;
+      if (nt * 16 + r < Tout[j]) s += (acc[j][i][0] + acc[j][i][1]) + (acc[j][i][2] + acc[j][i][3]);
+    }
+    s = wave_sum_as<WS>(s);
+    if (lane == 0) am_red_row(red, j, 0)[wave] = s;
+  }
+  __syncthreads();
+#pragma unroll
+  for (int j = 0; j < N; ++j) {
+    const float *rr = am_red_row(red, j, 0);
+    float s = 0.f;
+#pragma unroll
+    for (int w = 0; w < AM_WAVES; ++w) s += rr[w];
+    mean[j] = s / (float)(Cout[j] * Tout[j]);
+  }
+#pragma unroll
+  for (int j = 0; j < N; ++j) {
+    const int ntt = (Tout[j] + 15) >> 4;
+    const int tiles = (Cout[j] >> 4) * ntt;
+    float v = 0.f;
+#pragma unroll
+    for (int i = 0; i < AM_MAXT; ++i) {
+      const int ti = wave + AM_WAVES * i;
+      if (ti >= tiles) continue;
+      const int nt = ti % ntt;
+      if (nt * 16 + r < Tout[j]) {
+#pragma unroll
+        for (int e = 0; e < 4; ++e) { const float d = acc[j][i][e] - mean[j]; v = fmaf(d, d, v); }
+      }
+    }
+    v = wave_sum_as<WS>(v);
+    if (lane == 0) am_red_row(red, j, 1)[wave] = v;
+  }
+  __syncthreads();
+#pragma unroll
+  for (int j = 0; j < N; ++j) {
+    const float *rr = am_red_row(red, j, 1);
+    float s = 0.f;
+#pragma unroll
+    for (int w = 0; w < AM_WAVES; ++w) s += rr[w];
+    rstd[j] = 1.0f / sqrtf(s / (float)(Cout[j] * Tout[j]) + 1e-5f);
+  }
+}
+
+__device__ __forceinline__ void am_gn_affine(int Cout, int Tout, const float *__restrict__ g, const float *__restrict__ b,
+                                             f32x4 (&gg)[AM_MAXT], f32x4 (&bb)[AM_MAXT]) {
+  const int lane = threadIdx.x & 63, wave = threadIdx.x >> 6;
+  const int q = lane >> 4;
+  const int ntt = (Tout + 15) >> 4;
+  const int tiles = (Cout >> 4) * ntt;
+#pragma unroll
+  for (int i = 0; i < AM_MAXT; ++i) {
+    const int ti = wave + AM_WAVES * i;
+    if (ti >= tiles) continue;
+    const int mt = ti / ntt;
+    gg[i] = *(const f32x4 *)(g + mt * 16 + q * 4);
+    bb[i] = *(const f32x4 *)(b + mt * 16 + q * 4);
+  }
+}
+
 template <int NP>
-__device__ __forceinline__ void am_gn(f32x4 (&acc)[AM_MAXT], int Cout, int Tout, const float *__restrict__ g,
-                                      const float *__restrict__ b, const u32 *resid, const float *up, bool relu, u32 *outs,
-                                      float *outf, float *__restrict__ gout, float *red) {
+__device__ __forceinline__ void am_gn_apply(const f32x4 (&acc)[AM_MAXT], int Cout, int Tout, float mean, float rstd,
+                                            const f32x4 (&gg)[AM_MAXT], const f32x4 (&bb)[AM_MAXT], const u32 *resid, const float *up,
+                                            bool relu, u32 *outs, float *outf, float *__restrict__ gout) {
   const int lane = threadIdx.x & 63, wave = threadIdx.x >> 6;
   const int r = lane & 15, q = lane >> 4;
   const int ntt = (Tout + 15) >> 4;
   const int tiles = (Cout >> 4) * ntt;
   const int RSD = AM_RSD(Cout), PLANE = Cout >> 1;
-  f32x4 gg[AM_MAXT], bb[AM_MAXT];
-  float s = 0.f;
-#pragma unroll
-  for (int i = 0; i < AM_MAXT; ++i) {
-    const int ti = wave + AM_WAVES * i;
-    if (ti >= tiles) continue;
-    const int mt = ti / ntt, nt = ti - mt * ntt;
-    gg[i] = *(const f32x4 *)(g + mt * 16 + q * 4);
-    bb[i] = *(const f32x4 *)(b + mt * 16 + q * 4);
-    if (nt * 16 + r < Tout) s += (acc[i][0] + acc[i][1]) + (acc[i][2] + acc[i][3]);
-  }
-  const float n = (float)(Cout * Tout);
-  const float mean = am_block_sum(s, red, 0) / n;
-  float v = 0.f;
-#pragma unroll
-  for (int i = 0; i < AM_MAXT; ++i) {
-    const int ti = wave + AM_WAVES * i;
-    if (ti >= tiles) continue;
-    const int nt = ti % ntt;
-    if (nt * 16 + r < Tout) {
-#pragma unroll
-      for (int e = 0; e < 4; ++e) { const float d = acc[i][e] - mean; v = fmaf(d, d, v); }
-    }
-  }
-  const float rstd = 1.0f / sqrtf(am_block_sum(v, red, 1) / n + 1e-5f);
 #pragma unroll
   for (int i = 0; i < AM_MAXT; ++i) {
     const int ti = wave + AM_WAVES * i;
@@ -174,43 +215,95 @@
       am_store_split<NP>(outs + t * RSD + (co >> 1), PLANE, y);
     }
   }
-  __syncthreads();
-}
-
-template <int NP, int LGCI, int LGCO, int STRIDE, bool DS>
+}
+
+template <int NP, int WS = 1>
+__device__ __forceinline__ void am_gn(f32x4 (&acc)[AM_MAXT], int Cout, int Tout, const float *__restrict__ g,
+                                      const float *__restrict__ b, const u32 *resid, const float *up, bool relu, u32 *outs,
+                                      float *outf, float *__restrict__ gout, float *red) {
+  f32x4 gg[AM_MAXT], bb[AM_MAXT];
+  am_gn_affine(Cout, Tout, g, b, gg, bb);
+  const int C1[1] = {Cout}, T1[1] = {Tout};
+  float mean[1], rstd[1];
+  am_gn_stats<WS, 1>(reinterpret_cast<const f32x4 (&)[1][AM_MAXT]>(acc), C1, T1, red, mean, rstd);
+  am_gn_apply<NP>(acc, Cout, Tout, mean[0], rstd[0], gg, bb, resid, up, relu, outs, outf, gout);
+  __syncthreads();
+}
+
+template <int NP, int WS, bool JOINT, int LGCI, int LGCO, int STRIDE, bool DS>
 __device__ __forceinline__ void am_res(const u32 *in, int Tin, const AmRes &W, u32 *out, u32 *t1, u32 *t2, float *red) {
   constexpr int Cout = 1 << LGCO;
   const int Tout = Tin / STRIDE;
+  const u32 *resid = in;
+  if (DS && JOINT) {
+    f32x4 acc2[2][AM_MAXT];
+    am_conv<NP, LGCI, 3, STRIDE>(in, Tin, W.c1, Cout, Tout, acc2[0]);
+      am_conv<NP, LGCI, 1, STRIDE>(in, Tin, W.ds, Cout, Tout, acc2[1]);
+      AM_MARK();
+    f32x4 gg[2][AM_MAXT], bb[2][AM_MAXT];
+    am_gn_affine(Cout, Tout, W.g1, W.b1, gg[0], bb[0]);
+    am_gn_affine(Cout, Tout, W.gd, W.bd, gg[1], bb[1]);
+    const int C2[2] = {Cout, Cout}, T2[2] = {Tout, Tout};
+    float mean[2], rstd[2];
+    am_gn_stats<WS, 2>(acc2, C2, T2, red, mean, rstd);
+    am_gn_apply<NP>(acc2[0], Cout, Tout, mean[0], rstd[0], gg[0], bb[0], nullptr, nullptr, true, t1, nullptr, nullptr);
+    am_gn_apply<NP>(acc2[1], Cout, Tout, mean[1], rstd[1], gg[1], bb[1], nullptr, nullptr, false, t2, nullptr, nullptr);
+    __syncthreads();
+    AM_MARK();
+    resid = t2;
+  }
   f32x4 acc[AM_MAXT];
-  am_conv<NP, LGCI, 3, STRIDE>(in, Tin, W.c1, Cout, Tout, acc);
-  AM_MARK();
-  am_gn<NP>(acc, Cout, Tout, W.g1, W.b1, nullptr, nullptr, true, t1, nullptr, nullptr, red);
-  AM_MARK();
-  const u32 *resid = in;
-  if (DS) {
-    am_conv<NP, LGCI, 1, STRIDE>(in, Tin, W.ds, Cout, Tout, acc);
-    AM_MARK();
-    am_gn<NP>(acc, Cout, Tout, W.gd, W.bd, nullptr, nullptr, false, t2, nullptr, nullptr, red);
-    AM_MARK();
-    resid = t2;
+  if (!(DS && JOINT)) {
+    am_conv<NP, LGCI, 3, STRIDE>(in, Tin, W.c1, Cout, Tout, acc);
+    AM_MARK();
+    am_gn<NP, WS>(acc, Cout, Tout, W.g1, W.b1, nullptr, nullptr, true, t1, nullptr, nullptr, red);
+    AM_MARK();
+    if (DS) {
+      am_conv<NP, LGCI, 1, STRIDE>(in, Tin, W.ds, Cout, Tout, acc);
+      AM_MARK();
+      am_gn<NP, WS>(acc, Cout, Tout, W.gd, W.bd, nullptr, nullptr, false, t2, nullptr, nullptr, red);
+      AM_MARK();
+      resid = t2;
+    }
   }
   am_conv<NP, LGCO, 3, 1>(t1, Tout, W.c2, Cout, Tout, acc);
   AM_MARK();
-  am_gn<NP>(acc, Cout, Tout, W.g2, W.b2, resid, nullptr, true, out, nullptr, nullptr, red);
-  AM_MARK();
-}
-
-template <int NP, int LGC>
+  am_gn<NP, WS>(acc, Cout, Tout, W.g2, W.b2, resid, nullptr, true, out, nullptr, nullptr, red);
+  AM_MARK();
+}
+
+template <int NP, int WS, int LGC>
 __device__ __forceinline__ void am_lateral(const u32 *src, int T, const AmLat &W, const float *up, float *dstf, u32 *dsts,
                                            float *red) {
   f32x4 acc[AM_MAXT];
   am_conv<NP, LGC, 3, 1>(src, T, W.w, 128, T, acc);
   AM_MARK();
-  am_gn<NP>(acc, 128, T, W.g, W.b, nullptr, up, false, dsts, dstf, nullptr, red);
-  AM_MARK();
-}
-
-template <int NP>
+  am_gn<NP, WS>(acc, 128, T, W.g, W.b, nullptr, up, false, dsts, dstf, nullptr, red);
+  AM_MARK();
+}
+
+template <int NP, int WS, int LGCA, int LGCB>
+__device__ __forceinline__ void am_lateral_pair(const u32 *srca, const u32 *srcb, int Ta , const AmLat &La,
+                                                const AmLat &Lb, const float *up, float *dsta, float *dstbf, u32 *dstbs, float *red) {
+  const int Tb = 2 * Ta;
+  f32x4 acc[2][AM_MAXT];
+  am_conv<NP, LGCA, 3, 1>(srca, Ta, La.w, 128, Ta, acc[0]);
+  am_conv<NP, LGCB, 3, 1>(srcb, Tb, Lb.w, 128, Tb, acc[1]);
+  AM_MARK();
+  f32x4 gg[2][AM_MAXT], bb[2][AM_MAXT];
+  am_gn_affine(128, Ta, La.g, La.b, gg[0], bb[0]);
+  am_gn_affine(128, Tb, Lb.g, Lb.b, gg[1], bb[1]);
+  const int C2[2] = {128, 128}, T2[2] = {Ta, Tb};
+  float mean[2], rstd[2];
+  am_gn_stats<WS, 2>(acc, C2, T2, red, mean, rstd);
+  am_gn_apply<NP>(acc[0], 128, Ta, mean[0], rstd[0], gg[0], bb[0], nullptr, up, false, nullptr, dsta, nullptr);
+  __syncthreads();
+  am_gn_apply<NP>(acc[1], 128, Tb, mean[1], rstd[1], gg[1], bb[1], nullptr, dsta, false, dstbs, dstbf, nullptr);
+  __syncthreads();
+  AM_MARK();
+}
+
+template <int NP, bool JOINT = true, int WS = 1>
 __global__ __launch_bounds__(AM_T) void k_actor_mfma(const float *__restrict__ actors , int n_actors,
                                                      float *__restrict__ out , AmW W, LcSlot *clk) {
   lc_stamp_in(clk);
@@ -238,33 +331,38 @@
   if (blockIdx.x == 0 && tid == 0) am_trn_ = 0;
 #endif
   AM_MARK();
-  am_res<NP, 4, 5, 1, true>(xin, 48, W.res[0], ta, tb, tc, red);
-  am_res<NP, 5, 5, 1, false>(ta, 48, W.res[1], o0, tb, tc, red);
-  am_res<NP, 5, 6, 2, true>(o0, 48, W.res[2], ta, tb, tc, red);
-  am_res<NP, 6, 6, 1, false>(ta, 24, W.res[3], o1, tb, tc, red);
-  am_res<NP, 6, 7, 2, true>(o1, 24, W.res[4], ta, tb, tc, red);
-  am_res<NP, 7, 7, 1, false>(ta, 12, W.res[5], o2, tb, tc, red);
-  am_res<NP, 7, 8, 2, true>(o2, 12, W.res[6], ta, tb, tc, red);
-  am_res<NP, 8, 8, 1, false>(ta, 6, W.res[7], o3, tb, tc, red);
-  am_lateral<NP, 8>(o3, 6, W.lat[3], nullptr, (float *)ta, nullptr, red);
-  am_lateral<NP, 7>(o2, 12, W.lat[2], (const float *)ta, (float *)tb, nullptr, red);
-  am_lateral<NP, 6>(o1, 24, W.lat[1], (const float *)tb, (float *)o2, nullptr, red);
-  am_lateral<NP, 5>(o0, 48, W.lat[0], (const float *)o2, nullptr, fa, red);
+  am_res<NP, WS, JOINT, 4, 5, 1, true>(xin, 48, W.res[0], ta, tb, tc, red);
+  am_res<NP, WS, JOINT, 5, 5, 1, false>(ta, 48, W.res[1], o0, tb, tc, red);
+  am_res<NP, WS, JOINT, 5, 6, 2, true>(o0, 48, W.res[2], ta, tb, tc, red);
+  am_res<NP, WS, JOINT, 6, 6, 1, false>(ta, 24, W.res[3], o1, tb, tc, red);
+  am_res<NP, WS, JOINT, 6, 7, 2, true>(o1, 24, W.res[4], ta, tb, tc, red);
+  am_res<NP, WS, JOINT, 7, 7, 1, false>(ta, 12, W.res[5], o2, tb, tc, red);
+  am_res<NP, WS, JOINT, 7, 8, 2, true>(o2, 12, W.res[6], ta, tb, tc, red);
+  am_res<NP, WS, JOINT, 8, 8, 1, false>(ta, 6, W.res[7], o3, tb, tc, red);
+  if (JOINT) {
+    am_lateral_pair<NP, WS, 8, 7>(o3, o2, 6, W.lat[3], W.lat[2], nullptr, (float *)ta, (float *)tb, nullptr, red);
+    am_lateral_pair<NP, WS, 6, 5>(o1, o0, 24, W.lat[1], W.lat[0], (const float *)tb, (float *)o2, nullptr, fa, red);
+  } else {
+    am_lateral<NP, WS, 8>(o3, 6, W.lat[3], nullptr, (float *)ta, nullptr, red);
+    am_lateral<NP, WS, 7>(o2, 12, W.lat[2], (const float *)ta, (float *)tb, nullptr, red);
+    am_lateral<NP, WS, 6>(o1, 24, W.lat[1], (const float *)tb, (float *)o2, nullptr, red);
+    am_lateral<NP, WS, 5>(o0, 48, W.lat[0], (const float *)o2, nullptr, fa, red);
+  }
   {
     const AmRes &R = W.res[8];
     f32x4 acc[AM_MAXT];
     am_conv<NP, 7, 3, 1>(fa, 48, R.c1, 128, 48, acc);
     AM_MARK();
-    am_gn<NP>(acc, 128, 48, R.g1, R.b1, nullptr, nullptr, true, o0, nullptr, nullptr, red);
+    am_gn<NP, WS>(acc, 128, 48, R.g1, R.b1, nullptr, nullptr, true, o0, nullptr, nullptr, red);
     AM_MARK();
     am_conv<NP, 7, 3, 1>(o0, 48, R.c2, 128, 48, acc);
     AM_MARK();
-    am_gn<NP>(acc, 128, 48, R.g2, R.b2, fa, nullptr, true, nullptr, nullptr, out + (size_t)a * 128, red);
+    am_gn<NP, WS>(acc, 128, 48, R.g2, R.b2, fa, nullptr, true, nullptr, nullptr, out + (size_t)a * 128, red);
     AM_MARK();
   }
 #ifdef MIND_ACTOR_TRACE
   if (blockIdx.x == 0 && tid == 0) {
-    printf("[k_actor_mfma<%d>] cycles conv/gn per stage:", NP);
+    printf("[k_actor_mfma<%d, %s>] cycles conv/gn per stage:", NP, JOINT ? "joint" : "stage by stage");
     for (int q = 1; q < am_trn_ && q < 64; ++q) printf(" %lld", am_tr_[q] - am_tr_[q - 1]);
     printf("\n");
   }
diff --git a/mind_amd/csrc/encdec_kernels.hip b/mind_amd/csrc/encdec_kernels.hip
--- a/mind_amd/csrc/encdec_kernels.hip
+++ b/mind_amd/csrc/encdec_kernels.hip
@@ -10,15 +10,7 @@
 
 #define NT 256
 
-__device__ __forceinline__ float wave_sum(float v) {
-  v += __shfl_xor(v, 32, 64);
-  v += __shfl_xor(v, 16, 64);
-  v += __shfl_xor(v, 8, 64);
-  v += __shfl_xor(v, 4, 64);
-  v += __shfl_xor(v, 2, 64);
-  v += __shfl_xor(v, 1, 64);
-  return v;
-}
+#include "wave_sum.h"
 
 __device__ __forceinline__ float block_sum(float v, float *red) {
   v = wave_sum(v);
@@ -376,6 +368,7 @@
 }
 
 #define LN_REGS 12
+template <int WS = 1 >
 __device__ __forceinline__ void ln_rows(float *buf, int ld, int R, int n, const float *__restrict__ g,
                                         const float *__restrict__ be, bool relu) {
   const int lane = threadIdx.x & 63, wave = threadIdx.x >> 6, nw = blockDim.x >> 6;
@@ -393,11 +386,11 @@
       float s = 0.f;
 #pragma unroll
       for (int i = 0; i < LN_REGS; ++i) if (lane + 64 * i < n) s += xv[i];
-      const float mean = wave_sum(s) / (float)n;
+      const float mean = wave_sum_as<WS>(s) / (float)n;
       float v = 0.f;
 #pragma unroll
       for (int i = 0; i < LN_REGS; ++i) if (lane + 64 * i < n) { const float d = xv[i] - mean; v = fmaf(d, d, v); }
-      const float rstd = 1.0f / sqrtf(wave_sum(v) / (float)n + 1e-5f);
+      const float rstd = 1.0f / sqrtf(wave_sum_as<WS>(v) / (float)n + 1e-5f);
 #pragma unroll
       for (int i = 0; i < LN_REGS; ++i) {
         const int k = lane + 64 * i;
@@ -411,10 +404,10 @@
     }
     float s = 0.f;
     for (int k = lane; k < n; k += 64) s += buf[r * ld + k];
-    const float mean = wave_sum(s) / (float)n;
+    const float mean = wave_sum_as<WS>(s) / (float)n;
     float v = 0.f;
     for (int k = lane; k < n; k += 64) { const float d = buf[r * ld + k] - mean; v = fmaf(d, d, v); }
-    const float rstd = 1.0f / sqrtf(wave_sum(v) / (float)n + 1e-5f);
+    const float rstd = 1.0f / sqrtf(wave_sum_as<WS>(v) / (float)n + 1e-5f);
     for (int k = lane; k < n; k += 64) {
       float y = (buf[r * ld + k] - mean) * rstd * g[k] + be[k];
       if (relu) y = fmaxf(y, 0.f);
@@ -429,56 +422,64 @@
 #ifndef DT
 #define DT 1024
 #endif
+#define LANE_PF (2 * LR * 128)
+template <int NPL, int K>
+__device__ __forceinline__ void lane_dense(const float *in, int ldi, const float *__restrict__ WT, const float *__restrict__ b, float *out, int ldo,
+                                           float *part) {
+  if (NPL == PL) dense<LR>(in, ldi, K, WT, b, 128, out, ldo, part, LANE_PF);
+  else dense_ksplit<NPL * 10, 3>(in, ldi, K, WT, b, 128, out, ldo, part, dense_scalar_kp(LR, 128, K, DT, LANE_PF));
+}
+template <int NPL, int WS>
 __global__ __launch_bounds__(DT) void k_lane_net(const float *__restrict__ feats, int n_poly,
                                                  float *__restrict__ out, LaneW W) {
-  __shared__ __attribute__((aligned(16))) float xin[LR][16];
-  __shared__ __attribute__((aligned(16))) float x[LR][128];
-  __shared__ __attribute__((aligned(16))) float hcat[LR][256];
-  __shared__ __attribute__((aligned(16))) float t1[LR][128];
-  __shared__ __attribute__((aligned(16))) float part[2 * LR * 128];
-  const int PF = 2 * LR * 128;
-  const int tid = threadIdx.x;
-  const int p0 = blockIdx.x * PL;
-  for (int i = tid; i < LR * 16; i += blockDim.x) {
+  constexpr int NR = NPL * 10;
+  __shared__ __attribute__((aligned(16))) float xin[NR][16];
+  __shared__ __attribute__((aligned(16))) float x[NR][128];
+  __shared__ __attribute__((aligned(16))) float hcat[NR][256];
+  __shared__ __attribute__((aligned(16))) float t1[NR][128];
+  __shared__ __attribute__((aligned(16))) float part[2 * NR * 128];
+  const int tid = threadIdx.x;
+  const int p0 = blockIdx.x * NPL;
+  for (int i = tid; i < NR * 16; i += blockDim.x) {
     const int r = i / 16, c = i % 16;
     const int pl = p0 + r / 10;
     xin[r][c] = pl < n_poly ? feats[((size_t)pl * 10 + r % 10) * 16 + c] : 0.f;
   }
   __syncthreads();
-  dense<LR>(&xin[0][0], 16, 16, W.pW, W.pb, 128, &x[0][0], 128, part, PF);
-  __syncthreads();
-  ln_rows(&x[0][0], 128, LR, 128, W.pg, W.pbe, true);
+  lane_dense<NPL, 16>(&xin[0][0], 16, W.pW, W.pb, &x[0][0], 128, part);
+  __syncthreads();
+  ln_rows<WS>(&x[0][0], 128, NR, 128, W.pg, W.pbe, true);
   __syncthreads();
   for (int blk = 0; blk < 2; ++blk) {
-    dense<LR>(&x[0][0], 128, 128, W.f10W[blk], W.f10b[blk], 128, &t1[0][0], 128, part, PF);
-    __syncthreads();
-    ln_rows(&t1[0][0], 128, LR, 128, W.f10g[blk], W.f10be[blk], true);
-    __syncthreads();
-    dense<LR>(&t1[0][0], 128, 128, W.f13W[blk], W.f13b[blk], 128, &hcat[0][0], 256, part, PF);
-    __syncthreads();
-    ln_rows(&hcat[0][0], 256, LR, 128, W.f13g[blk], W.f13be[blk], true);
-    __syncthreads();
-    for (int i = tid; i < PL * 128; i += blockDim.x) {
+    lane_dense<NPL, 128>(&x[0][0], 128, W.f10W[blk], W.f10b[blk], &t1[0][0], 128, part);
+    __syncthreads();
+    ln_rows<WS>(&t1[0][0], 128, NR, 128, W.f10g[blk], W.f10be[blk], true);
+    __syncthreads();
+    lane_dense<NPL, 128>(&t1[0][0], 128, W.f13W[blk], W.f13b[blk], &hcat[0][0], 256, part);
+    __syncthreads();
+    ln_rows<WS>(&hcat[0][0], 256, NR, 128, W.f13g[blk], W.f13be[blk], true);
+    __syncthreads();
+    for (int i = tid; i < NPL * 128; i += blockDim.x) {
       const int pl = i / 128, c = i % 128;
       float m = hcat[pl * 10][c];
       for (int q = 1; q < 10; ++q) m = fmaxf(m, hcat[pl * 10 + q][c]);
       for (int q = 0; q < 10; ++q) hcat[pl * 10 + q][128 + c] = m;
     }
     __syncthreads();
-    dense<LR>(&hcat[0][0], 256, 256, W.f20W[blk], W.f20b[blk], 128, &t1[0][0], 128, part, PF);
-    __syncthreads();
-    ln_rows(&t1[0][0], 128, LR, 128, W.f20g[blk], W.f20be[blk], true);
-    __syncthreads();
-    dense<LR>(&t1[0][0], 128, 128, W.f23W[blk], W.f23b[blk], 128, &hcat[0][0], 256, part, PF);
-    __syncthreads();
-    ln_rows(&hcat[0][0], 256, LR, 128, W.f23g[blk], W.f23be[blk], true);
-    __syncthreads();
-    for (int i = tid; i < LR * 128; i += blockDim.x) x[i / 128][i % 128] += hcat[i / 128][i % 128];
-    __syncthreads();
-    ln_rows(&x[0][0], 128, LR, 128, W.ng[blk], W.nbe[blk], false);
-    __syncthreads();
-  }
-  for (int i = tid; i < PL * 128; i += blockDim.x) {
+    lane_dense<NPL, 256>(&hcat[0][0], 256, W.f20W[blk], W.f20b[blk], &t1[0][0], 128, part);
+    __syncthreads();
+    ln_rows<WS>(&t1[0][0], 128, NR, 128, W.f20g[blk], W.f20be[blk], true);
+    __syncthreads();
+    lane_dense<NPL, 128>(&t1[0][0], 128, W.f23W[blk], W.f23b[blk], &hcat[0][0], 256, part);
+    __syncthreads();
+    ln_rows<WS>(&hcat[0][0], 256, NR, 128, W.f23g[blk], W.f23be[blk], true);
+    __syncthreads();
+    for (int i = tid; i < NR * 128; i += blockDim.x) x[i / 128][i % 128] += hcat[i / 128][i % 128];
+    __syncthreads();
+    ln_rows<WS>(&x[0][0], 128, NR, 128, W.ng[blk], W.nbe[blk], false);
+    __syncthreads();
+  }
+  for (int i = tid; i < NPL * 128; i += blockDim.x) {
     const int pl = i / 128, c = i % 128;
     if (p0 + pl < n_poly) {
       float m = x[pl * 10][c];
diff --git a/mind_amd/csrc/mind_hip.hip b/mind_amd/csrc/mind_hip.hip
--- a/mind_amd/csrc/mind_hip.hip
+++ b/mind_amd/csrc/mind_hip.hip
@@ -195,6 +195,7 @@
   std::vector<float> lc_last[LC_KINDS], ev_last[LC_KINDS];
   int n_cu = 256;
   int debug_layers = 6;
+  int enc_forms[3] = {-1, -1, -1};
   int last_ntok = 0;
   size_t il_dbg[6] = {0, 0, 0, 0, 0, 0};
   long long last_edge_pairs = 0;
@@ -247,6 +248,8 @@
       {k_pair<0>, pair}, {k_pair<1>, pair}, {k_pair_bf<0, 3>, pair_bf}, {k_pair_bf<1, 3>, pair_bf}, {k_pair_bf<0, 1>, pair_bf}, {k_pair_bf<1, 1>, pair_bf},
       {k_pair_t<0, 3>, pair_bf}, {k_pair_t<1, 3>, pair_bf}, {k_pair_t<0, 1>, pair_bf}, {k_pair_t<1, 1>, pair_bf}, {k_pair_t6<0>, pair_bf}, {k_pair_t6<1>, pair_bf},
       {k_actor_net, mind_actor_lds_bytes()}, {k_actor_mfma<3>, actor_m}, {k_actor_mfma<6>, actor_m}, {k_actor_mfma<1>, actor_m},
+      {k_actor_mfma<3, false>, actor_m}, {k_actor_mfma<6, false>, actor_m}, {k_actor_mfma<1, false>, actor_m}, {k_actor_mfma<6, true, 0>, actor_m},
+      {k_actor_mfma<6, false, 0>, actor_m},
       {k_dec_actor_mfma<1>, dec_m}, {k_dec_actor_mfma<3>, dec_m}, {k_dec_actor_mfma<6>, dec_m}, {k_actor_f32<1>, mind_actor_f32_lds_bytes(1)}, {k_actor_f32<2>, mind_actor_f32_lds_bytes(2)},
       {k_ilqr<true, 0>, il}, {k_ilqr<false, 1>, il}, {k_ilqr<false, 0>, il}, {k_ilqr<false, 2>, il}, {k_token_mfma<0>, tok_m}, {k_token_mfma<1>, tok_m},
       {k_dec_scene, dec_s}, {k_dec_scene_mw, dec_s}, {k_dec_scene_c, dec_s}, {k_dec_cls, dec_s}, {k_dec_tgt, dec_s},
@@ -1119,6 +1122,31 @@
   c->debug_layers = n;
   return MIND_OK;
 }
+extern "C" int mind_debug_encoder_forms(mind_ctx *c, int actor_form, int lane_form, int wave_sum_form) {
+  if (!c || actor_form < -1 || actor_form > 0 || lane_form < -1 || lane_form > 0 || wave_sum_form < -1 || wave_sum_form > 0) return MIND_EINVAL;
+  c->enc_forms[0] = actor_form; c->enc_forms[1] = lane_form; c->enc_forms[2] = wave_sum_form;
+  return MIND_OK;
+}
+__global__ void k_debug_wave_sum(const float *__restrict__ in, float *__restrict__ out_shuffle, float *__restrict__ out_register) {
+  const size_t i = (size_t)blockIdx.x * 64 + threadIdx.x;
+  const float v = in[i];
+  out_shuffle[i] = wave_sum_shfl(v);
+  out_register[i] = wave_sum_reg(v);
+}
+extern "C" int mind_debug_wave_sum(mind_ctx *c, const float *in, int n_waves, float *out_shuffle, float *out_register) {
+  if (!c || !in || !out_shuffle || !out_register || n_waves <= 0 || n_waves > (1 << 20)) return MIND_EINVAL;
+  const size_t n = (size_t)n_waves * 64, bytes = n * sizeof(float);
+  DevBuf d;
+  if (d.alloc(3 * bytes) != hipSuccess) return fail(c, MIND_ENOMEM, "hipMalloc(%zu) failed", 3 * bytes);
+  float *di = (float *)d.p;
+  HIPCHK(c, hipMemcpy(di, in, bytes, hipMemcpyHostToDevice));
+  hipLaunchKernelGGL(k_debug_wave_sum, dim3(n_waves), dim3(64), 0, c->stream, (const float *)di, di + n, di + 2 * n);
+  HIPCHK(c, hipGetLastError());
+  HIPCHK(c, hipStreamSynchronize(c->stream));
+  HIPCHK(c, hipMemcpy(out_shuffle, di + n, bytes, hipMemcpyDeviceToHost));
+  HIPCHK(c, hipMemcpy(out_register, di + 2 * n, bytes, hipMemcpyDeviceToHost));
+  return MIND_OK;
+}
 extern "C" int64_t mind_debug_read(mind_ctx *c, const char *name, float *host, int64_t max_floats) {
   if (!c || !name) return MIND_EINVAL;
   const void *src = nullptr;
diff --git a/mind_amd/csrc/predict.hip b/mind_amd/csrc/predict.hip
--- a/mind_amd/csrc/predict.hip
+++ b/mind_amd/csrc/predict.hip
@@ -323,11 +323,35 @@
     break;
   }
   default:
-    if (ch.np == 6) hipLaunchKernelGGL(k_actor_mfma<6>, grid, dim3(AM_T), mind_actor_mfma_lds_bytes(), p.st, actors, A, actor_feat, c->W.actorB, clk);
-    else if (ch.np == 3) hipLaunchKernelGGL(k_actor_mfma<3>, grid, dim3(AM_T), mind_actor_mfma_lds_bytes(), p.st, actors, A, actor_feat, c->W.actorB, clk);
-    else hipLaunchKernelGGL(k_actor_mfma<1>, grid, dim3(AM_T), mind_actor_mfma_lds_bytes(), p.st, actors, A, actor_feat, c->W.actorB, clk);
-  }
-  return MIND_OK;
+    {
+      const bool joint = c->enc_forms[0] != 0, wsr = c->enc_forms[2] != 0;
+      const size_t lds = mind_actor_mfma_lds_bytes();
+#define ACTOR_MFMA(...) hipLaunchKernelGGL((k_actor_mfma<__VA_ARGS__>), grid, dim3(AM_T), lds, p.st, actors, A, actor_feat, c->W.actorB, clk)
+      if (ch.np == 6) {
+        if (joint && wsr) ACTOR_MFMA(6);
+        else if (joint) ACTOR_MFMA(6, true, 0);
+        else if (wsr) ACTOR_MFMA(6, false);
+        else ACTOR_MFMA(6, false, 0);
+      } else if (ch.np == 3) {
+        if (joint) ACTOR_MFMA(3); else ACTOR_MFMA(3, false);
+      } else {
+        if (joint) ACTOR_MFMA(1); else ACTOR_MFMA(1, false);
+      }
+#undef ACTOR_MFMA
+    }
+  }
+  return MIND_OK;
+}
+
+static void lane_net_launch(mind_ctx *c, hipStream_t st, const float *feats, int n, float *out) {
+  const bool one = c->enc_forms[1] != 0 && n <= c->n_cu, wsr = c->enc_forms[2] != 0;
+  if (one) {
+    if (wsr) hipLaunchKernelGGL((k_lane_net<1, 1>), dim3(n), dim3(DT), 0, st, feats, n, out, c->W.lane);
+    else hipLaunchKernelGGL((k_lane_net<1, 0>), dim3(n), dim3(DT), 0, st, feats, n, out, c->W.lane);
+  } else {
+    if (wsr) hipLaunchKernelGGL((k_lane_net<PL, 1>), dim3((n + PL - 1) / PL), dim3(DT), 0, st, feats, n, out, c->W.lane);
+    else hipLaunchKernelGGL((k_lane_net<PL, 0>), dim3((n + PL - 1) / PL), dim3(DT), 0, st, feats, n, out, c->W.lane);
+  }
 }
 
 static int pred_encoders(PredCall &p) {
@@ -363,8 +387,7 @@
   p.lane_feat = in->lane_feat;
   if (!p.lane_feat) {
     float *lf = p.out->lane_feat ? p.out->lane_feat : (float *)c->lane_feat.p;
-    if (Ltot > 0)
-      hipLaunchKernelGGL(k_lane_net, dim3((Ltot + PL - 1) / PL), dim3(DT), 0, ss, in->lanes, Ltot, lf, c->W.lane);
+    if (Ltot > 0) lane_net_launch(c, ss, in->lanes, Ltot, lf);
     p.lane_feat = lf;
   } else if (p.out->lane_feat && p.out->lane_feat != in->lane_feat && Ltot > 0) {
     HIPCHK(c, hipMemcpyAsync(p.out->lane_feat, in->lane_feat, (size_t)Ltot * 128 * sizeof(float), hipMemcpyDeviceToDevice, ss));
@@ -375,7 +398,7 @@
     HIPCHK(c, hipEventRecord(c->ev_side, c->side));
     HIPCHK(c, hipStreamWaitEvent(st, c->ev_side, 0));
   }
-  hipLaunchKernelGGL(k_lane_net, dim3((Bn + PL - 1) / PL), dim3(DT), 0, ss, in->tgt_nodes, Bn, (float *)c->tgt_feat.p, c->W.lane);
+  lane_net_launch(c, ss, in->tgt_nodes, Bn, (float *)c->tgt_feat.p);
   hipLaunchKernelGGL(k_dec_tgt, dim3(Bn), dim3(DT), mind_dec_scene_lds_bytes(), ss, (const float *)c->tgt_feat.p, in->tgt_rpe, (float *)c->tgt_emb.p,
                      c->W.dec);
   if (c->enc_post) {
diff --git a/mind_amd/csrc/wave_sum.h b/mind_amd/csrc/wave_sum.h
--- /dev/null
+++ b/mind_amd/csrc/wave_sum.h
@@ -0,0 +1,38 @@
+#pragma once
+#include <hip/hip_runtime.h>
+
+__device__ __forceinline__ float wave_sum_shfl(float v) {
+  v += __shfl_xor(v, 32, 64);
+  v += __shfl_xor(v, 16, 64);
+  v += __shfl_xor(v, 8, 64);
+  v += __shfl_xor(v, 4, 64);
+  v += __shfl_xor(v, 2, 64);
+  v += __shfl_xor(v, 1, 64);
+  return v;
+}
+
+template <int CTRL, int BANK_MASK>
+__device__ __forceinline__ float wave_dpp(float old, float v) {
+  return __uint_as_float((unsigned)__builtin_amdgcn_update_dpp((int)__float_as_uint(old), (int)__float_as_uint(v), CTRL, 0xf, BANK_MASK, false));
+}
+
+__device__ __forceinline__ float wave_sum_reg(float v) {
+  {
+    const auto p = __builtin_amdgcn_permlane32_swap(__float_as_uint(v), __float_as_uint(v), false, false);
+    v = __uint_as_float(p[0]) + __uint_as_float(p[1]);
+  }
+  {
+    const auto p = __builtin_amdgcn_permlane16_swap(__float_as_uint(v), __float_as_uint(v), false, false);
+    v = __uint_as_float(p[0]) + __uint_as_float(p[1]);
+  }
+  v += wave_dpp<0x128, 0xf>(v, v);
+  v += wave_dpp<0x104, 0x5>(wave_dpp<0x114, 0xa>(v, v), v);
+  v += wave_dpp<0x4e, 0xf>(v, v);
+  v += wave_dpp<0xb1, 0xf>(v, v);
+  return v;
+}
+
+__device__ __forceinline__ float wave_sum(float v) { return wave_sum_reg(v); }
+
+template <int FORM >
+__device__ __forceinline__ float wave_sum_as(float v) { return FORM == 0 ? wave_sum_shfl(v) : wave_sum_reg(v); }
diff --git a/mind_amd/predictor.py b/mind_amd/predictor.py
--- a/mind_amd/predictor.py
+++ b/mind_amd/predictor.py
@@ -273,6 +273,18 @@
 
     def debug_set_layers(self, n):
         _lib.check(self.lib, self.ctx, self.lib.mind_debug_set_layers(self.ctx, n), "mind_debug_set_layers")
+
+    def debug_encoder_forms(self, actor_form=-1, lane_form=-1, wave_sum_form=-1):
+        _lib.check(self.lib, self.ctx, self.lib.mind_debug_encoder_forms(self.ctx, actor_form, lane_form, wave_sum_form), "mind_debug_encoder_forms")
+
+    def debug_wave_sum(self, values):
+        v = np.ascontiguousarray(values, np.float32)
+        assert v.ndim == 2 and v.shape[1] == 64, v.shape
+        a, b = np.empty_like(v), np.empty_like(v)
+        fp = C.POINTER(C.c_float)
+        _lib.check(self.lib, self.ctx, self.lib.mind_debug_wave_sum(self.ctx, v.ctypes.data_as(fp), v.shape[0], a.ctypes.data_as(fp), b.ctypes.data_as(fp)),
+                   "mind_debug_wave_sum")
+        return a, b
 
     def debug_read(self, name):
         n = self.lib.mind_debug_read(self.ctx, name.encode(), None, 0)
```

New measurement: 1950, median of 6. No clear change (+1.1%).
